# ascentai/diy-gym

Hardware: NVIDIA B200
Metric: aggregate env-steps/sec (higher is better)
Workload: dtype f32

## Files before the change

diy_gym_b200/csrc/dg_env.cuh:

```cuda
#pragma once
#include "dg_math.cuh"
#include "dg_scene.h"

namespace dg {

struct Env {
  const DevScene* sc;
  float* ws;
  float* wg;
  float* st;
  float* pr;
  const float* act;
  float* obs;
  float* rew;
  uint8_t* term;
  const int* link_i;
  const float* link_f;
  const float* link_x;
  uint32_t seed;
  int env_id;
  bool active;
  int grp0, grp1;
  unsigned long long opmask[2];
  unsigned long long* dbg;
  unsigned* dropped;
  int split;
  int* rs_lists; int rs_stride;
  int* rs_count;
  int e_local;
  unsigned* rs_used;
  int no_hot;
};

#define SC (*C.sc)
#if defined(__CUDA_ARCH__)
DG_HD float* as_shared(float* p) { __builtin_assume(__isShared(p)); return p; }
DG_HD float* as_global(float* p) { __builtin_assume(__isGlobal(p)); return p; }
template <class P> DG_HD const P* gc(const P* p) { __builtin_assume(__isGlobal(p)); return p; }
template <class P> DG_HD const P* shc(const P* p) { __builtin_assume(__isShared(p)); return p; }
#else
DG_HD float* as_shared(float* p) { return p; }
DG_HD float* as_global(float* p) { return p; }
template <class P> DG_HD const P* gc(const P* p) { return p; }
template <class P> DG_HD const P* shc(const P* p) { return p; }
#endif
#define WSH(C, off) (as_shared((C).ws) + (off))
#define WSG(C, off) (as_global((C).wg) + (off))
#define WSI(C) ((int*)as_shared((C).ws))
#define WSP(C, off) ((off) >= 0 ? (C).ws + (off) : (C).wg + ~(off))
#define WSIP(C, off) ((int*)WSP(C, off))
#define KIN(s) (WSG(C, SC.W_KIN) + 12 * (s))
#define LNK(gl) (WSG(C, SC.W_LINK) + LK_W * (gl))
#define ABA(s) (WSG(C, SC.X_ABA) + AB_W * (s))
#define LNX(gl) (WSG(C, SC.X_LNK) + LX_W * (gl))
#define DOF(k, d) (as_shared(C.ws)[SC.W_DOF + (k) * SC.nd + (d)])
#define BST(di) (WSH(C, SC.W_BST) + 13 * (di))
#define ST(name) (as_global(C.st) + DG_SO(C.sc, name))
#define PR(name) (as_global(C.pr) + DG_PO(C.sc, name))

DG_HD float clampf(float x, float lo, float hi) { return fminf(fmaxf(x, lo), hi); }
DG_HD int float_as_int(float f) { union { float f; int i; } u; u.f = f; return u.i; }
DG_HD float int_as_float(int i) { union { float f; int i; } u; u.i = i; return u.f; }

DG_FN void phase_load(const Env& C, int ln, int nt) {
  const DevScene& sc = SC;
  for (int i = ln; i < 13 * sc.ndyn; i += nt) {
    int di = i / 13, k = i - 13 * di, b = gc(sc.dyn_body)[di];
    float v;
    if (k < 3) v = ST(S_BPOS)[3 * b + k];
    else if (k < 7) v = ST(S_BQUAT)[4 * b + k - 3];
    else if (k < 10) v = ST(S_BVEL)[3 * b + k - 7];
    else v = ST(S_BOMEGA)[3 * b + k - 10];
    BST(di)[k] = v;
  }
  for (int d = ln; d < sc.nd; d += nt) {
    float qd = ST(S_QD)[d];
    DOF(D_Q, d) = ST(S_Q)[d]; DOF(D_QD, d) = qd; DOF(D_APPLIED, d) = ST(S_MAPPLIED)[d];
    DOF(D_TAU, d) = ST(S_JTORQUE)[d] - PR(P_JDAMP)[d] * qd;
  }
  for (int f = ln; f < sc.nb; f += nt) {
    int s = gc(sc.frame_slot)[f];
    if (s < 0 || gc(sc.body_i)[DG_BODY_I_W * f] != 0) continue;
    float* K = KIN(s);
    q_to_mat(K, ST(S_BQUAT) + 4 * f); v_cpy(K + 9, ST(S_BPOS) + 3 * f);
  }
  if (ln == 0) for (int i = 0; i < WH_COUNT; i++) WSI(C)[sc.W_HDR + i] = 0;
}

DG_FN void joint_xform(const Env& C, int gl, float q, float* E, float* r) {
  const int* li = shc(C.link_i) + DG_LINK_I_W * gl; const float* lf = shc(C.link_f) + DG_LINK_F_W * gl; const float* R0 = shc(C.link_x) + 16 * gl;
  float Rrel[9], tmp[3];
  if (li[2] == 1) { float Ra[9]; axis_angle_mat(Ra, lf + 10, q, C.sc->precise != 0); m_mul(Rrel, R0, Ra); m_vec(tmp, Rrel, lf + 7); }
  else if (li[2] == 2) { m_cpy(Rrel, R0); float dd[3] = {lf[7] + lf[10] * q, lf[8] + lf[11] * q, lf[9] + lf[12] * q}; m_vec(tmp, R0, dd); }
  else { m_cpy(Rrel, R0); m_vec(tmp, R0, lf + 7); }
  v_add(r, lf + 4, tmp);
  E[0] = Rrel[0]; E[1] = Rrel[3]; E[2] = Rrel[6]; E[3] = Rrel[1]; E[4] = Rrel[4]; E[5] = Rrel[7]; E[6] = Rrel[2]; E[7] = Rrel[5]; E[8] = Rrel[8];
}
DG_HD int parent_slot(const int* li, int l0, int s0) { return li[1] < 0 ? s0 : s0 + 1 + (li[1] - l0); }

struct F4 { float x, y, z, w; };
DG_HD F4 ld4(const float* p) {
#if defined(__CUDA_ARCH__)
  float4 v = *reinterpret_cast<const float4*>(p); F4 o = {v.x, v.y, v.z, v.w}; return o;
#else
  F4 o = {p[0], p[1], p[2], p[3]}; return o;
#endif
}
DG_HD void st4(float* p, float x, float y, float z, float w) {
#if defined(__CUDA_ARCH__)
  *reinterpret_cast<float4*>(p) = make_float4(x, y, z, w);
#else
  p[0] = x; p[1] = y; p[2] = z; p[3] = w;
#endif
}
template <int N> DG_HD void ldn(const float* p, float* o) {
#pragma unroll
  for (int c = 0; c < N / 4; c++) { F4 v = ld4(p + 4 * c); o[4 * c] = v.x; o[4 * c + 1] = v.y; o[4 * c + 2] = v.z; o[4 * c + 3] = v.w; }
}
template <int N> DG_HD void stn(float* p, const float* v) {
#pragma unroll
  for (int c = 0; c < N / 4; c++) st4(p + 4 * c, v[4 * c], v[4 * c + 1], v[4 * c + 2], v[4 * c + 3]);
}

template <bool BIAS>
DG_FN void fk_vel_body(const Env& C, int b) {
  const DevScene& sc = SC;
  const int* bi = gc(sc.body_i) + DG_BODY_I_W * b; const int* bp = gc(sc.body_plan) + BP_W * b;
  const int kind = bi[0], l0 = bi[1], nlb = bi[2], s0 = bp[BP_SLOT];
  const float* bs = BST(bp[BP_DI]);
  const float *mass = PR(P_MASS), *inertia = PR(P_INERTIA);
  const float kl = PR(P_LINDAMP)[b], ka = PR(P_ANGDAMP)[b];
  float Kp[12], Vp[6];
  q_to_mat(Kp, bs + 3); v_cpy(Kp + 9, bs);
  mT_vec(Vp, Kp, bs + 10); mT_vec(Vp + 3, Kp, bs + 7);
  int prev = s0;
  for (int k = -1; k < nlb; k++) {
    const int s = s0 + 1 + k, f = k < 0 ? b : sc.nb + l0 + k;
    float K[12], V[6], cacc[8] = {0, 0, 0, 0, 0, 0, 0, 0};
    if (k < 0) {
      for (int i = 0; i < 12; i++) K[i] = Kp[i];
      for (int i = 0; i < 6; i++) V[i] = Vp[i];
    } else {
      const int gl = l0 + k; const int* li = shc(C.link_i) + DG_LINK_I_W * gl; const float* lx = shc(C.link_x) + 16 * gl;
      const int ps = parent_slot(li, l0, s0), dof = li[3];
      if (ps != prev) { ldn<12>(KIN(ps), Kp); const float* pv = ABA(ps) + AB_WV; for (int i = 0; i < 6; i++) Vp[i] = pv[i]; }
      float E[9], r[3], t[3], t2[3];
      joint_xform(C, gl, dof >= 0 ? DOF(D_Q, dof) : 0.f, E, r);
      float* L = LNK(gl);
      st4(L, E[0], E[1], E[2], E[3]); st4(L + 4, E[4], E[5], E[6], E[7]); st4(L + 8, E[8], r[0], r[1], r[2]);
      m_mulT(K, Kp, E);
      m_vec(t, Kp, r); v_add(K + 9, Kp + 9, t);
      m_vec(V, E, Vp);
      v_cross(t, Vp, r); v_add(t2, Vp + 3, t); m_vec(V + 3, E, t2);
      if (dof >= 0) {
        const float qd = DOF(D_QD, dof);
        if (BIAS) { float sa[3], sl[3]; v_scale(sa, lx + 9, qd); v_scale(sl, lx + 12, qd); v_cross(cacc, V, sa); v_cross(cacc + 3, V, sl); v_cross(t2, V + 3, sa); v_add(cacc + 3, cacc + 3, t2); }
        v_madd(V, lx + 9, qd); v_madd(V + 3, lx + 12, qd);
      }
      if (BIAS) stn<8>(LNX(gl), cacc);
    }
    stn<12>(KIN(s), K);
    float* X = ABA(s);
    if (!BIAS) {
      for (int i = 0; i < 6; i++) X[AB_WV + i] = V[i];
    } else if (k < 0 && kind != 2) {
      float z[40]; for (int i = 0; i < 40; i++) z[i] = 0.f;
      for (int i = 0; i < 6; i++) z[AB_WV + i] = V[i];
      stn<40>(X, z);
    } else {
      const float wsc = ((sc.sem & SEM_WRENCH_FIRST_SUBSTEP) && WSI(C)[sc.W_HDR + WH_SUB] > 0) ? 0.f : 1.f;
      const float efv[3] = {wsc * ST(S_EXTF)[3 * f], wsc * ST(S_EXTF)[3 * f + 1], wsc * ST(S_EXTF)[3 * f + 2]}, etv[3] = {wsc * ST(S_EXTT)[3 * f], wsc * ST(S_EXTT)[3 * f + 1], wsc * ST(S_EXTT)[3 * f + 2]};
      const float *ef = efv, *et = etv;
      const float m = mass[f]; const float* I = inertia + 3 * f; const float *w = V, *v = V + 3;
      float Iw[3] = {I[0] * w[0], I[1] * w[1], I[2] * w[2]}, t[3], fw[3], pa[3], pl[3];
      v_cross(pa, w, Iw);
      v_cross(t, w, v); v_scale(pl, t, m);
      fw[0] = sc.g[0] * m + ef[0]; fw[1] = sc.g[1] * m + ef[1]; fw[2] = sc.g[2] * m + ef[2];
      mT_vec(t, K, fw); v_sub(pl, pl, t);
      mT_vec(t, K, et); v_sub(pa, pa, t);
      const float wn = v_len(w), vn = v_len(v);
      const bool dlin = (sc.sem & SEM_DAMPING_LINEAR) != 0;
      v_madd(pa, Iw, dlin ? ka : ka + ka * wn);
      float mv[3]; v_scale(mv, v, m); v_madd(pl, mv, dlin ? kl : kl + kl * vn);
      float z[40]; for (int i = 0; i < 40; i++) z[i] = 0.f;
      for (int i = 0; i < 3; i++) { z[AB_PA + i] = pa[i]; z[AB_PA + 3 + i] = pl[i]; z[AB_WV + i] = w[i]; z[AB_WV + 3 + i] = v[i]; }
      z[AB_A] = I[0]; z[AB_A + 4] = I[1]; z[AB_A + 8] = I[2]; z[AB_C] = m; z[AB_C + 4] = m; z[AB_C + 8] = m;
      stn<40>(X, z);
    }
    for (int i = 0; i < 12; i++) Kp[i] = K[i];
    for (int i = 0; i < 6; i++) Vp[i] = V[i];
    prev = s;
  }
}

DG_HD void ia_mul(const float* A, const float* B, const float* Cm, const float* a, const float* l, float* n, float* f) {
  float t[3]; m_vec(n, A, a); m_vec(t, B, l); v_add(n, n, t); mT_vec(f, B, a); m_vec(t, Cm, l); v_add(f, f, t);
}
DG_FN int invert_small(float* M, int n, float* inv) {
  for (int i = 0; i < n; i++) for (int j = 0; j < n; j++) inv[i * n + j] = (i == j) ? 1.f : 0.f;
  for (int c = 0; c < n; c++) {
    int p = c;
    for (int r2 = c + 1; r2 < n; r2++) if (fabsf(M[r2 * n + c]) > fabsf(M[p * n + c])) p = r2;
    if (fabsf(M[p * n + c]) < 1e-30f) return -1;
    if (p != c) for (int j = 0; j < n; j++) { float t = M[c * n + j]; M[c * n + j] = M[p * n + j]; M[p * n + j] = t; t = inv[c * n + j]; inv[c * n + j] = inv[p * n + j]; inv[p * n + j] = t; }
    float d = 1.0f / M[c * n + c];
    for (int j = 0; j < n; j++) { M[c * n + j] *= d; inv[c * n + j] *= d; }
    for (int r2 = 0; r2 < n; r2++) if (r2 != c) {
      float fct = M[r2 * n + c];
      if (fct != 0.f) for (int j = 0; j < n; j++) { M[r2 * n + j] -= fct * M[c * n + j]; inv[r2 * n + j] -= fct * inv[c * n + j]; }
    }
  }
  return 0;
}

template <int N> DG_HD void inv_spd(const float (&A)[N][N], float (&Out)[N][N]) {
  float L[N][N], Li[N][N], invd[N];
#pragma unroll
  for (int j = 0; j < N; j++) {
    float d = A[j][j];
#pragma unroll
    for (int k = 0; k < N; k++) if (k < j) d -= L[j][k] * L[j][k];
    const float ljj = sqrtf(fmaxf(d, 1e-30f)), inv = 1.0f / ljj;
    L[j][j] = ljj; invd[j] = inv;
#pragma unroll
    for (int i = 0; i < N; i++) if (i > j) {
      float v = A[i][j];
#pragma unroll
      for (int k = 0; k < N; k++) if (k < j) v -= L[i][k] * L[j][k];
      L[i][j] = v * inv;
    }
  }
#pragma unroll
  for (int j = 0; j < N; j++) {
    Li[j][j] = invd[j];
#pragma unroll
    for (int i = 0; i < N; i++) if (i > j) {
      float v = 0.f;
#pragma unroll
      for (int k = 0; k < N; k++) if (k >= j && k < i) v -= L[i][k] * Li[k][j];
      Li[i][j] = v * invd[i];
    }
  }
#pragma unroll
  for (int i = 0; i < N; i++)
#pragma unroll
    for (int j = 0; j < N; j++) {
      float v = 0.f;
#pragma unroll
      for (int k = 0; k < N; k++) if (k >= i && k >= j) v += Li[k][i] * Li[k][j];
      Out[i][j] = v;
    }
}
DG_FN void aba_body(const Env& C, int b, float h) {
  const DevScene& sc = SC;
  const int* bi = gc(sc.body_i) + DG_BODY_I_W * b; const int* bp = gc(sc.body_plan) + BP_W * b;
  const int kind = bi[0], l0 = bi[1], nlb = bi[2], s0 = bp[BP_SLOT], di = bp[BP_DI];
  for (int k = nlb - 1; k >= 0; k--) {
    const int gl = l0 + k, s = s0 + 1 + k; const int* li = shc(C.link_i) + DG_LINK_I_W * gl;
    const int ps = parent_slot(li, l0, s0);
    float Xr[40], Lr[12], cx[8];
    ldn<40>(ABA(s), Xr); ldn<12>(LNK(gl), Lr); ldn<8>(LNX(gl), cx);
    float* Aa = Xr + AB_A; float* Ba = Xr + AB_B; float* Ca = Xr + AB_C; const float* pA = Xr + AB_PA;
    float pa[6], n[3], fo[3];
    if (li[3] >= 0) {
      const float* lx = shc(C.link_x) + 16 * gl; const float *sa = lx + 9, *sl = lx + 12;
      float U[6];
      ia_mul(Aa, Ba, Ca, sa, sl, U, U + 3);
      const float D = v_dot(sa, U) + v_dot(sl, U + 3);
      const float uu = DOF(D_TAU, li[3]) - (v_dot(sa, pA) + v_dot(sl, pA + 3));
      float* L = LNK(gl);
      st4(L + 12, U[0], U[1], U[2], U[3]); st4(L + 16, U[4], U[5], D, 0.f);
      LNX(gl)[6] = uu;
      const float Dinv = 1.0f / D;
#pragma unroll
      for (int i = 0; i < 3; i++)
#pragma unroll
        for (int j = 0; j < 3; j++) { Aa[3 * i + j] -= U[i] * U[j] * Dinv; Ba[3 * i + j] -= U[i] * U[3 + j] * Dinv; Ca[3 * i + j] -= U[3 + i] * U[3 + j] * Dinv; }
      ia_mul(Aa, Ba, Ca, cx, cx + 3, n, fo);
      for (int i = 0; i < 3; i++) { pa[i] = pA[i] + n[i] + U[i] * uu * Dinv; pa[3 + i] = pA[3 + i] + fo[i] + U[3 + i] * uu * Dinv; }
    } else {
      ia_mul(Aa, Ba, Ca, cx, cx + 3, n, fo);
      for (int i = 0; i < 3; i++) { pa[i] = pA[i] + n[i]; pa[3 + i] = pA[3 + i] + fo[i]; }
    }
    const float* E = Lr; const float* r = Lr + 9;
    float T1[9], Ar[9], Br[9], Cr[9];
    mT_mul(T1, E, Aa); m_mul(Ar, T1, E); mT_mul(T1, E, Ba); m_mul(Br, T1, E); mT_mul(T1, E, Ca); m_mul(Cr, T1, E);
    const float Kx[9] = {0, -r[2], r[1], r[2], 0, -r[0], -r[1], r[0], 0};
    float KC[9], BK[9], KBt[9], KCK[9];
    m_mul(KC, Kx, Cr); m_mul(BK, Br, Kx); m_mulT(KBt, Kx, Br); m_mul(KCK, KC, Kx);
    float fp[3], np_[3], t[3];
    mT_vec(fp, E, pa + 3); mT_vec(np_, E, pa); v_cross(t, r, fp); v_add(np_, np_, t);
    float* P = ABA(ps);
    float Pr[40];
    ldn<40>(P, Pr);
    for (int i = 0; i < 9; i++) { Pr[AB_A + i] += Ar[i] - BK[i] + KBt[i] - KCK[i]; Pr[AB_B + i] += Br[i] + KC[i]; Pr[AB_C + i] += Cr[i]; }
    for (int i = 0; i < 3; i++) { Pr[AB_PA + i] += np_[i]; Pr[AB_PA + 3 + i] += fp[i]; }
    stn<40>(P, Pr);
  }
  float* X0 = ABA(s0); float* a0 = X0 + AB_ACC;
#if defined(DG_OLD_INV)
  if (kind == 2) {
    float* M = WSG(C, sc.X_I0T) + bp[BP_I0OFF]; float* Iv = WSG(C, sc.W_I0) + bp[BP_I0OFF];
    const float *A = X0 + AB_A, *B = X0 + AB_B, *Cm = X0 + AB_C;
    for (int i = 0; i < 3; i++) for (int j = 0; j < 3; j++) { M[6 * i + j] = A[3 * i + j]; M[6 * i + 3 + j] = B[3 * i + j]; M[6 * (3 + i) + j] = B[3 * j + i]; M[6 * (3 + i) + 3 + j] = Cm[3 * i + j]; }
    invert_small(M, 6, Iv);
    for (int i = 0; i < 6; i++) { float sum = 0.f; for (int j = 0; j < 6; j++) sum -= Iv[6 * i + j] * X0[AB_PA + j]; a0[i] = sum; }
  } else for (int i = 0; i < 6; i++) a0[i] = 0.f;
#else
  if (kind == 2) {
    float* Iv = WSG(C, sc.W_I0) + bp[BP_I0OFF];
    float Xr[40]; ldn<40>(X0, Xr);
    const float *A = Xr + AB_A, *B = Xr + AB_B, *Cm = Xr + AB_C;
    float M[6][6], Inv[6][6];
#pragma unroll
    for (int i = 0; i < 3; i++)
#pragma unroll
      for (int j = 0; j < 3; j++) { M[i][j] = A[3 * i + j]; M[i][3 + j] = B[3 * i + j]; M[3 + i][j] = B[3 * j + i]; M[3 + i][3 + j] = Cm[3 * i + j]; }
    inv_spd<6>(M, Inv);
    float iv[36];
#pragma unroll
    for (int i = 0; i < 6; i++)
#pragma unroll
      for (int j = 0; j < 6; j++) iv[6 * i + j] = Inv[i][j];
    stn<36>(Iv, iv);
#pragma unroll
    for (int i = 0; i < 6; i++) { float sum = 0.f;
#pragma unroll
      for (int j = 0; j < 6; j++) sum -= Inv[i][j] * Xr[AB_PA + j];
      a0[i] = sum; }
  } else for (int i = 0; i < 6; i++) a0[i] = 0.f;
#endif
  float ap[8]; int prev = s0;
  ldn<8>(a0, ap);
  for (int k = 0; k < nlb; k++) {
    const int gl = l0 + k, s = s0 + 1 + k; const int* li = shc(C.link_i) + DG_LINK_I_W * gl;
    const int ps = parent_slot(li, l0, s0);
    if (ps != prev) ldn<8>(ABA(ps) + AB_ACC, ap);
    float Lr[20], cx[8];
    ldn<20>(LNK(gl), Lr); ldn<8>(LNX(gl), cx);
    float t[3], t2[3], acc[8];
    m_vec(acc, Lr, ap); v_cross(t, ap, Lr + 9); v_add(t2, ap + 3, t); m_vec(acc + 3, Lr, t2);
    v_add(acc, acc, cx); v_add(acc + 3, acc + 3, cx + 3);
    if (li[3] >= 0) {
      const float* lx = shc(C.link_x) + 16 * gl;
      const float qdd = (cx[6] - (v_dot(Lr + 12, acc) + v_dot(Lr + 15, acc + 3))) / Lr[18];
      DOF(D_QD, li[3]) += h * qdd;
      v_madd(acc, lx + 9, qdd); v_madd(acc + 3, lx + 12, qdd);
    }
    acc[6] = 0.f; acc[7] = 0.f;
    stn<8>(ABA(s) + AB_ACC, acc);
    for (int i = 0; i < 8; i++) ap[i] = acc[i];
    prev = s;
  }
  if (kind == 2) {
    const float* K0 = KIN(s0); float* bs = BST(di); float t[3], lin[3], aw[3];
    v_cross(t, X0 + AB_WV, X0 + AB_WV + 3); v_add(lin, a0 + 3, t);
    m_vec(aw, K0, a0); v_madd(bs + 10, aw, h);
    m_vec(aw, K0, lin); v_madd(bs + 7, aw, h);
  }
}

DG_FN void joint_reactions(const Env& C, int b) {
  const DevScene& sc = SC;
  const int* bi = gc(sc.body_i) + DG_BODY_I_W * b; const int l0 = bi[1], nlb = bi[2], s0 = gc(sc.body_plan)[BP_W * b + BP_SLOT];
  for (int k = 0; k < nlb; k++) {
    float X[48], n[3], f[3];
    ldn<48>(ABA(s0 + 1 + k), X);
    ia_mul(X + AB_A, X + AB_B, X + AB_C, X + AB_ACC, X + AB_ACC + 3, n, f);
    float* o = ST(S_JREACT) + 6 * (l0 + k);
    for (int i = 0; i < 3; i++) { o[i] = X[AB_PA + 3 + i] + f[i]; o[3 + i] = X[AB_PA + i] + n[i]; }
  }
}
DG_FN void phase_dynamics(const Env& C, int ln, int nt, float h) {
  for (int di = ln; di < SC.ndyn; di += nt) { int b = gc(SC.dyn_body)[di]; fk_vel_body<true>(C, b); aba_body(C, b, h); if (SC.need_react) joint_reactions(C, b); }
}

DG_FN void minv_column(const Env& C, int b, int col, float* scr) {
  const DevScene& sc = SC;
  const int* bi = gc(sc.body_i) + DG_BODY_I_W * b; const int* bp = gc(sc.body_plan) + BP_W * b;
  const int kind = bi[0], l0 = bi[1], nlb = bi[2], d0 = bi[3], s0 = bp[BP_SLOT], g = bp[BP_GDIM], gs = bp[BP_GS];
  const int jo = kind == 2 ? 6 : 0;
  float* out = WSH(C, sc.W_MINV) + bp[BP_MINVOFF] + col * gs;
  for (int i = g; i < gs; i++) out[i] = 0.f;
  (void)scr;
  float uu[DG_MINV_MAXL], ast[6 * DG_MINV_MAXD];
  for (int k = 0; k < nlb; k++) uu[k] = 0.f;
  float p[6] = {0, 0, 0, 0, 0, 0};
  if (col >= jo) {
    int k0 = -1;
    for (int k = 0; k < nlb; k++) if (shc(C.link_i)[DG_LINK_I_W * (l0 + k) + 3] == d0 + col - jo) { k0 = k; break; }
    for (int k = k0; k >= 0;) {
      const int gl = l0 + k; const int* li = shc(C.link_i) + DG_LINK_I_W * gl;
      float L[20]; ldn<20>(LNK(gl), L);
      float pa[6] = {p[0], p[1], p[2], p[3], p[4], p[5]};
      if (li[3] >= 0) {
        const float* lx = shc(C.link_x) + 16 * gl;
        const float u1 = (k == k0 ? 1.f : 0.f) - (v_dot(lx + 9, pa) + v_dot(lx + 12, pa + 3));
        uu[k] = u1; const float s = u1 / L[18];
        for (int i = 0; i < 6; i++) pa[i] += L[12 + i] * s;
      }
      float fp[3], np_[3], t[3];
      mT_vec(fp, L, pa + 3); mT_vec(np_, L, pa); v_cross(t, L + 9, fp); v_add(np_, np_, t);
      v_cpy(p, np_); v_cpy(p + 3, fp);
      k = li[1] < 0 ? -1 : li[1] - l0;
    }
  }
  float a0[6];
  if (kind == 2) {
    float K0[12]; ldn<12>(KIN(s0), K0); const float* Iv = WSG(C, sc.W_I0) + bp[BP_I0OFF];
    float gen[6] = {0, 0, 0, 0, 0, 0}, rhs[6], t[3];
    for (int i = 0; i < 6; i++) gen[i] = (i == col) ? 1.f : 0.f;
    mT_vec(t, K0, gen); v_sub(rhs, t, p); mT_vec(t, K0, gen + 3); v_sub(rhs + 3, t, p + 3);
    for (int i = 0; i < 6; i++) { float s = 0.f; for (int j = 0; j < 6; j++) s += Iv[6 * i + j] * rhs[j]; a0[i] = s; }
    m_vec(out, K0, a0); m_vec(out + 3, K0, a0 + 3);
  } else for (int i = 0; i < 6; i++) a0[i] = 0.f;
  for (int i = 0; i < 6; i++) ast[i] = a0[i];
  float ap[6] = {a0[0], a0[1], a0[2], a0[3], a0[4], a0[5]}; int prev_dep = -1;
  for (int k = 0; k < nlb; k++) {
    const int gl = l0 + k; const int* li = shc(C.link_i) + DG_LINK_I_W * gl;
    const int dep = gc(sc.link_depth)[gl];
    if (dep - 1 != prev_dep) { const float* src = ast + 6 * dep; for (int i = 0; i < 6; i++) ap[i] = src[i]; }
    float L[20]; ldn<20>(LNK(gl), L);
    float t[3], t2[3], aa[3], al[3];
    m_vec(aa, L, ap); v_cross(t, ap, L + 9); v_add(t2, ap + 3, t); m_vec(al, L, t2);
    if (li[3] >= 0) {
      const float* lx = shc(C.link_x) + 16 * gl;
      const float qdd = (uu[k] - (v_dot(L + 12, aa) + v_dot(L + 15, al))) / L[18];
      out[jo + li[3] - d0] = qdd;
      v_madd(aa, lx + 9, qdd); v_madd(al, lx + 12, qdd);
    }
    float* ak = ast + 6 * (dep + 1);
    v_cpy(ak, aa); v_cpy(ak + 3, al);
    v_cpy(ap, aa); v_cpy(ap + 3, al); prev_dep = dep;
  }
}
DG_FN void phase_minv(const Env& C, int ln, int nt) {
  const DevScene& sc = SC;
  float* scr = WSG(C, sc.X_MSCR) + sc.mscr_stride * ln;
  int item = 0;
  for (int di = 0; di < sc.ndyn; di++) {
    int b = gc(sc.dyn_body)[di], g = gc(sc.body_plan)[BP_W * b + BP_GDIM];
    for (int col = 0; col < g; col++, item++) if (item % nt == ln) minv_column(C, b, col, scr);
  }
}

struct Ct { int fa, fb; float pa[3], pb[3], n[3], dist, mu; };

DG_FN void shape_pose(const Env& C, int s, const float** R, const float** p) {
  int sl = gc(SC.shape_slot)[s];
  const float* w = sl >= 0 ? WSP(C, SC.X_SHW) + 12 * sl : gc(SC.shape_wb) + 12 * s;
  *R = w; *p = w + 9;
}
DG_FN void phase_shape_world(const Env& C, int ln, int nt) {
  const DevScene& sc = SC;
  for (int s = ln; s < sc.ns; s += nt) {
    int sl = gc(sc.shape_slot)[s];
    if (sl < 0) continue;
    const float* sf = gc(sc.shape_f) + DG_SHAPE_F_W * s; const float* K = KIN(gc(sc.frame_slot)[gc(sc.shape_i)[DG_SHAPE_I_W * s + 1]]);
    float* w = WSP(C, sc.X_SHW) + 12 * sl; float Rl[9], R[9], t[3];
    q_to_mat(Rl, sf + 3); m_mul(R, K, Rl); m_cpy(w, R); m_vec(t, K, sf); v_add(w + 9, K + 9, t);
  }
  int nw = (sc.npair + 31) / 32;
  for (int i = ln; i < nw; i += nt) WSIP(C, sc.X_SURV)[i] = 0;
  if (ln == 0) { int* hdr = WSI(C) + sc.W_HDR; hdr[WH_NCONTACT] = 0; hdr[WH_RS_R] = 0; hdr[WH_RS_DEFER] = 0; }
}
DG_HD void ct_add(Ct* list, int* n, int cap, int fa, int fb, const float* pa, const float* pb, const float* nrm, float dist, float mu, float margin) {
  if (dist > margin || *n >= cap) return;
  Ct* c = &list[(*n)++]; c->fa = fa; c->fb = fb; v_cpy(c->pa, pa); v_cpy(c->pb, pb); v_cpy(c->n, nrm); c->dist = dist; c->mu = mu;
}
DG_FN int sphere_box(const float* c, float r, const float* Rb, const float* pb, const float* h, float* pa_out, float* pb_out, float* n, float* dist) {
  float d[3], cl[3], q[3]; v_sub(d, c, pb); mT_vec(cl, Rb, d);
  int inside = 1;
  for (int i = 0; i < 3; i++) { q[i] = cl[i]; if (q[i] > h[i]) { q[i] = h[i]; inside = 0; } else if (q[i] < -h[i]) { q[i] = -h[i]; inside = 0; } }
  float nl[3] = {0, 0, 0};
  if (!inside) {
    float dv[3]; v_sub(dv, cl, q); float len = v_len(dv);
    if (len < 1e-12f) return 0;
    v_scale(nl, dv, 1.0f / len); *dist = len - r;
  } else {
    int ax = 0; float best = 1e30f;
    for (int i = 0; i < 3; i++) { float pen = h[i] - fabsf(cl[i]); if (pen < best) { best = pen; ax = i; } }
    float sg = cl[ax] >= 0 ? 1.0f : -1.0f;
    for (int i = 0; i < 3; i++) if (i == ax) { nl[i] = sg; q[i] = sg * h[i]; }
    *dist = -best - r;
  }
  m_vec(n, Rb, nl); float t[3]; m_vec(t, Rb, q); v_add(pb_out, pb, t);
  v_scale(t, n, -r); v_add(pa_out, c, t);
  return 1;
}
DG_FN int point_box(const float* p, const float* Rb, const float* pb, const float* h, float margin, float* pb_out, float* n, float* dist) {
  float d[3], pl[3]; v_sub(d, p, pb); mT_vec(pl, Rb, d);
  int ax = 0; float best = 1e30f;
  for (int i = 0; i < 3; i++) { float pen = h[i] - fabsf(pl[i]); if (pen < -margin) return 0; if (pen < best) { best = pen; ax = i; } }
  float nl[3] = {0, 0, 0}, q[3] = {pl[0], pl[1], pl[2]};
  float sg = pl[ax] >= 0 ? 1.0f : -1.0f;
  for (int i = 0; i < 3; i++) if (i == ax) { nl[i] = sg; q[i] = sg * h[i]; }
  m_vec(n, Rb, nl); float t[3]; m_vec(t, Rb, q); v_add(pb_out, pb, t); *dist = -best;
  return 1;
}
DG_FN void seg_closest(const float* p1, const float* d1, const float* p2, const float* d2, float* s, float* t) {
  float r[3]; v_sub(r, p1, p2);
  float a = v_dot(d1, d1), e = v_dot(d2, d2), f = v_dot(d2, r);
  if (a <= 1e-18f && e <= 1e-18f) { *s = *t = 0; return; }
  if (a <= 1e-18f) { *s = 0; *t = clampf(f / e, 0.f, 1.f); return; }
  float c = v_dot(d1, r);
  if (e <= 1e-18f) { *t = 0; *s = clampf(-c / a, 0.f, 1.f); return; }
  float b = v_dot(d1, d2), den = a * e - b * b;
  *s = den > 1e-18f ? clampf((b * f - c * e) / den, 0.f, 1.f) : 0.0f;
  *t = (b * (*s) + f) / e;
  if (*t < 0) { *t = 0; *s = clampf(-c / a, 0.f, 1.f); } else if (*t > 1) { *t = 1; *s = clampf((b - c) / a, 0.f, 1.f); }
}
DG_FN void as_capsule(int type, const float* dims, const float* R, const float* p, float* e0, float* e1, float* rad) {
  float half = 0; *rad = dims[0];
  if (type == SHAPE_CAPSULE) half = dims[1];
  else if (type == SHAPE_CYLINDER) half = dims[1] - dims[0] > 0 ? dims[1] - dims[0] : 0;
  float ax[3] = {R[2] * half, R[5] * half, R[8] * half};
  v_sub(e0, p, ax); v_add(e1, p, ax);
}
DG_HD bool pair_in_reach(const Env& C, int sa, int sb) {
  const float *Ra, *pa, *Rb, *pb;
  shape_pose(C, sa, &Ra, &pa); shape_pose(C, sb, &Rb, &pb);
  float dc[3]; v_sub(dc, pa, pb);
  const float ra = gc(SC.shape_f)[DG_SHAPE_F_W * sa + 11], rb = gc(SC.shape_f)[DG_SHAPE_F_W * sb + 11];
  float reach = ra + rb + SC.margin;
  if (v_dot(dc, dc) > reach * reach) return false;
  for (int side = 0; side < 2; side++) {
    const int sx = side ? sa : sb;
    const int* ix = gc(SC.shape_i) + DG_SHAPE_I_W * sx;
    if (ix[2] != SHAPE_BOX || ix[5] > 0) continue;
    const float *Rx = side ? Ra : Rb, *px = side ? pa : pb, *po = side ? pb : pa; const float* h = gc(SC.shape_f) + DG_SHAPE_F_W * sx + 7;
    float d[3], pl[3]; v_sub(d, po, px); mT_vec(pl, Rx, d);
    float d2 = 0.f;
    for (int i = 0; i < 3; i++) { const float ex = fabsf(pl[i]) - h[i]; if (ex > 0.f) d2 += ex * ex; }
    const float r = (side ? rb : ra) + SC.margin;
    if (d2 > r * r) return false;
  }
  return true;
}
DG_FN int point_hull(const float* p, const float* R, const float* pos, const float* planes, int np_, float margin, float* surf, float* n, float* dist) {
  float d[3], pl[3]; v_sub(d, p, pos); mT_vec(pl, R, d);
  float best = -1e30f; int bi = 0;
  for (int k = 0; k < np_; k++) { const float* q = planes + 4 * k; const float s = q[0] * pl[0] + q[1] * pl[1] + q[2] * pl[2] - q[3]; if (s > margin) return 0; if (s > best) { best = s; bi = k; } }
  m_vec(n, R, planes + 4 * bi); *dist = best;
  surf[0] = p[0] - n[0] * best; surf[1] = p[1] - n[1] * best; surf[2] = p[2] - n[2] * best;
  return 1;
}
DG_FN void collide_convex(const Env& C, const int* ia, const float* fa, const float* Ra, const float* pa, const int* ib, const float* fb, const float* Rb, const float* pb,
                          float mu, float margin, Ct* loc, int* nloc) {
  const float* H = gc(SC.hull_f);
  for (int side = 0; side < 2; side++) {
    const int* ix = side ? ib : ia; const int* iy = side ? ia : ib; const float* fx = side ? fb : fa; const float* fy = side ? fa : fb;
    const float *Rx = side ? Rb : Ra, *px = side ? pb : pa, *Ry = side ? Ra : Rb, *py = side ? pa : pb;
    const int nvx = ix[5] > 0 ? ix[5] : 8;
    const float reach2 = (fy[11] + margin) * (fy[11] + margin);
    for (int k = 0; k < nvx; k++) {
      float vl[3], t[3], pt[3], surf[3], n[3], dist;
      if (ix[5] > 0) { const float* v = H + ix[4] + 3 * k; vl[0] = v[0]; vl[1] = v[1]; vl[2] = v[2]; }
      else { vl[0] = (k & 1 ? 1 : -1) * fx[7]; vl[1] = (k & 2 ? 1 : -1) * fx[8]; vl[2] = (k & 4 ? 1 : -1) * fx[9]; }
      m_vec(t, Rx, vl); v_add(pt, px, t);
      { float dy[3]; v_sub(dy, pt, py); if (v_dot(dy, dy) > reach2) continue; }
      const int hit = iy[5] > 0 ? point_hull(pt, Ry, py, H + iy[6], iy[7], margin, surf, n, &dist) : point_box(pt, Ry, py, fy + 7, margin, surf, n, &dist);
      if (!hit) continue;
      if (side == 0) ct_add(loc, nloc, 16, ia[1], ib[1], pt, surf, n, dist, mu, margin);
      else { float nn[3]; v_scale(nn, n, -1.0f); ct_add(loc, nloc, 16, ia[1], ib[1], surf, pt, nn, dist, mu, margin); }
    }
  }
}
DG_FN int collide_pair(const Env& C, int sa, int sb, Ct* out) {
  const DevScene& sc = SC;
  const int *ia = gc(sc.shape_i) + DG_SHAPE_I_W * sa, *ib = gc(sc.shape_i) + DG_SHAPE_I_W * sb;
  const float *fa = gc(sc.shape_f) + DG_SHAPE_F_W * sa, *fb = gc(sc.shape_f) + DG_SHAPE_F_W * sb;
  const float *Ra, *pa, *Rb, *pb;
  shape_pose(C, sa, &Ra, &pa); shape_pose(C, sb, &Rb, &pb);
  float margin = sc.margin;
  int ta = ia[2], tb = ib[2];
  float mu = PR(P_FRICTION)[sa] * PR(P_FRICTION)[sb];
  int nt_ = 0;
  float ca[3], cb[3], n[3], dist;
  const bool ha = ia[5] > 0, hb_ = ib[5] > 0;
  if ((ha && (hb_ || tb == SHAPE_BOX)) || (hb_ && (ha || ta == SHAPE_BOX))) {
    Ct loc[16]; int nloc = 0;
    collide_convex(C, ia, fa, Ra, pa, ib, fb, Rb, pb, mu, margin, loc, &nloc);
    for (int i = 0; i < nloc; i++) for (int j = i + 1; j < nloc; j++) if (loc[j].dist < loc[i].dist) { Ct t = loc[i]; loc[i] = loc[j]; loc[j] = t; }
    if (nloc > 4) nloc = 4;
    for (int i = 0; i < nloc; i++) out[nt_++] = loc[i];
    return nt_;
  }
  if (ta != SHAPE_BOX && tb != SHAPE_BOX) {
    float a0[3], a1[3], b0[3], b1[3], ra, rb, d1[3], d2[3], s, t, c1[3], c2[3];
    as_capsule(ta, fa + 7, Ra, pa, a0, a1, &ra); as_capsule(tb, fb + 7, Rb, pb, b0, b1, &rb);
    v_sub(d1, a1, a0); v_sub(d2, b1, b0); seg_closest(a0, d1, b0, d2, &s, &t);
    v_cpy(c1, a0); v_madd(c1, d1, s); v_cpy(c2, b0); v_madd(c2, d2, t);
    float d[3]; v_sub(d, c1, c2); float len = v_len(d);
    if (len < 1e-12f) v_set(n, 0, 0, 1); else v_scale(n, d, 1.0f / len);
    dist = len - ra - rb; float tt[3]; v_scale(tt, n, -ra); v_add(ca, c1, tt); v_scale(tt, n, rb); v_add(cb, c2, tt);
    ct_add(out, &nt_, 4, ia[1], ib[1], ca, cb, n, dist, mu, margin);
    return nt_;
  }
  int swap = (tb != SHAPE_BOX);
  const float *Rx = swap ? Rb : Ra, *px = swap ? pb : pa, *dx = swap ? fb + 7 : fa + 7;
  const float *Rbx = swap ? Ra : Rb, *pbx = swap ? pa : pb, *hb = swap ? fa + 7 : fb + 7;
  int tx = swap ? tb : ta; int fx = swap ? ib[1] : ia[1], fbx = swap ? ia[1] : ib[1];
  Ct loc[16]; int nloc = 0;
  if (tx == SHAPE_SPHERE) {
    if (sphere_box(px, dx[0], Rbx, pbx, hb, ca, cb, n, &dist)) ct_add(loc, &nloc, 16, fx, fbx, ca, cb, n, dist, mu, margin);
  } else if (tx == SHAPE_CAPSULE) {
    float e0[3], e1[3], rad, mid[3], dseg[3], rel[3];
    as_capsule(tx, dx, Rx, px, e0, e1, &rad);
    v_sub(dseg, e1, e0); v_sub(rel, pbx, e0);
    float dd = v_dot(dseg, dseg), tt = dd > 1e-18f ? clampf(v_dot(rel, dseg) / dd, 0.f, 1.f) : 0.0f;
    v_cpy(mid, e0); v_madd(mid, dseg, tt);
    if (sphere_box(e0, rad, Rbx, pbx, hb, ca, cb, n, &dist)) ct_add(loc, &nloc, 16, fx, fbx, ca, cb, n, dist, mu, margin);
    if (dd > 1e-18f && sphere_box(e1, rad, Rbx, pbx, hb, ca, cb, n, &dist)) ct_add(loc, &nloc, 16, fx, fbx, ca, cb, n, dist, mu, margin);
    if (tt > 1e-6f && tt < 1 - 1e-6f && sphere_box(mid, rad, Rbx, pbx, hb, ca, cb, n, &dist)) ct_add(loc, &nloc, 16, fx, fbx, ca, cb, n, dist, mu, margin);
  } else if (tx == SHAPE_CYLINDER) {
    float zc[3] = {Rx[2], Rx[5], Rx[8]}, xc[3] = {Rx[0], Rx[3], Rx[6]}, yc[3] = {Rx[1], Rx[4], Rx[7]};
    for (int cap = -1; cap <= 1; cap += 2) {
      float cc[3]; v_cpy(cc, px); v_madd(cc, zc, cap * dx[1]);
      for (int k = 0; k < 6; k++) {
        float sg = k < 3 ? 1.f : -1.f; int a3 = k % 3;
        float nk[3] = {-Rbx[a3] * sg, -Rbx[3 + a3] * sg, -Rbx[6 + a3] * sg};
        float t[3]; v_cpy(t, nk); v_madd(t, zc, -v_dot(nk, zc));
        float len = v_len(t), pt[3];
        int npt = len < 1e-6f ? 4 : 1;
        for (int j4 = 0; j4 < npt; j4++) {
          if (npt == 4) { const float* bx = (j4 & 1) ? yc : xc; float s2 = (j4 & 2) ? -1.0f : 1.0f; v_cpy(pt, cc); v_madd(pt, bx, s2 * dx[0]); }
          else { v_cpy(pt, cc); v_madd(pt, t, dx[0] / len); }
          if (point_box(pt, Rbx, pbx, hb, margin, cb, n, &dist)) {
            int dup = 0;
            for (int j = 0; j < nloc; j++) { float dd[3]; v_sub(dd, loc[j].pa, pt); if (v_dot(dd, dd) < 1e-12f) dup = 1; }
            if (!dup) ct_add(loc, &nloc, 16, fx, fbx, pt, cb, n, dist, mu, margin);
          }
        }
      }
    }
  } else {
    for (int k = 0; k < 8; k++) {
      float cl[3] = {(k & 1 ? 1 : -1) * dx[0], (k & 2 ? 1 : -1) * dx[1], (k & 4 ? 1 : -1) * dx[2]}, pt[3], t[3];
      m_vec(t, Rx, cl); v_add(pt, px, t);
      if (point_box(pt, Rbx, pbx, hb, margin, cb, n, &dist)) ct_add(loc, &nloc, 16, fx, fbx, pt, cb, n, dist, mu, margin);
    }
    for (int k = 0; k < 8; k++) {
      float cl[3] = {(k & 1 ? 1 : -1) * hb[0], (k & 2 ? 1 : -1) * hb[1], (k & 4 ? 1 : -1) * hb[2]}, pt[3], t[3], nn[3], cx[3];
      m_vec(t, Rbx, cl); v_add(pt, pbx, t);
      if (point_box(pt, Rx, px, dx, margin, cx, nn, &dist)) { v_scale(nn, nn, -1.0f); ct_add(loc, &nloc, 16, fx, fbx, cx, pt, nn, dist, mu, margin); }
    }
  }
  for (int i = 0; i < nloc; i++) for (int j = i + 1; j < nloc; j++) if (loc[j].dist < loc[i].dist) { Ct t = loc[i]; loc[i] = loc[j]; loc[j] = t; }
  if (nloc > 4) nloc = 4;
  for (int i = 0; i < nloc; i++) {
    Ct c = loc[i];
    if (swap) { Ct s2 = c; s2.fa = c.fb; s2.fb = c.fa; v_cpy(s2.pa, c.pb); v_cpy(s2.pb, c.pa); v_scale(s2.n, c.n, -1.0f); c = s2; }
    out[nt_++] = c;
  }
  return nt_;
}
DG_HD void surv_set(int* word, int bit) {
#if defined(__CUDA_ARCH__)
  atomicOr(word, 1 << bit);
#else
  *word |= 1 << bit;
#endif
}
DG_HD int ffs64(unsigned long long x) {
#if defined(__CUDA_ARCH__)
  return __ffsll((long long)x);
#else
  return __builtin_ffsll((long long)x);
#endif
}
DG_HD int popc32(unsigned x) {
#if defined(__CUDA_ARCH__)
  return __popc(x);
#else
  return __builtin_popcount(x);
#endif
}
DG_FN void phase_broad(const Env& C, int ln, int nt) {
  const DevScene& sc = SC;
  for (int it = ln; it < sc.ngrp + sc.nloose; it += nt) {
    if (it < sc.ngrp) {
      const int* g = gc(sc.grp_i) + 4 * it; const float* w = gc(sc.shape_wb) + 12 * g[0];
      const float* cb = KIN(gc(sc.body_plan)[BP_W * g[1] + BP_SLOT]) + 9;
      float dc[3]; v_sub(dc, w + 9, cb);
      float reach = gc(sc.shape_f)[DG_SHAPE_F_W * g[0] + 11] + gc(sc.body_reach)[g[1]] + sc.margin;
      if (v_dot(dc, dc) > reach * reach) continue;
      {
        const int* is = gc(sc.shape_i) + DG_SHAPE_I_W * g[0];
        if (is[2] == SHAPE_BOX && is[5] == 0) {
          const float* h = gc(sc.shape_f) + DG_SHAPE_F_W * g[0] + 7;
          float d[3], pl[3]; v_sub(d, cb, w + 9); mT_vec(pl, w, d);
          float d2 = 0.f;
          for (int i = 0; i < 3; i++) { const float ex = fabsf(pl[i]) - h[i]; if (ex > 0.f) d2 += ex * ex; }
          const float r = gc(sc.body_reach)[g[1]] + sc.margin;
          if (d2 > r * r) continue;
        }
      }
      for (int j = 0; j < g[3]; j++) {
        int k = gc(sc.grp_pairs)[g[2] + j];
        if (pair_in_reach(C, gc(sc.pair_i)[2 * k], gc(sc.pair_i)[2 * k + 1])) surv_set(WSIP(C, sc.X_SURV) + (k >> 5), k & 31);
      }
    } else {
      int k = gc(sc.loose_pairs)[it - sc.ngrp];
      if (pair_in_reach(C, gc(sc.pair_i)[2 * k], gc(sc.pair_i)[2 * k + 1])) surv_set(WSIP(C, sc.X_SURV) + (k >> 5), k & 31);
    }
  }
}
DG_FN void phase_count_survivors(const Env& C, int ln, int nt) {
  if (ln != 0) return;
  int nw = (SC.npair + 31) / 32, n = 0;
  for (int i = 0; i < nw; i++) n += popc32((unsigned)WSIP(C, SC.X_SURV)[i]);
  WSI(C)[SC.W_HDR + WH_NSURV] = n;
}
DG_FN void phase_narrow(const Env& C, int ln, int nt, int rnd) {
  const DevScene& sc = SC;
  float* tmp = WSG(C, sc.X_CTMP) + sc.ctmp_stride * ln;
  int want = rnd * nt + ln, nw = (sc.npair + 31) / 32, seen = 0, pair = -1;
  for (int i = 0; i < nw && pair < 0; i++) {
    unsigned wd = (unsigned)WSIP(C, sc.X_SURV)[i]; int c = popc32(wd);
    if (seen + c <= want) { seen += c; continue; }
    for (int bit = 0; bit < 32; bit++) if (wd & (1u << bit)) { if (seen == want) { pair = 32 * i + bit; break; } seen++; }
  }
  int n = 0;
  if (pair >= 0) {
    Ct out[4];
    n = collide_pair(C, gc(sc.pair_i)[2 * pair], gc(sc.pair_i)[2 * pair + 1], out);
    for (int i = 0; i < n; i++) {
      float* c = tmp + 1 + CT_W * i;
      c[CT_FA] = int_as_float(out[i].fa); c[CT_FB] = int_as_float(out[i].fb);
      v_cpy(c + CT_PA, out[i].pa); v_cpy(c + CT_PB, out[i].pb); v_cpy(c + CT_N, out[i].n); c[CT_DIST] = out[i].dist; c[CT_MU] = out[i].mu;
    }
  }
  tmp[0] = int_as_float(n);
}
DG_FN void phase_append(const Env& C, int ln, int nt) {
  if (ln != 0) return;
  const DevScene& sc = SC;
  int nc = WSI(C)[sc.W_HDR + WH_NCONTACT], lost = 0;
  for (int l = 0; l < nt; l++) {
    const float* tmp = WSG(C, sc.X_CTMP) + sc.ctmp_stride * l; int n = float_as_int(tmp[0]);
    for (int i = 0; i < n; i++) {
      const float* src = tmp + 1 + CT_W * i; float* dst;
      if (nc < sc.maxc) dst = WSP(C, sc.X_CON) + CT_W * nc++;
      else {
        lost++;
        int worst = 0; float wd = (WSP(C, sc.X_CON))[CT_DIST];
        for (int j = 1; j < nc; j++) { const float dj = (WSP(C, sc.X_CON) + CT_W * j)[CT_DIST]; if (dj > wd) { wd = dj; worst = j; } }
        if (nc == 0 || !(src[CT_DIST] < wd)) continue;
        dst = WSP(C, sc.X_CON) + CT_W * worst;
      }
      for (int j = 0; j < CT_W; j++) dst[j] = src[j];
    }
  }
  WSI(C)[sc.W_HDR + WH_NCONTACT] = nc;
  if (lost && C.dropped) {
#if defined(__CUDA_ARCH__)
    atomicAdd(C.dropped, (unsigned)lost);
#else
    *C.dropped += (unsigned)lost;
#endif
  }
}

DG_HD int body_of_frame(const Env& C, int f) { return f < C.sc->nb ? f : shc(C.link_i)[DG_LINK_I_W * (f - C.sc->nb)]; }
DG_FN void point_jacobian(const Env& C, int f, const float* p, const float* dir, float* J) {
  const DevScene& sc = SC;
  int b = body_of_frame(C, f); const int* bi = gc(sc.body_i) + DG_BODY_I_W * b; const int* bp = gc(sc.body_plan) + BP_W * b;
  int g = bp[BP_GDIM], d0 = bi[3], s0 = bp[BP_SLOT], l0 = bi[1];
  for (int i = 0; i < g; i++) J[i] = 0.f;
  int jo = 0;
  if (bi[0] == 2) { float rel[3]; v_sub(rel, p, KIN(s0) + 9); v_cross(J, rel, dir); v_cpy(J + 3, dir); jo = 6; }
  int gl = f < sc.nb ? -1 : f - sc.nb;
  while (gl >= 0) {
    const int* li = shc(C.link_i) + DG_LINK_I_W * gl; const float* lf = shc(C.link_f) + DG_LINK_F_W * gl; const float* K = KIN(s0 + 1 + gl - l0);
    if (li[2] == 1) {
      float aw[3], dw[3], o[3], rel[3], t[3];
      m_vec(aw, K, lf + 10); m_vec(dw, K, lf + 7); v_sub(o, K + 9, dw);
      v_sub(rel, p, o); v_cross(t, aw, rel); J[jo + li[3] - d0] = v_dot(dir, t);
    } else if (li[2] == 2) { float aw[3]; m_vec(aw, K, lf + 10); J[jo + li[3] - d0] = v_dot(dir, aw); }
    gl = li[1];
  }
}
DG_FN void angular_jacobian(const Env& C, int f, const float* dir, float* J) {
  const DevScene& sc = SC;
  int b = body_of_frame(C, f); const int* bi = gc(sc.body_i) + DG_BODY_I_W * b; const int* bp = gc(sc.body_plan) + BP_W * b;
  int g = bp[BP_GDIM], d0 = bi[3], s0 = bp[BP_SLOT], l0 = bi[1], jo = 0;
  for (int i = 0; i < g; i++) J[i] = 0.f;
  if (bi[0] == 2) { v_cpy(J, dir); jo = 6; }
  for (int gl = f < sc.nb ? -1 : f - sc.nb; gl >= 0; gl = shc(C.link_i)[DG_LINK_I_W * gl + 1]) {
    const int* li = shc(C.link_i) + DG_LINK_I_W * gl;
    if (li[2] == 1) { float aw[3]; m_vec(aw, KIN(s0 + 1 + gl - l0), shc(C.link_f) + DG_LINK_F_W * gl + 10); J[jo + li[3] - d0] = v_dot(dir, aw); }
  }
}
DG_FN void body_genvel(const Env& C, int b, float* gv) {
  const int* bi = gc(SC.body_i) + DG_BODY_I_W * b; int jo = 0;
  if (bi[0] == 2) { const float* bs = BST(gc(SC.body_plan)[BP_W * b + BP_DI]); v_cpy(gv, bs + 10); v_cpy(gv + 3, bs + 7); jo = 6; }
  for (int i = 0; i < bi[4]; i++) gv[jo + i] = DOF(D_QD, bi[3] + i);
}
DG_FN void phase_unit_rows(const Env& C, int ln, int nt, float h) {
  const DevScene& sc = SC;
  for (int di = ln; di < sc.ndyn; di += nt) {
    int b = gc(sc.dyn_body)[di]; const int* bi = gc(sc.body_i) + DG_BODY_I_W * b; const int* bp = gc(sc.body_plan) + BP_W * b;
    int l0 = bi[1], nlb = bi[2], d0 = bi[3], g = bp[BP_GDIM], gs = bp[BP_GS], jo = bi[0] == 2 ? 6 : 0;
    const float* Minv = WSH(C, sc.W_MINV) + bp[BP_MINVOFF];
    float* rows = WSH(C, sc.X_UROW) + UR_W * bp[BP_UROW]; int n = 0;
    for (int k = 0; k < nlb; k++) {
      const int* li = shc(C.link_i) + DG_LINK_I_W * (l0 + k); const float* lf = shc(C.link_f) + DG_LINK_F_W * (l0 + k);
      int d = li[3];
      if (d < 0 || !li[4]) continue;
      for (int side = 0; side < 2; side++) {
        float pen = side == 0 ? DOF(D_Q, d) - lf[20] : lf[21] - DOF(D_Q, d);
        if (pen > 0) continue;
        int col = jo + d - d0; float sg = side == 0 ? 1.f : -1.f;
        float den = Minv[col * gs + col], dinv = den > 1e-30f ? 1.0f / den : 0.f, rel = sg * DOF(D_QD, d);
        float* r = rows + UR_W * n++;
        r[UR_RHS] = (-rel + (-pen) * sc.erp / h) * dinv; r[UR_DINV] = dinv; r[UR_LO] = 0.f; r[UR_HI] = sc.limit_max_impulse; r[UR_APPLIED] = 0.f;
        r[UR_COL] = int_as_float(side == 0 ? col : -1 - col); r[UR_MOTOR] = int_as_float(-1);
      }
    }
    for (int k = 0; k < nlb; k++) {
      int d = shc(C.link_i)[DG_LINK_I_W * (l0 + k) + 3];
      if (d < 0) continue;
      float maxf = ST(S_MMAXF)[d];
      DOF(D_APPLIED, d) = 0.f;
      if (maxf <= 0) continue;
      int col = jo + d - d0;
      float den = Minv[col * gs + col], dinv = den > 1e-30f ? 1.0f / den : 0.f, qd = DOF(D_QD, d);
      float desired = ST(S_MKP)[d] * (ST(S_MTPOS)[d] - DOF(D_Q, d)) / h + qd + ST(S_MKD)[d] * (ST(S_MTVEL)[d] - qd);
      float* r = rows + UR_W * n++;
      r[UR_RHS] = (desired - qd) * dinv; r[UR_DINV] = dinv; const float cdt = (sc.sem & SEM_MOTOR_CLAMP_SUBSTEP) ? h : sc.dt;
      r[UR_LO] = -maxf * cdt; r[UR_HI] = maxf * cdt; r[UR_APPLIED] = 0.f;
      r[UR_COL] = int_as_float(col); r[UR_MOTOR] = int_as_float(d);
    }
    WSI(C)[sc.W_UCNT + di] = n;
    float* dv = WSH(C, sc.W_DV) + bp[BP_GVOFF];
    for (int i = 0; i < gs; i++) dv[i] = 0.f;
    int nrs = bp[BP_NRS];
    if (n <= nrs) {
      float* A = WSH(C, sc.X_AMAT) + bp[BP_AOFF];
      for (int r = 0; r < n; r++) {
        int cr = float_as_int(rows[UR_W * r + UR_COL]); float sr = 1.f; if (cr < 0) { cr = -1 - cr; sr = -1.f; }
        for (int s2 = 0; s2 < nrs; s2++) {
          float a = 0.f;
          if (s2 < n) { int cs = float_as_int(rows[UR_W * s2 + UR_COL]); float ss = 1.f; if (cs < 0) { cs = -1 - cs; ss = -1.f; } a = sr * ss * Minv[cr * gs + cs]; }
          A[r * nrs + s2] = a;
        }
      }
    }
  }
  if (ln == 0) { WSI(C)[sc.W_HDR + WH_NCROW] = 3 * WSI(C)[sc.W_HDR + WH_NCONTACT]; WSI(C)[sc.W_HDR + WH_COUPLED] = 0; }
}
DG_FN void plane_space(const float* n, float* p, float* q) {
  if (fabsf(n[2]) > 0.7071067811865475244f) { float a = n[1] * n[1] + n[2] * n[2], k = 1.0f / sqrtf(a); p[0] = 0; p[1] = -n[2] * k; p[2] = n[1] * k; q[0] = a * k; q[1] = -n[0] * p[2]; q[2] = n[0] * p[1]; }
  else { float a = n[0] * n[0] + n[1] * n[1], k = 1.0f / sqrtf(a); p[0] = -n[1] * k; p[1] = n[0] * k; p[2] = 0; q[0] = -n[2] * p[1]; q[1] = n[2] * p[0]; q[2] = a * k; }
}
DG_FN void phase_contact_rows(const Env& C, int ln, int nt, float h) {
  const DevScene& sc = SC;
  int nc = WSI(C)[sc.W_HDR + WH_NCONTACT];
  for (int r = ln; r < 3 * nc; r += nt) {
    int k = r < nc ? r : (r - nc) >> 1, dirk = r < nc ? -1 : (r - nc) & 1;
    const float* c = WSP(C, sc.X_CON) + CT_W * k;
    int fa = float_as_int(c[CT_FA]), fb = float_as_int(c[CT_FB]);
    float dir[3];
    if (dirk < 0) v_cpy(dir, c + CT_N); else { float t1[3], t2[3]; plane_space(c + CT_N, t1, t2); v_cpy(dir, dirk == 0 ? t1 : t2); }
    float* row = WSP(C, sc.X_CROW) + sc.crow_stride * r; float* J = row + CR_HDR; float* M = J + sc.GP;
    int ba = body_of_frame(C, fa), bb = body_of_frame(C, fb);
    int dia = gc(sc.body_plan)[BP_W * ba + BP_DI], dib = gc(sc.body_plan)[BP_W * bb + BP_DI];
    float den = 0.f, rel = 0.f; int ga = 0;
    if (dia >= 0) {
      const int* bp = gc(sc.body_plan) + BP_W * ba; ga = bp[BP_GDIM]; const int gsa = bp[BP_GS]; const float* Minv = WSH(C, sc.W_MINV) + bp[BP_MINVOFF];
      point_jacobian(C, fa, c + CT_PA, dir, J);
      body_genvel(C, ba, M);
      for (int i = 0; i < ga; i++) rel += J[i] * M[i];
      for (int i = 0; i < ga; i++) { float s = 0.f; for (int j = 0; j < ga; j++) s += Minv[j * gsa + i] * J[j]; M[i] = s; }
      for (int i = 0; i < ga; i++) den += J[i] * M[i];
    }
    if (dib >= 0) {
      const int* bp = gc(sc.body_plan) + BP_W * bb; int gb = bp[BP_GDIM]; const int gsb = bp[BP_GS]; const float* Minv = WSH(C, sc.W_MINV) + bp[BP_MINVOFF];
      float nd_[3]; v_scale(nd_, dir, -1.0f);
      float *JB = J + ga, *MB = M + ga;
      point_jacobian(C, fb, c + CT_PB, nd_, JB);
      body_genvel(C, bb, MB);
      for (int i = 0; i < gb; i++) rel += JB[i] * MB[i];
      for (int i = 0; i < gb; i++) { float s = 0.f; for (int j = 0; j < gb; j++) s += Minv[j * gsb + i] * JB[j]; MB[i] = s; }
      for (int i = 0; i < gb; i++) den += JB[i] * MB[i];
    }
    { int used = ga + (dib >= 0 ? gc(sc.body_plan)[BP_W * bb + BP_GDIM] : 0); for (int i = used; i < sc.GP; i++) { J[i] = 0.f; M[i] = 0.f; } }
    if (dia >= 0 && dib >= 0) WSI(C)[sc.W_HDR + WH_COUPLED] = 1;
    float dinv = den > 1e-30f ? 1.0f / den : 0.f;
    row[CR_DINV] = dinv; row[CR_APPLIED] = 0.f; row[CR_MU] = c[CT_MU]; WSH(C, sc.W_CAPP)[r] = 0.f;
    row[CR_DA] = int_as_float(dia); row[CR_DB] = int_as_float(dib);
    if (dirk < 0) {
      float pen = c[CT_DIST] + sc.slop, pos_err = 0.f, vel_err = -rel;
      if (pen > 0) vel_err -= pen / h; else pos_err = -pen * sc.cerp / h;
      row[CR_RHS] = (pos_err + vel_err) * dinv; row[CR_LO] = 0.f; row[CR_HI] = 1e10f; row[CR_PARENT] = int_as_float(-1);
    } else {
      row[CR_RHS] = -rel * dinv; row[CR_LO] = 0.f; row[CR_HI] = 0.f; row[CR_PARENT] = int_as_float(k);
    }
  }
}

DG_FN void pgs_unit_sweep(const Env& C, int b, int di, int it) {
  const DevScene& sc = SC;
  const int* bp = gc(sc.body_plan) + BP_W * b; int g = bp[BP_GDIM], gs = bp[BP_GS], n = WSI(C)[sc.W_UCNT + di];
  const float* Minv = WSH(C, sc.W_MINV) + bp[BP_MINVOFF]; float* dv = WSH(C, sc.W_DV) + bp[BP_GVOFF];
  float* rows = WSH(C, sc.X_UROW) + UR_W * bp[BP_UROW];
  for (int j = 0; j < n; j++) {
    float* r = rows + UR_W * ((it & 1) ? j : n - 1 - j);
    int colc = float_as_int(r[UR_COL]); float sg = 1.f; int col = colc;
    if (colc < 0) { col = -1 - colc; sg = -1.f; }
    float d = r[UR_RHS] - sg * dv[col] * r[UR_DINV];
    float ap = r[UR_APPLIED], sum = ap + d, lo = r[UR_LO], hi = r[UR_HI];
    if (sum < lo) { d = lo - ap; sum = lo; } else if (sum > hi) { d = hi - ap; sum = hi; }
    r[UR_APPLIED] = sum;
    float sd = sg * d; const float* Mc = Minv + col * gs;
    for (int i = 0; i < g; i++) dv[i] = fmaf(Mc[i], sd, dv[i]);
  }
}
template <int NR>
DG_FN void pgs_unit_fast(const Env& C, int b, int di, int it0, int it1) {
  const DevScene& sc = SC;
  const int* bp = gc(sc.body_plan) + BP_W * b; const int g = bp[BP_GDIM], gs = bp[BP_GS], nrs = bp[BP_NRS], n = WSI(C)[sc.W_UCNT + di];
  const float* Minv = WSH(C, sc.W_MINV) + bp[BP_MINVOFF]; float* dv = WSH(C, sc.W_DV) + bp[BP_GVOFF];
  float* rows = WSH(C, sc.X_UROW) + UR_W * bp[BP_UROW]; const float* A = WSH(C, sc.X_AMAT) + bp[BP_AOFF];
  constexpr bool kRegA = NR <= 8;
  float rhs[NR], dinv[NR], lo[NR], hi[NR], ap[NR], ap0[NR], y[NR], Ar[kRegA ? NR * NR : 1];
#pragma unroll
  for (int r = 0; r < NR; r++) {
    rhs[r] = 0.f; dinv[r] = 0.f; lo[r] = 0.f; hi[r] = 0.f; ap[r] = 0.f; y[r] = 0.f;
    if (r < n) {
      const float* rw = rows + UR_W * r;
      rhs[r] = rw[UR_RHS]; dinv[r] = rw[UR_DINV]; lo[r] = rw[UR_LO]; hi[r] = rw[UR_HI]; ap[r] = rw[UR_APPLIED];
      int c = float_as_int(rw[UR_COL]);
      y[r] = c < 0 ? -dv[-1 - c] : dv[c];
    }
    ap0[r] = ap[r];
    if (kRegA) {
#pragma unroll
      for (int s2 = 0; s2 < NR; s2++) Ar[kRegA ? r * NR + s2 : 0] = (r < n && s2 < n) ? A[r * nrs + s2] : 0.f;
    }
  }
#define DG_PGS_ROW(r)                                                                        \
  {                                                                                          \
    float d = rhs[r] - y[r] * dinv[r];                                                       \
    float sum = ap[r] + d;                                                                   \
    const bool below = sum < lo[r], above = sum > hi[r];                                     \
    d = below ? lo[r] - ap[r] : (above ? hi[r] - ap[r] : d);                                 \
    ap[r] = below ? lo[r] : (above ? hi[r] : sum);                                           \
    if (kRegA) {                                                                             \
      _Pragma("unroll") for (int s2 = 0; s2 < NR; s2++) y[s2] = fmaf(Ar[kRegA ? (r) * NR + s2 : 0], d, y[s2]); \
    } else if ((r) < n) {                                                                    \
      const float* Am = A + (r) * nrs;                                                       \
      _Pragma("unroll") for (int s2 = 0; s2 < NR; s2++) y[s2] = fmaf(Am[s2], d, y[s2]);      \
    }                                                                                        \
  }
  for (int it = it0; it < it1; it++) {
    if (it & 1) {
#pragma unroll
      for (int r = 0; r < NR; r++) DG_PGS_ROW(r)
    } else {
#pragma unroll
      for (int r = NR - 1; r >= 0; r--) DG_PGS_ROW(r)
    }
  }
#undef DG_PGS_ROW
#pragma unroll
  for (int r = 0; r < NR; r++) if (r < n) {
    float* rw = rows + UR_W * r;
    rw[UR_APPLIED] = ap[r];
    float dl = ap[r] - ap0[r];
    int c = float_as_int(rw[UR_COL]); if (c < 0) { c = -1 - c; dl = -dl; }
    const float* Mc = Minv + c * gs;
    for (int i = 0; i < g; i++) dv[i] = fmaf(Mc[i], dl, dv[i]);
  }
}
DG_FN void pgs_unit_any(const Env& C, int b, int di, int it0, int it1) {
  const int nrs = gc(SC.body_plan)[BP_W * b + BP_NRS], n = WSI(C)[SC.W_UCNT + di];
  if (n == 0) return;
  if (n <= nrs) {
    if (n <= 4) { pgs_unit_fast<4>(C, b, di, it0, it1); return; }
    if (n <= 6 && nrs >= 8) { pgs_unit_fast<6>(C, b, di, it0, it1); return; }
    if (n <= 8) { pgs_unit_fast<8>(C, b, di, it0, it1); return; }
    if (n <= 12) { pgs_unit_fast<12>(C, b, di, it0, it1); return; }
    if (n <= 16) { pgs_unit_fast<16>(C, b, di, it0, it1); return; }
  }
  for (int it = it0; it < it1; it++) pgs_unit_sweep(C, b, di, it);
}
template <int G>
DG_FN void pgs_body_full(const Env& C, int b, int di) {
  const DevScene& sc = SC;
  const int* bp = gc(sc.body_plan) + BP_W * b; const int gs = bp[BP_GS], n = WSI(C)[sc.W_UCNT + di];
  const int ncr = WSI(C)[sc.W_HDR + WH_NCROW];
  const float* Minv = WSH(C, sc.W_MINV) + bp[BP_MINVOFF]; float* dvs = WSH(C, sc.W_DV) + bp[BP_GVOFF];
  float* rows = WSH(C, sc.X_UROW) + UR_W * bp[BP_UROW];
  float* capp = WSH(C, sc.W_CAPP);
  unsigned long long mine = 0ull;
  for (int rr = 0; rr < ncr && rr < 63; rr++) {
    const float* row = WSP(C, sc.X_CROW) + sc.crow_stride * rr;
    if (float_as_int(row[CR_DA]) == di || float_as_int(row[CR_DB]) == di) mine |= 1ull << rr;
  }
  float dv[G];
#pragma unroll
  for (int i = 0; i < G; i++) dv[i] = 0.f;
  for (int it = 0; it < sc.iters; it++) {
    for (int j = 0; j < n; j++) {
      float* r = rows + UR_W * ((it & 1) ? j : n - 1 - j);
      int col = float_as_int(r[UR_COL]); float sg = 1.f;
      if (col < 0) { col = -1 - col; sg = -1.f; }
      float x = 0.f;
#pragma unroll
      for (int i = 0; i < G; i++) x = (i == col) ? dv[i] : x;
      float d = r[UR_RHS] - sg * x * r[UR_DINV];
      float ap = r[UR_APPLIED], sum = ap + d, lo = r[UR_LO], hi = r[UR_HI];
      if (sum < lo) { d = lo - ap; sum = lo; } else if (sum > hi) { d = hi - ap; sum = hi; }
      r[UR_APPLIED] = sum;
      float sd = sg * d; const float* Mc = Minv + col * gs;
#pragma unroll
      for (int c4 = 0; c4 < G / 4; c4++) if (4 * c4 < gs) {
        F4 m = ld4(Mc + 4 * c4);
        dv[4 * c4] = fmaf(m.x, sd, dv[4 * c4]); dv[4 * c4 + 1] = fmaf(m.y, sd, dv[4 * c4 + 1]);
        dv[4 * c4 + 2] = fmaf(m.z, sd, dv[4 * c4 + 2]); dv[4 * c4 + 3] = fmaf(m.w, sd, dv[4 * c4 + 3]);
      }
    }
    for (unsigned long long m = mine; m != 0ull; m &= m - 1ull) {
      const int rr = ffs64(m) - 1;
      const float* row = WSP(C, sc.X_CROW) + sc.crow_stride * rr;
      const float* J = row + CR_HDR; const float* M = J + sc.GP;
      const F4 h = ld4(row), h2 = ld4(row + 4), h3 = ld4(row + 8);
      F4 jv[G / 4], mv[G / 4];
#pragma unroll
      for (int c4 = 0; c4 < G / 4; c4++) {
        if (4 * c4 < gs) { jv[c4] = ld4(J + 4 * c4); mv[c4] = ld4(M + 4 * c4); }
        else { F4 z = {0.f, 0.f, 0.f, 0.f}; jv[c4] = z; mv[c4] = z; }
      }
      float d0 = 0.f, d1 = 0.f, d2 = 0.f, d3 = 0.f;
#pragma unroll
      for (int c4 = 0; c4 < G / 4; c4++) {
        d0 = fmaf(jv[c4].x, dv[4 * c4], d0); d1 = fmaf(jv[c4].y, dv[4 * c4 + 1], d1); d2 = fmaf(jv[c4].z, dv[4 * c4 + 2], d2); d3 = fmaf(jv[c4].w, dv[4 * c4 + 3], d3);
      }
      float d = h.x - ((d0 + d1) + (d2 + d3)) * h.y;
      float lo = h.z, hi = h.w;
      const int par = float_as_int(h3.x);
      if (par >= 0) { hi = h2.y * capp[par]; lo = -hi; }
      const float ap = capp[rr]; float sum = ap + d;
      const bool below = sum < lo, above = sum > hi;
      d = below ? lo - ap : (above ? hi - ap : d);
      capp[rr] = below ? lo : (above ? hi : sum);
#pragma unroll
      for (int c4 = 0; c4 < G / 4; c4++) {
        dv[4 * c4] = fmaf(mv[c4].x, d, dv[4 * c4]); dv[4 * c4 + 1] = fmaf(mv[c4].y, d, dv[4 * c4 + 1]);
        dv[4 * c4 + 2] = fmaf(mv[c4].z, d, dv[4 * c4 + 2]); dv[4 * c4 + 3] = fmaf(mv[c4].w, d, dv[4 * c4 + 3]);
      }
    }
  }
#pragma unroll
  for (int i = 0; i < G; i++) if (i < gs) dvs[i] = dv[i];
}
DG_FN void phase_pgs_full(const Env& C, int ln, int nt) {
  for (int di = ln; di < SC.ndyn; di += nt) {
    int b = gc(SC.dyn_body)[di], gs = gc(SC.body_plan)[BP_W * b + BP_GS];
    if (gs <= 8) pgs_body_full<8>(C, b, di); else if (gs <= 16) pgs_body_full<16>(C, b, di); else pgs_body_full<32>(C, b, di);
  }
}
DG_FN void pgs_contact_sweep(const Env& C) {
  const DevScene& sc = SC;
  int ncr = WSI(C)[sc.W_HDR + WH_NCROW];
  for (int r = 0; r < ncr; r++) {
    float* row = WSP(C, sc.X_CROW) + sc.crow_stride * r; const float* J = row + CR_HDR; const float* M = J + sc.GP;
    int dia = float_as_int(row[CR_DA]), dib = float_as_int(row[CR_DB]);
    float dot = 0.f; int ga = 0; float *dva = nullptr, *dvb = nullptr; int gb = 0;
    if (dia >= 0) { const int* bp = gc(sc.body_plan) + BP_W * gc(sc.dyn_body)[dia]; ga = bp[BP_GDIM]; dva = WSH(C, sc.W_DV) + bp[BP_GVOFF]; for (int i = 0; i < ga; i++) dot += J[i] * dva[i]; }
    if (dib >= 0) { const int* bp = gc(sc.body_plan) + BP_W * gc(sc.dyn_body)[dib]; gb = bp[BP_GDIM]; dvb = WSH(C, sc.W_DV) + bp[BP_GVOFF]; for (int i = 0; i < gb; i++) dot += J[ga + i] * dvb[i]; }
    float d = row[CR_RHS] - dot * row[CR_DINV];
    float lo = row[CR_LO], hi = row[CR_HI];
    int par = float_as_int(row[CR_PARENT]);
    float* capp = WSH(C, sc.W_CAPP);
    if (par >= 0) { hi = row[CR_MU] * capp[par]; lo = -hi; }
    float ap = capp[r], sum = ap + d;
    if (sum < lo) { d = lo - ap; sum = lo; } else if (sum > hi) { d = hi - ap; sum = hi; }
    capp[r] = sum;
    for (int i = 0; i < ga; i++) dva[i] = fmaf(M[i], d, dva[i]);
    for (int i = 0; i < gb; i++) dvb[i] = fmaf(M[ga + i], d, dvb[i]);
  }
}
DG_FN void phase_pgs_unit(const Env& C, int ln, int nt, int it0, int it1) {
  for (int di = ln; di < SC.ndyn; di += nt) pgs_unit_any(C, gc(SC.dyn_body)[di], di, it0, it1);
}
DG_FN void phase_pgs_contact(const Env& C, int ln, int nt) { if (ln == 0) pgs_contact_sweep(C); }
struct RsLayout { int K, nu, nk, nc, P1, nrm0, nrm1, P2, fr1, Rp; };
DG_HD int rs_pad(int n, int K) { return (n + K - 1) / K * K; }
DG_HD int rs_total(int nu, int nk, int nc, int K) { return rs_pad(nu, K) + rs_pad(nk + nc, K) + rs_pad(2 * nc, K); }
DG_HD RsLayout rs_layout(int K, int nu, int nk, int nc) {
  RsLayout L; L.K = K; L.nu = nu; L.nk = nk; L.nc = nc; L.P1 = rs_pad(nu, K); L.nrm0 = L.P1 + nk; L.nrm1 = L.nrm0 + nc;
  L.P2 = L.P1 + rs_pad(nk + nc, K); L.fr1 = L.P2 + 2 * nc; L.Rp = L.P2 + rs_pad(2 * nc, K);
  return L;
}
DG_HD bool rs_real(const RsLayout& L, int p) { return p < L.nu || (p >= L.P1 && p < L.nrm1) || (p >= L.P2 && p < L.fr1); }
DG_FN RsLayout rs_layout_of(const Env& C) {
  const int* hdr = WSI(C) + SC.W_HDR;
  return rs_layout(hdr[WH_RS_K], hdr[WH_RS_NU], 6 * SC.ncons, hdr[WH_NCROW] / 3);
}
DG_HD int rs_kneed(int nu, int nk, int nc, int nt, int cap) {
  for (int K = 2; K <= RS_KMAX; K *= 2) { const int t = rs_total(nu, nk, nc, K); if (t <= K * nt && t <= cap) return K; }
  return 0;
}
DG_FN void phase_rs_plan(const Env& C, int ln, int nt) {
  if (ln != 0) return;
  const DevScene& sc = SC;
  int* hdr = WSI(C) + sc.W_HDR; const int ncr = hdr[WH_NCROW];
  int nu = 0;
  for (int di = 0; di < sc.ndyn; di++) nu += WSI(C)[sc.W_UCNT + di];
  const int nk = 6 * sc.ncons, nc = ncr / 3;
  const bool want = sc.solver == 1 && nt >= 2 && (nk > 0 || (ncr > 0 && (hdr[WH_COUPLED] != 0 || ncr >= sc.rs_min)));
  hdr[WH_RS_NU] = nu; hdr[WH_RS_R] = 0; hdr[WH_RS_DEFER] = 0;
  int need = want ? rs_kneed(nu, nk, nc, nt, sc.rs_cap) : 0;
  if (want && C.split) {
    for (int c = 0; c < RS_NCLS; c++) {
      const int kc = sc.rs_cls_k[c], rc = sc.rs_cls_r[c];
      if (rc <= 0) continue;
      const int t = rs_total(nu, nk, nc, kc);
      if (t <= rc && t <= sc.rs_cap) { need = kc; hdr[WH_RS_DEFER] = c + 1; break; }
    }
  }
  hdr[WH_RS_NEED] = need;
}
DG_FN void phase_rs_setup(const Env& C, int ln, int nt) {
  const DevScene& sc = SC;
  int* hdr = WSI(C) + sc.W_HDR; const int ncr = hdr[WH_NCROW], GV = sc.GV;
  if (hdr[WH_RS_NEED] == 0) return;
  int K = 0;
  const bool defer = hdr[WH_RS_DEFER] != 0;
  if (defer) K = hdr[WH_RS_NEED];
  else for (int e2 = C.grp0; e2 < C.grp1; e2++) {
    const int* h2 = (const int*)(as_shared(C.ws) + (long)e2 * sc.w_total) + sc.W_HDR;
    const int k2 = h2[WH_RS_DEFER] ? 0 : h2[WH_RS_NEED]; K = k2 > K ? k2 : K;
  }
  const int nu = hdr[WH_RS_NU], nk = 6 * sc.ncons;
  const RsLayout L = rs_layout(K, nu, nk, ncr / 3);
  if (L.Rp > sc.rs_cap) return;
  if (ln == 0) {
    hdr[WH_RS_R] = L.Rp; hdr[WH_RS_K] = K;
#if defined(__CUDA_ARCH__)
    if (C.rs_used) atomicAdd(C.rs_used, 1u);
    if (defer) { const int cls = hdr[WH_RS_DEFER] - 1; const int slot = atomicAdd(C.rs_count + cls, 1); C.rs_lists[(size_t)cls * C.rs_stride + slot] = C.e_local; }
#endif
  }
  float* RSV = WSG(C, sc.X_RSV); float* REC = WSG(C, sc.X_RSREC);
  for (int p = ln; p < L.Rp; p += nt) if (!rs_real(L, p)) { float* rc = REC + RR_W * p; st4(rc, 0.f, 0.f, 0.f, 0.f); st4(rc + 4, 0.f, int_as_float(-1), 0.f, int_as_float(-1)); }
  int r = 0;
  for (int di = 0; di < sc.ndyn; di++) {
    const int* bp = gc(sc.body_plan) + BP_W * gc(sc.dyn_body)[di]; const int n = WSI(C)[sc.W_UCNT + di];
    for (int j = 0; j < n; j++, r++) {
      if (r % nt != ln) continue;
      const float* u = WSH(C, sc.X_UROW) + UR_W * (bp[BP_UROW] + j);
      int col = float_as_int(u[UR_COL]); float sg = 1.f; if (col < 0) { col = -1 - col; sg = -1.f; }
      float* Jd = RSV + (size_t)r * 2 * GV; float* Md = Jd + GV;
      for (int i = 0; i < 2 * GV; i += 4) st4(Jd + i, 0.f, 0.f, 0.f, 0.f);
      const int go = bp[BP_GVOFF], gs = bp[BP_GS]; const float* Mc = WSH(C, sc.W_MINV) + bp[BP_MINVOFF] + col * gs;
      Jd[go + col] = sg;
      for (int i = 0; i < gs; i++) Md[go + i] = sg * Mc[i];
      float* rc = REC + RR_W * r;
      st4(rc, u[UR_RHS], u[UR_DINV], u[UR_LO], u[UR_HI]); st4(rc + 4, 0.f, int_as_float(-1), int_as_float(((go + col) & ~3) | ((((go + col) & ~3) + 4) << 16)), int_as_float((di << 16) | j));
    }
  }
  for (int kr = 0; kr < nk; kr++) {
    const int r2 = L.P1 + kr;
    if (kr % nt != ln) continue;
    const int kc = kr / 6, i = kr % 6;
    const int* ci = gc(sc.cons_i) + DG_CONS_I_W * kc; const float* cf = gc(sc.cons_f) + DG_CONS_F_W * kc;
    const int fa = ci[0], fb = ci[1], ba = body_of_frame(C, fa), bb = body_of_frame(C, fb);
    const float *Ka = KIN(gc(sc.frame_slot)[fa]), *Kb = KIN(gc(sc.frame_slot)[fb]);
    float Pa[3], Pb[3], t[3], err;
    m_vec(t, Ka, cf); v_add(Pa, Ka + 9, t); m_vec(t, Kb, cf + 7); v_add(Pb, Kb + 9, t);
    if (i < 3) err = Pa[i] - Pb[i];
    else {
      float qa[4], qb[4], qaw[4], qbw[4], dq[4];
      mat_to_q(qa, Ka); mat_to_q(qb, Kb); q_mul(qaw, qa, cf + 3); q_mul(qbw, qb, cf + 10);
      const float qbi[4] = {-qbw[0], -qbw[1], -qbw[2], qbw[3]};
      q_mul(dq, qaw, qbi);
      const float vn = v_len(dq); float ang = 2.f * atan2f(vn, dq[3]); if (ang > kPi) ang -= 2.f * kPi;
      err = vn < 1e-12f ? 0.f : dq[i - 3] * ang / vn;
    }
    float e[3] = {0.f, 0.f, 0.f}, ne[3] = {0.f, 0.f, 0.f}; e[i % 3] = 1.f; ne[i % 3] = -1.f;
    float* Jd = RSV + (size_t)r2 * 2 * GV; float* Md = Jd + GV;
    for (int c = 0; c < 2 * GV; c += 4) st4(Jd + c, 0.f, 0.f, 0.f, 0.f);
    float den = 0.f, rel = 0.f, gvl[RS_GVMAX + 8];
    for (int side = 0; side < 2; side++) {
      const int b = side ? bb : ba, f = side ? fb : fa; const int* bp = gc(sc.body_plan) + BP_W * b;
      if (bp[BP_DI] < 0) continue;
      const int go = bp[BP_GVOFF], g = bp[BP_GDIM], gs = bp[BP_GS]; const float* Minv = WSH(C, sc.W_MINV) + bp[BP_MINVOFF];
      if (i < 3) point_jacobian(C, f, side ? Pb : Pa, side ? ne : e, Jd + go); else angular_jacobian(C, f, side ? ne : e, Jd + go);
      body_genvel(C, b, gvl);
      for (int c = 0; c < g; c++) { float sm = 0.f; for (int j = 0; j < g; j++) sm += Minv[j * gs + c] * Jd[go + j]; Md[go + c] = sm; den += Jd[go + c] * sm; rel += Jd[go + c] * gvl[c]; }
    }
    const float dinv = den > 1e-30f ? 1.0f / den : 0.f, lim = cf[14] * sc.dt, hsub = sc.dt / (float)sc.substeps;
    float* rc = REC + RR_W * r2;
    st4(rc, (-rel - err * sc.erp / hsub) * dinv, dinv, -lim, lim); st4(rc + 4, 0.f, int_as_float(-1), int_as_float(0 | (GV << 16)), int_as_float(RS_CONTACT | 0xffff));
  }
  const int nc = ncr / 3;
  for (int rr = 0; rr < ncr; rr++) {
    const int r2 = rr < nc ? L.nrm0 + rr : L.P2 + (rr - nc);
    if (rr % nt != ln) continue;
    const float* row = WSP(C, sc.X_CROW) + sc.crow_stride * rr; const float* J = row + CR_HDR; const float* M = J + sc.GP;
    const int dia = float_as_int(row[CR_DA]), dib = float_as_int(row[CR_DB]);
    float* Jd = RSV + (size_t)r2 * 2 * GV; float* Md = Jd + GV;
    for (int i = 0; i < 2 * GV; i += 4) st4(Jd + i, 0.f, 0.f, 0.f, 0.f);
    int off = 0, slo = GV, shi = 0;
#define DG_COPY_ROW(dstJ, dstM, srcJ, srcM, g_)                                                                                   \
    { int i_ = 0;                                                                                                                  \
      for (; i_ + 4 <= (g_); i_ += 4) {                                                                                            \
        const float j0_ = (srcJ)[i_], j1_ = (srcJ)[i_ + 1], j2_ = (srcJ)[i_ + 2], j3_ = (srcJ)[i_ + 3];                            \
        const float m0_ = (srcM)[i_], m1_ = (srcM)[i_ + 1], m2_ = (srcM)[i_ + 2], m3_ = (srcM)[i_ + 3];                            \
        (dstJ)[i_] = 0.f + j0_; (dstJ)[i_ + 1] = 0.f + j1_; (dstJ)[i_ + 2] = 0.f + j2_; (dstJ)[i_ + 3] = 0.f + j3_;                \
        (dstM)[i_] = 0.f + m0_; (dstM)[i_ + 1] = 0.f + m1_; (dstM)[i_ + 2] = 0.f + m2_; (dstM)[i_ + 3] = 0.f + m3_;                \
      }                                                                                                                            \
      for (; i_ < (g_); i_++) { const float j0_ = (srcJ)[i_], m0_ = (srcM)[i_]; (dstJ)[i_] = 0.f + j0_; (dstM)[i_] = 0.f + m0_; } }
    if (dia >= 0) { const int* bp = gc(sc.body_plan) + BP_W * gc(sc.dyn_body)[dia]; const int go = bp[BP_GVOFF], g = bp[BP_GDIM]; DG_COPY_ROW(Jd + go, Md + go, J, M, g) off = g; slo = go < slo ? go : slo; shi = go + bp[BP_GS] > shi ? go + bp[BP_GS] : shi; }
    if (dib >= 0) {
      const int* bp = gc(sc.body_plan) + BP_W * gc(sc.dyn_body)[dib]; const int go = bp[BP_GVOFF], g = bp[BP_GDIM];
      if (dib == dia) { for (int i = 0; i < g; i++) { Jd[go + i] += J[off + i]; Md[go + i] += M[off + i]; } }
      else DG_COPY_ROW(Jd + go, Md + go, J + off, M + off, g)
      slo = go < slo ? go : slo; shi = go + bp[BP_GS] > shi ? go + bp[BP_GS] : shi;
    }
    if (shi <= slo) { slo = 0; shi = 0; }
    float* rc = REC + RR_W * r2;
    st4(rc, row[CR_RHS], row[CR_DINV], row[CR_LO], row[CR_HI]); st4(rc + 4, row[CR_MU], row[CR_PARENT], int_as_float(slo | (shi << 16)), int_as_float(RS_CONTACT | rr));
  }
}
#undef DG_COPY_ROW
DG_FN void phase_rs_build(const Env& C, int ln, int nt) {
  const DevScene& sc = SC;
  const RsLayout L = rs_layout_of(C); const int GV = sc.GV, cap = sc.rs_cap;
  int ncol = L.K * nt; if (ncol > cap) ncol = cap; if (ncol < L.Rp) ncol = L.Rp;
  const float* RSV = WSG(C, sc.X_RSV); const float* REC = WSG(C, sc.X_RSREC); float* A = WSG(C, sc.X_RSA);
  for (int s2 = ln; s2 < ncol; s2 += nt) {
    const bool rs2 = s2 < L.Rp && rs_real(L, s2);
    int c0 = 0, c1 = 0;
    if (rs2) { const int sup = float_as_int(REC[RR_W * s2 + RR_APPLIED]); c0 = sup & 0xffff; c1 = (sup >> 16) & 0xffff; if (c1 > GV) c1 = GV; }
    const float* Jd = RSV + (size_t)s2 * 2 * GV;
    for (int p = 0; p < L.Rp; p++) {
      float a0 = 0.f, a1 = 0.f, a2 = 0.f, a3 = 0.f;
      if (rs2 && rs_real(L, p)) {
        const float* Md = RSV + (size_t)p * 2 * GV + GV;
        for (int c = c0; c < c1; c += 4) { const F4 jv = ld4(Jd + c), mv = ld4(Md + c); a0 = fmaf(jv.x, mv.x, a0); a1 = fmaf(jv.y, mv.y, a1); a2 = fmaf(jv.z, mv.z, a2); a3 = fmaf(jv.w, mv.w, a3); }
      }
      A[p * cap + s2] = (a0 + a1) + (a2 + a3);
    }
  }
}
DG_FN void phase_rs_finish(const Env& C, int ln, int nt) {
  const DevScene& sc = SC;
  const RsLayout L = rs_layout_of(C); const int GV = sc.GV;
  const float* RSV = WSG(C, sc.X_RSV); const float* REC = WSG(C, sc.X_RSREC); float* dv = WSH(C, sc.W_DV);
  for (int i = ln; i < GV; i += nt) {
    float sum = 0.f;
    for (int p = 0; p < L.Rp; p++) if (rs_real(L, p)) sum = fmaf(RSV[(size_t)p * 2 * GV + GV + i], REC[RR_W * p + RR_APPLIED], sum);
    dv[i] = sum;
  }
  for (int r = ln; r < L.nu; r += nt) {
    const int v = float_as_int(REC[RR_W * r + RR_ID]); const int* bp = gc(sc.body_plan) + BP_W * gc(sc.dyn_body)[(v >> 16) & 0x3fff];
    (WSH(C, sc.X_UROW) + UR_W * (bp[BP_UROW] + (v & 0xffff)))[UR_APPLIED] = REC[RR_W * r + RR_APPLIED];
  }
}
#if defined(__CUDA_ARCH__) && defined(DG_STEP_T)
template <int K> struct RsRow { float v[K]; };
template <int K> __device__ __forceinline__ RsRow<K> rs_ldrow(const float* p) {
  RsRow<K> r;
  if constexpr (K == 2) { const float2 v = *reinterpret_cast<const float2*>(p); r.v[0] = v.x; r.v[1] = v.y; }
  else {
#pragma unroll
    for (int c = 0; c < K / 4; c++) { const float4 v = *reinterpret_cast<const float4*>(p + 4 * c); r.v[4 * c] = v.x; r.v[4 * c + 1] = v.y; r.v[4 * c + 2] = v.z; r.v[4 * c + 3] = v.w; }
  }
  return r;
}
template <int K, int NT, bool FULL>
__device__ __noinline__ void rs_solve_team(const Env& C, const int l, const unsigned wmask_rt, const RsLayout L) {
  const unsigned wmask = FULL ? 0xffffffffu : wmask_rt;
  const DevScene& sc = SC;
  const int tbase = (threadIdx.x & 31) & ~(NT - 1), cap = sc.rs_cap;
  float* REC = WSG(C, sc.X_RSREC); const float* Al = WSG(C, sc.X_RSA) + l * K; float* capp = WSH(C, sc.W_CAPP);
  float rhs[K], dinv[K], lo[K], hi[K], ap[K], y[K], mu[K]; int par[K];
#pragma unroll
  for (int k = 0; k < K; k++) {
    rhs[k] = 0.f; dinv[k] = 0.f; lo[k] = 0.f; hi[k] = 0.f; ap[k] = 0.f; y[k] = 0.f; mu[k] = 0.f; par[k] = -1;
    const int p = l * K + k;
    if (p < L.Rp) { const F4 r0 = ld4(REC + RR_W * p), r1 = ld4(REC + RR_W * p + 4); rhs[k] = r0.x; dinv[k] = r0.y; lo[k] = r0.z; hi[k] = r0.w; mu[k] = r1.x; par[k] = float_as_int(r1.y); }
  }
  const int nb1 = L.P1 / K, nb2 = (L.P2 - L.P1) / K, nb3 = (L.Rp - L.P2) / K, plast = L.Rp > 0 ? L.Rp - 1 : 0;
  const int nb1m = __reduce_max_sync(wmask, nb1), nb2m = __reduce_max_sync(wmask, nb2), nb3m = __reduce_max_sync(wmask, nb3);
  float bprev = 0.f; int pprev = 0;
#define DG_RS_STEP(jt_, act_, k, HAND, NORMAL)                                                                   \
  {                                                                                                              \
    const int jc_ = (jt_) < NT ? (jt_) : NT - 1;                                                                 \
    const int p_ = min(jc_ * K + (k), plast);                                                                    \
    const bool own_ = (act_) && l == (jt_);                                                                      \
    if (HAND) {                                                                                                  \
      const RsRow<K> h_ = rs_ldrow<K>(Al + pprev * cap);                                                         \
      _Pragma("unroll") for (int kk = 0; kk < K; kk++) y[kk] = fmaf(h_.v[kk], bprev, y[kk]);                     \
      bprev = 0.f;                                                                                               \
    }                                                                                                            \
    const RsRow<K> a_ = rs_ldrow<K>(Al + (own_ ? p_ : pprev) * cap);                                             \
    const float new_ = fminf(fmaxf(ap[k] + fmaf(-y[k], dinv[k], rhs[k]), lo[k]), hi[k]);                         \
    const float dl_ = own_ ? new_ - ap[k] : 0.f;                                                                 \
    if (own_) { ap[k] = new_; if ((NORMAL) && p_ >= L.nrm0 && p_ < L.nrm1) capp[p_ - L.nrm0] = new_; }           \
    const float b_ = __shfl_sync(wmask, dl_, tbase + jc_);                                                       \
    const float cf_ = own_ ? dl_ : bprev;                                                                        \
    _Pragma("unroll") for (int kk = 0; kk < K; kk++) y[kk] = fmaf(a_.v[kk], cf_, y[kk]);                         \
    bprev = own_ ? 0.f : b_; pprev = p_;                                                                         \
  }
#define DG_RS_BLOCK_FWD(jt_, act_, NORMAL)                                                                       \
  { _Pragma("unroll") for (int k = 0; k < K; k++) { if (k == 0) DG_RS_STEP(jt_, act_, k, true, NORMAL) else DG_RS_STEP(jt_, act_, k, false, NORMAL) } }
#define DG_RS_BLOCK_REV(jt_, act_)                                                                               \
  { _Pragma("unroll") for (int k = K - 1; k >= 0; k--) { if (k == K - 1) DG_RS_STEP(jt_, act_, k, true, false) else DG_RS_STEP(jt_, act_, k, false, false) } }
  for (int it = 0; it < sc.iters; it++) {
    if (it & 1) { for (int jj = 0; jj < nb1m; jj++) DG_RS_BLOCK_FWD(jj, jj < nb1, false) }
    else { for (int jj = nb1m - 1; jj >= 0; jj--) DG_RS_BLOCK_REV(jj, jj < nb1) }
    for (int jj = 0; jj < nb2m; jj++) DG_RS_BLOCK_FWD(nb1 + jj, jj < nb2, true)
    __syncwarp(wmask);
#pragma unroll
    for (int k = 0; k < K; k++) if (par[k] >= 0) { hi[k] = mu[k] * capp[par[k]]; lo[k] = -hi[k]; }
    for (int jj = 0; jj < nb3m; jj++) DG_RS_BLOCK_FWD(nb1 + nb2 + jj, jj < nb3, false)
  }
#undef DG_RS_BLOCK_FWD
#undef DG_RS_BLOCK_REV
#undef DG_RS_STEP
#pragma unroll
  for (int k = 0; k < K; k++) { const int p = l * K + k; if (p < L.Rp) REC[RR_W * p + RR_APPLIED] = ap[k]; }
}
template <int NT>
__device__ __forceinline__ void rs_solve_block(const Env& C) {
  if constexpr (NT >= 2) {
  const DevScene& sc = SC;
  const int E = blockDim.x / NT, ei = threadIdx.x % E, e2 = threadIdx.x / NT, l2 = threadIdx.x % NT;
  Env C2 = C;
  C2.ws = C.ws + (long)(e2 - ei) * sc.w_total; C2.wg = C.wg + (long)(e2 - ei) * sc.g_total;
  const unsigned in_warp = blockDim.x - (threadIdx.x & ~31u);
  const unsigned wmask = in_warp >= 32u ? 0xffffffffu : (1u << in_warp) - 1u;
  const int* hdr = WSI(C2) + sc.W_HDR;
  const int R = hdr[WH_RS_DEFER] ? 0 : hdr[WH_RS_R];
  const RsLayout L = R > 0 ? rs_layout(hdr[WH_RS_K], hdr[WH_RS_NU], 6 * sc.ncons, hdr[WH_NCROW] / 3) : rs_layout(2, 0, 0, 0);
  const int Kw = __reduce_max_sync(wmask, R > 0 ? L.K : 0);
  if (Kw > 0) {
    if ((blockDim.x & 31u) == 0u) {
      if (Kw <= 2) rs_solve_team<2, NT, true>(C2, l2, wmask, L);
      else if (Kw <= 4) rs_solve_team<4, NT, true>(C2, l2, wmask, L);
      else rs_solve_team<RS_KMAX, NT, true>(C2, l2, wmask, L);
    } else {
      if (Kw <= 4) rs_solve_team<4, NT, false>(C2, l2, wmask, L);
      else rs_solve_team<RS_KMAX, NT, false>(C2, l2, wmask, L);
    }
  }
  }
}
#elif defined(__CUDA_ARCH__)
template <int NT> __device__ __forceinline__ void rs_solve_block(const Env&) {}
#else
DG_FN void rs_solve_serial(const Env& C, int nt) {
  (void)nt;
  const DevScene& sc = SC;
  const RsLayout L = rs_layout_of(C); const int cap = sc.rs_cap;
  float* REC = WSG(C, sc.X_RSREC); const float* A = WSG(C, sc.X_RSA); float* capp = WSH(C, sc.W_CAPP);
  float lo[RS_KMAX * 32], hi[RS_KMAX * 32], ap[RS_KMAX * 32], y[RS_KMAX * 32];
  for (int p = 0; p < L.Rp; p++) { lo[p] = REC[RR_W * p + RR_LO]; hi[p] = REC[RR_W * p + RR_HI]; ap[p] = 0.f; y[p] = 0.f; }
  auto update = [&](int p, bool normal) {
    const float* rc = REC + RR_W * p;
    const float nw = fminf(fmaxf(ap[p] + fmaf(-y[p], rc[RR_DINV], rc[RR_RHS]), lo[p]), hi[p]), d = nw - ap[p];
    ap[p] = nw;
    if (normal && p >= L.nrm0 && p < L.nrm1) capp[p - L.nrm0] = nw;
    for (int s2 = 0; s2 < L.Rp; s2++) y[s2] = fmaf(A[p * cap + s2], d, y[s2]);
  };
  for (int it = 0; it < sc.iters; it++) {
    if (it & 1) for (int p = 0; p < L.P1; p++) update(p, false); else for (int p = L.P1 - 1; p >= 0; p--) update(p, false);
    for (int p = L.P1; p < L.P2; p++) update(p, true);
    for (int p = L.P2; p < L.fr1; p++) { hi[p] = REC[RR_W * p + RR_MU] * capp[float_as_int(REC[RR_W * p + RR_PAR])]; lo[p] = -hi[p]; }
    for (int p = L.P2; p < L.Rp; p++) update(p, false);
  }
  for (int p = 0; p < L.Rp; p++) REC[RR_W * p + RR_APPLIED] = ap[p];
}
#endif

DG_FN void integrate_base_quat(float* q, const float* om, float h) {
  float ang = v_len(om), ax[3];
  if (ang * h > 0.25f * kPi) ang = 0.25f * kPi / h;
  if (ang < 0.001f) v_scale(ax, om, 0.5f * h - h * h * h * 0.020833333333f * ang * ang); else v_scale(ax, om, sinf(0.5f * ang * h) / ang);
  float dq[4] = {ax[0], ax[1], ax[2], cosf(0.5f * ang * h)}, out[4];
  q_mul(out, dq, q); q_norm(out); q[0] = out[0]; q[1] = out[1]; q[2] = out[2]; q[3] = out[3];
}
DG_FN void phase_integrate(const Env& C, int ln, int nt, float h) {
  const DevScene& sc = SC;
  for (int di = ln; di < sc.ndyn; di += nt) {
    int b = gc(sc.dyn_body)[di]; const int* bi = gc(sc.body_i) + DG_BODY_I_W * b; const int* bp = gc(sc.body_plan) + BP_W * b;
    const float* dv = WSH(C, sc.W_DV) + bp[BP_GVOFF]; int jo = 0;
    int n = WSI(C)[sc.W_UCNT + di]; const float* rows = WSH(C, sc.X_UROW) + UR_W * bp[BP_UROW];
    for (int j = 0; j < n; j++) { int md = float_as_int(rows[UR_W * j + UR_MOTOR]); if (md >= 0) DOF(D_APPLIED, md) = rows[UR_W * j + UR_APPLIED]; }
    if (bi[0] == 2) {
      float* bs = BST(di);
      for (int i = 0; i < 3; i++) { bs[10 + i] += dv[i]; bs[7 + i] += dv[3 + i]; }
      for (int i = 0; i < 3; i++) bs[i] += h * bs[7 + i];
      integrate_base_quat(bs + 3, bs + 10, h);
      jo = 6;
    }
    for (int i = 0; i < bi[4]; i++) {
      int d = bi[3] + i; float qd = DOF(D_QD, d) + dv[jo + i];
      qd = clampf(qd, -sc.max_joint_vel, sc.max_joint_vel);
      DOF(D_QD, d) = qd; DOF(D_Q, d) += h * qd;
      if ((sc.sem & SEM_WRENCH_FIRST_SUBSTEP) && WSI(C)[sc.W_HDR + WH_SUB] == 0) DOF(D_TAU, d) -= ST(S_JTORQUE)[d];
    }
  }
}
DG_FN void phase_next_substep(const Env& C, int ln, int nt) { (void)nt; if (ln == 0) WSI(C)[SC.W_HDR + WH_SUB] += 1; }
DG_FN void phase_final_kin(const Env& C, int ln, int nt) {
  for (int di = ln; di < SC.ndyn; di += nt) fk_vel_body<false>(C, gc(SC.dyn_body)[di]);
}
DG_FN void phase_store(const Env& C, int ln, int nt, int clear_forces) {
  const DevScene& sc = SC;
  for (int i = ln; i < 13 * sc.ndyn; i += nt) {
    int di = i / 13, k = i - 13 * di, b = gc(sc.dyn_body)[di]; float v = BST(di)[k];
    if (k < 3) ST(S_BPOS)[3 * b + k] = v;
    else if (k < 7) ST(S_BQUAT)[4 * b + k - 3] = v;
    else if (k < 10) ST(S_BVEL)[3 * b + k - 7] = v;
    else ST(S_BOMEGA)[3 * b + k - 10] = v;
  }
  for (int d = ln; d < sc.nd; d += nt) {
    ST(S_Q)[d] = DOF(D_Q, d); ST(S_QD)[d] = DOF(D_QD, d); ST(S_MAPPLIED)[d] = DOF(D_APPLIED, d);
    if (clear_forces) ST(S_JTORQUE)[d] = 0.f;
  }
  for (int gl = ln; gl < sc.nl; gl += nt) {
    int s = gc(sc.frame_slot)[sc.nb + gl];
    if (s < 0) continue;
    const float* K = KIN(s); float q[4], t[3];
    v_cpy(ST(S_LPOS) + 3 * gl, K + 9);
    mat_to_q(q, K); for (int i = 0; i < 4; i++) ST(S_LQUAT)[4 * gl + i] = q[i];
    const float* V = ABA(s) + AB_WV;
    m_vec(t, K, V + 3); v_cpy(ST(S_LVEL) + 3 * gl, t);
    m_vec(t, K, V); v_cpy(ST(S_LOMEGA) + 3 * gl, t);
  }
  if (clear_forces) for (int f = ln; f < sc.nframes; f += nt) {
    if (gc(sc.frame_slot)[f] < 0) continue;
    for (int i = 0; i < 3; i++) { ST(S_EXTF)[3 * f + i] = 0.f; ST(S_EXTT)[3 * f + i] = 0.f; }
  }
}

DG_FN void frame_com_state(const Env& C, int f, float* pos, float* quat, float* vel, float* om) {
  const DevScene& sc = SC;
  if (f < sc.nb) { v_cpy(pos, ST(S_BPOS) + 3 * f); for (int i = 0; i < 4; i++) quat[i] = ST(S_BQUAT)[4 * f + i]; v_cpy(vel, ST(S_BVEL) + 3 * f); v_cpy(om, ST(S_BOMEGA) + 3 * f); }
  else { int gl = f - sc.nb; v_cpy(pos, ST(S_LPOS) + 3 * gl); for (int i = 0; i < 4; i++) quat[i] = ST(S_LQUAT)[4 * gl + i]; v_cpy(vel, ST(S_LVEL) + 3 * gl); v_cpy(om, ST(S_LOMEGA) + 3 * gl); }
}
DG_FN void frame_link_pose(const Env& C, int f, float* pos, float* quat) {
  float v[3], o[3];
  frame_com_state(C, f, pos, quat, v, o);
  if (f >= SC.nb) {
    const float* lf = C.link_f + DG_LINK_F_W * (f - SC.nb);
    float R[9], t[3], qi[4] = {-lf[16], -lf[17], -lf[18], lf[19]}, qo[4];
    q_to_mat(R, quat); m_vec(t, R, lf + 7); v_sub(pos, pos, t);
    q_mul(qo, quat, qi); for (int i = 0; i < 4; i++) quat[i] = qo[i];
  }
}

DG_FN int solve_dense(float* A, float* bvec, int n) {
  for (int c = 0; c < n; c++) {
    int p = c;
    for (int r2 = c + 1; r2 < n; r2++) if (fabsf(A[r2 * n + c]) > fabsf(A[p * n + c])) p = r2;
    if (fabsf(A[p * n + c]) < 1e-30f) return -1;
    if (p != c) { for (int j = 0; j < n; j++) { float t = A[c * n + j]; A[c * n + j] = A[p * n + j]; A[p * n + j] = t; } float t = bvec[c]; bvec[c] = bvec[p]; bvec[p] = t; }
    for (int r2 = c + 1; r2 < n; r2++) { float f = A[r2 * n + c] / A[c * n + c]; if (f != 0.f) { for (int j = c; j < n; j++) A[r2 * n + j] -= f * A[c * n + j]; bvec[r2] -= f * bvec[c]; } }
  }
  for (int r2 = n - 1; r2 >= 0; r2--) { float s = bvec[r2]; for (int j = r2 + 1; j < n; j++) s -= A[r2 * n + j] * bvec[j]; bvec[r2] = s / A[r2 * n + r2]; }
  return 0;
}
DG_FN void ik_solve(const Env& C, int b, int ee_gl, const float* tpos_w, const float* torn_w, int use_orn, int nullspace,
                    const float* lower, const float* upper, const float* range, const float* rest, float* scr) {
  const DevScene& sc = SC;
  const int* bi = gc(sc.body_i) + DG_BODY_I_W * b; int d0 = bi[3], ndb = bi[4];
  int mc = sc.max_depth + 2;
  float* qb = scr; float* nullv = qb + ndb; float* dth = nullv + ndb; float* J = dth + ndb;
  float* A = J + 6 * ndb; int asz = ndb * ndb > 36 ? ndb * ndb : 36;
  float* rhs = A + asz; float* axw = rhs + (ndb > 6 ? ndb : 6); float* orgw = axw + 3 * mc;
  int* chain = (int*)(orgw + 3 * mc);
  for (int i = 0; i < ndb; i++) qb[i] = ST(S_Q)[d0 + i];
  const float *bp = ST(S_BPOS) + 3 * b, *bq = ST(S_BQUAT) + 4 * b;
  float Rb[9], tp[3], d[3], tq[4] = {0, 0, 0, 1};
  q_to_mat(Rb, bq); v_sub(d, tpos_w, bp); mT_vec(tp, Rb, d);
  if (use_orn) { float bqi[4] = {-bq[0], -bq[1], -bq[2], bq[3]}; q_mul(tq, bqi, torn_w); }
  if (nullspace) for (int i = 0; i < ndb; i++) {
    float nv = 0.001f * (rest[i] - qb[i]);
    if (qb[i] > upper[i]) nv += 10.0f * (upper[i] - qb[i]) / range[i];
    if (qb[i] < lower[i]) nv += 10.0f * (lower[i] - qb[i]) / range[i];
    nullv[i] = nv;
  }
  int nc = 0;
  for (int gl = ee_gl; gl >= 0; gl = shc(C.link_i)[DG_LINK_I_W * gl + 1]) chain[nc++] = gl;
  int m = use_orn ? 6 : 3;
  float diff = 1e30f;
  for (int it = 0; it < sc.ik_iters && diff > sc.ik_threshold; it++) {
    float Rc[9] = {1, 0, 0, 0, 1, 0, 0, 0, 1}, pc[3] = {0, 0, 0};
    for (int i = nc - 1; i >= 0; i--) {
      int gl = chain[i]; const int* li = shc(C.link_i) + DG_LINK_I_W * gl; const float* lf = shc(C.link_f) + DG_LINK_F_W * gl;
      float E[9], r[3], t[3], Rn[9];
      joint_xform(C, gl, li[3] >= 0 ? qb[li[3] - d0] : 0.0f, E, r);
      m_vec(t, Rc, r); v_add(pc, pc, t); m_mulT(Rn, Rc, E); m_cpy(Rc, Rn);
      m_vec(axw + 3 * i, Rc, lf + 10);
      float dw[3]; m_vec(dw, Rc, lf + 7); v_sub(orgw + 3 * i, pc, dw);
    }
    const float* lfe = shc(C.link_f) + DG_LINK_F_W * ee_gl;
    float pos[3], R[9], dw[3], Rli[9], qi[4] = {-lfe[16], -lfe[17], -lfe[18], lfe[19]};
    m_vec(dw, Rc, lfe + 7); v_sub(pos, pc, dw);
    q_to_mat(Rli, qi); m_mul(R, Rc, Rli);
    for (int i = 0; i < 6 * ndb; i++) J[i] = 0.f;
    for (int i = 0; i < nc; i++) {
      const int* li = shc(C.link_i) + DG_LINK_I_W * chain[i];
      if (li[3] < 0) continue;
      int jd = li[3] - d0;
      if (li[2] == 1) { float rel[3], t[3]; v_sub(rel, pos, orgw + 3 * i); v_cross(t, axw + 3 * i, rel); for (int k = 0; k < 3; k++) { J[k * ndb + jd] = t[k]; J[(3 + k) * ndb + jd] = axw[3 * i + k]; } }
      else if (li[2] == 2) for (int k = 0; k < 3; k++) J[k * ndb + jd] = axw[3 * i + k];
    }
    float e[6];
    v_sub(e, tp, pos); diff = v_len(e);
    if (use_orn) {
      float qc[4], qci[4], dq[4]; mat_to_q(qc, R); qci[0] = -qc[0]; qci[1] = -qc[1]; qci[2] = -qc[2]; qci[3] = qc[3];
      q_mul(dq, tq, qci);
      float vn = v_len(dq), ax[3];
      float ang = 2 * atan2f(vn, dq[3]);
      if (vn * vn < 10 * 2.220446049250313e-16f) v_set(ax, 1, 0, 0); else v_scale(ax, dq, 1.0f / vn);
      if (ang > kPi) ang -= 2 * kPi; else if (ang < -kPi) ang += 2 * kPi;
      v_scale(e + 3, ax, ang);
    }
    if (!nullspace) {
      for (int i = 0; i < ndb; i++) {
        for (int j = 0; j < ndb; j++) { float s = 0.f; for (int k = 0; k < m; k++) s += J[k * ndb + i] * J[k * ndb + j]; A[i * ndb + j] = s + (i == j ? sc.ik_damping : 0.f); }
        float s = 0.f; for (int k = 0; k < m; k++) s += J[k * ndb + i] * e[k]; rhs[i] = s;
      }
      if (solve_dense(A, rhs, ndb) != 0) break;
      for (int i = 0; i < ndb; i++) dth[i] = rhs[i];
    } else {
      for (int i = 0; i < m; i++) { float s = 0.f; for (int k = 0; k < ndb; k++) s += J[i * ndb + k] * nullv[k]; rhs[i] = e[i] - s; }
      for (int i = 0; i < m; i++) for (int j = 0; j < m; j++) { float s = 0.f; for (int k = 0; k < ndb; k++) s += J[i * ndb + k] * J[j * ndb + k]; A[i * m + j] = s + (i == j ? sc.ik_null_lambda_sq : 0.f); }
      if (solve_dense(A, rhs, m) != 0) break;
      for (int k = 0; k < ndb; k++) { float s = nullv[k]; for (int i = 0; i < m; i++) s += J[i * ndb + k] * rhs[i]; dth[k] = s; }
    }
    float mx = 0.f; for (int i = 0; i < ndb; i++) mx = fmaxf(mx, fabsf(dth[i]));
    float cap = 45.0f * kPi / 180.0f;
    if (mx > cap) for (int i = 0; i < ndb; i++) dth[i] *= cap / mx;
    for (int i = 0; i < ndb; i++) qb[i] += dth[i];
  }
}

template <int MAXD, int M>
DG_FN void ik_solve_fast(const Env& C, int b, int ee_gl, const float* tpos_w, const float* torn_w, int nullspace,
                         const float* lower, const float* upper, const float* range, const float* rest, float* scr) {
  const DevScene& sc = SC;
  const int* bi = gc(sc.body_i) + DG_BODY_I_W * b; const int d0 = bi[3], ndb = bi[4];
  const int mc = sc.max_depth + 2;
  float* qb = scr; float* axw = scr + MAXD; float* orgw = axw + 3 * mc;
  int* chain = (int*)(orgw + 3 * mc); int* cpos = chain + mc;
  float nullv[MAXD];
#pragma unroll
  for (int k = 0; k < MAXD; k++) { nullv[k] = 0.f; if (k < ndb) { qb[k] = ST(S_Q)[d0 + k]; cpos[k] = -1; } }
  const float *bp = ST(S_BPOS) + 3 * b, *bq = ST(S_BQUAT) + 4 * b;
  float Rb[9], tp[3], d[3], tq[4] = {0, 0, 0, 1};
  q_to_mat(Rb, bq); v_sub(d, tpos_w, bp); mT_vec(tp, Rb, d);
  if (M == 6) { float bqi[4] = {-bq[0], -bq[1], -bq[2], bq[3]}; q_mul(tq, bqi, torn_w); }
  if (nullspace) {
#pragma unroll
    for (int k = 0; k < MAXD; k++) if (k < ndb) {
      float q = qb[k], nv = 0.001f * (rest[k] - q);
      if (q > upper[k]) nv += 10.0f * (upper[k] - q) / range[k];
      if (q < lower[k]) nv += 10.0f * (lower[k] - q) / range[k];
      nullv[k] = nv;
    }
  }
  int nc = 0;
  for (int gl = ee_gl; gl >= 0; gl = shc(C.link_i)[DG_LINK_I_W * gl + 1]) { int dof = shc(C.link_i)[DG_LINK_I_W * gl + 3]; if (dof >= 0) cpos[dof - d0] = nc; chain[nc++] = gl; }
  const float lam = nullspace ? sc.ik_null_lambda_sq : sc.ik_damping;
  const float* lfe = shc(C.link_f) + DG_LINK_F_W * ee_gl;
  float Rli[9]; { float qi[4] = {-lfe[16], -lfe[17], -lfe[18], lfe[19]}; q_to_mat(Rli, qi); }
  float diff = 1e30f;
  for (int it = 0; it < sc.ik_iters && diff > sc.ik_threshold; it++) {
    float Rc[9] = {1, 0, 0, 0, 1, 0, 0, 0, 1}, pc[3] = {0, 0, 0};
    for (int i = nc - 1; i >= 0; i--) {
      int gl = chain[i]; const int* li = shc(C.link_i) + DG_LINK_I_W * gl; const float* lf = shc(C.link_f) + DG_LINK_F_W * gl;
      float E[9], r[3], t[3], Rn[9];
      joint_xform(C, gl, li[3] >= 0 ? qb[li[3] - d0] : 0.0f, E, r);
      m_vec(t, Rc, r); v_add(pc, pc, t); m_mulT(Rn, Rc, E); m_cpy(Rc, Rn);
      if (li[3] >= 0) { m_vec(axw + 3 * i, Rc, lf + 10); float dw[3]; m_vec(dw, Rc, lf + 7); v_sub(orgw + 3 * i, pc, dw); }
    }
    float pos[3], dw[3];
    m_vec(dw, Rc, lfe + 7); v_sub(pos, pc, dw);
    float J[M][MAXD];
#pragma unroll
    for (int k = 0; k < MAXD; k++) {
#pragma unroll
      for (int r = 0; r < M; r++) J[r][k] = 0.f;
      if (k < ndb && cpos[k] >= 0) {
        int i = cpos[k]; const float* ax = axw + 3 * i;
        if (shc(C.link_i)[DG_LINK_I_W * chain[i] + 2] == 1) {
          float rel[3], t[3]; v_sub(rel, pos, orgw + 3 * i); v_cross(t, ax, rel);
          J[0][k] = t[0]; J[1][k] = t[1]; J[2][k] = t[2];
          if (M == 6) { J[M - 3][k] = ax[0]; J[M - 2][k] = ax[1]; J[M - 1][k] = ax[2]; }
        } else { J[0][k] = ax[0]; J[1][k] = ax[1]; J[2][k] = ax[2]; }
      }
    }
    float e[M];
    { float e3[3]; v_sub(e3, tp, pos); diff = v_len(e3); e[0] = e3[0]; e[1] = e3[1]; e[2] = e3[2]; }
    if (M == 6) {
      float R[9], qc[4], qci[4], dq[4]; m_mul(R, Rc, Rli); mat_to_q(qc, R); qci[0] = -qc[0]; qci[1] = -qc[1]; qci[2] = -qc[2]; qci[3] = qc[3];
      q_mul(dq, tq, qci);
      float vn = v_len(dq), ax[3];
      float ang = 2 * atan2f(vn, dq[3]);
      if (vn * vn < 10 * 2.220446049250313e-16f) v_set(ax, 1, 0, 0); else v_scale(ax, dq, 1.0f / vn);
      if (ang > kPi) ang -= 2 * kPi; else if (ang < -kPi) ang += 2 * kPi;
      e[M - 3] = ax[0] * ang; e[M - 2] = ax[1] * ang; e[M - 1] = ax[2] * ang;
    }
    float x[M], U[M][M];
#pragma unroll
    for (int r = 0; r < M; r++) {
      float sdot = 0.f;
#pragma unroll
      for (int k = 0; k < MAXD; k++) sdot = fmaf(J[r][k], nullv[k], sdot);
      x[r] = e[r] - sdot;
#pragma unroll
      for (int c = 0; c <= r; c++) {
        float u = 0.f;
#pragma unroll
        for (int k = 0; k < MAXD; k++) u = fmaf(J[r][k], J[c][k], u);
        U[r][c] = u + (r == c ? lam : 0.f);
      }
    }
#pragma unroll
    for (int c = 0; c < M; c++) {
      float inv = 1.0f / U[c][c];
#pragma unroll
      for (int r = c + 1; r < M; r++) {
        float urc = U[r][c], f = urc * inv;
#pragma unroll
        for (int c2 = c + 1; c2 < r; c2++) U[r][c2] -= urc * U[c2][c];
        U[r][r] -= urc * f;
        x[r] -= f * x[c];
        U[r][c] = f;
      }
    }
#pragma unroll
    for (int r = M - 1; r >= 0; r--) {
      float sdot = x[r] / U[r][r];
#pragma unroll
      for (int r2 = r + 1; r2 < M; r2++) sdot -= U[r2][r] * x[r2];
      x[r] = sdot;
    }
    float dth[MAXD], mx = 0.f;
#pragma unroll
    for (int k = 0; k < MAXD; k++) {
      float sdot = nullv[k];
#pragma unroll
      for (int r = 0; r < M; r++) sdot = fmaf(J[r][k], x[r], sdot);
      dth[k] = sdot; mx = fmaxf(mx, fabsf(sdot));
    }
    const float cap = 45.0f * kPi / 180.0f;
    float sc_ = mx > cap ? cap / mx : 1.0f;
#pragma unroll
    for (int k = 0; k < MAXD; k++) if (k < ndb) qb[k] += dth[k] * sc_;
  }
}
DG_FN void ik_solve_any(const Env& C, int b, int ee_gl, const float* tpos_w, const float* torn_w, int use_orn, int nullspace,
                        const float* lower, const float* upper, const float* range, const float* rest, float* scr) {
  const int ndb = gc(SC.body_i)[DG_BODY_I_W * b + 4];
  if (ndb <= 6) { if (use_orn) ik_solve_fast<6, 6>(C, b, ee_gl, tpos_w, torn_w, nullspace, lower, upper, range, rest, scr); else ik_solve_fast<6, 3>(C, b, ee_gl, tpos_w, torn_w, nullspace, lower, upper, range, rest, scr); }
  else if (ndb <= 12) { if (use_orn) ik_solve_fast<12, 6>(C, b, ee_gl, tpos_w, torn_w, nullspace, lower, upper, range, rest, scr); else ik_solve_fast<12, 3>(C, b, ee_gl, tpos_w, torn_w, nullspace, lower, upper, range, rest, scr); }
  else ik_solve(C, b, ee_gl, tpos_w, torn_w, use_orn, nullspace, lower, upper, range, rest, scr);
}

DG_FN void admittance_update(const Env& C, const int* ia, const float* fa, const float* a);
DG_FN void phase_actions(const Env& C, int ln, int nt) {
  const DevScene& sc = SC;
  int ik_seen = 0;
  for (int k = 0; k < sc.nop; k++) {
    const int* op = gc(sc.op_i) + DG_OP_I_W * k; const int* ia = gc(sc.oparg_i) + op[1]; const float* fa = gc(sc.oparg_f) + op[2];
    const float* a = op[3] >= 0 ? C.act + op[3] : nullptr;
    if (k < 128 && !((C.opmask[k >> 6] >> (k & 63)) & 1ull)) { if (op[0] == OP_IK_CTRL) ik_seen++; continue; }
    if (op[0] == OP_JOINT_CTRL && ln == 0) {
      int mode = ia[0], n = ia[1];
      for (int i = 0; i < n; i++) {
        int d = ia[2 + i];
        if (mode == 2) { ST(S_JTORQUE)[d] += a[i]; continue; }
        ST(S_MKD)[d] = fa[1]; ST(S_MMAXF)[d] = fa[2 + i];
        if (mode == 0) { ST(S_MKP)[d] = fa[0]; ST(S_MTPOS)[d] = a[i]; ST(S_MTVEL)[d] = 0.f; }
        else { ST(S_MKP)[d] = 0.f; ST(S_MTPOS)[d] = 0.f; ST(S_MTVEL)[d] = a[i]; }
      }
    } else if (op[0] == OP_EXT_FORCE && ln == 0) {
      int f = ia[0]; float pos[3], quat[4], v[3], o[3], F[3], rel[3], t[3];
      frame_com_state(C, f, pos, quat, v, o);
      if (ia[1] == 0) { v_cpy(F, a); v_sub(rel, fa, pos); }
      else { float R[9]; q_to_mat(R, quat); m_vec(F, R, a); m_vec(rel, R, fa); }
      v_add(ST(S_EXTF) + 3 * f, ST(S_EXTF) + 3 * f, F); v_cross(t, rel, F); v_add(ST(S_EXTT) + 3 * f, ST(S_EXTT) + 3 * f, t);
    } else if (op[0] == OP_FILTERED_WRENCH && ln == 0) {
      float* st_ = ST(S_ADDON) + ia[2]; const float s_ = st_[0] + (a[0] - st_[0]) * fa[0];
      st_[0] = s_;
      const int f = ia[0]; float pos[3], quat[4], v[3], o[3], R[9], F[3], T[3], rel[3], t[3];
      frame_com_state(C, f, pos, quat, v, o); q_to_mat(R, quat);
      const float Fl[3] = {fa[1] * s_, fa[2] * s_, fa[3] * s_}, Tl[3] = {fa[4] * s_, fa[5] * s_, fa[6] * s_};
      m_vec(F, R, Fl); m_vec(T, R, Tl); m_vec(rel, R, fa + 7);
      v_add(ST(S_EXTF) + 3 * f, ST(S_EXTF) + 3 * f, F); v_cross(t, rel, F); v_add(t, t, T); v_add(ST(S_EXTT) + 3 * f, ST(S_EXTT) + 3 * f, t);
    } else if (op[0] == OP_ADMITTANCE && ln == 0) {
      admittance_update(C, ia, fa, a);
    } else if (op[0] == OP_IK_CTRL) {
      int mine = (ik_seen++ % nt) == ln;
      if (!mine) continue;
      int b = ia[0], ee = ia[1], n = ia[2], use_orn = ia[3], nsp = ia[4]; int ndb = gc(sc.body_i)[DG_BODY_I_W * b + 4];
      float pos[3], quat[4], v[3], o[3], tq[4] = {0, 0, 0, 1};
      frame_com_state(C, sc.nb + ee, pos, quat, v, o);
      float tpos[3] = {pos[0] + a[0], pos[1] + a[1], pos[2] + a[2]};
      if (use_orn) { float dq[4]; q_from_euler(dq, a + 3); q_mul(tq, quat, dq); }
      const float* lim = fa + 2 + n;
      float* scr = WSG(C, sc.X_IK) + sc.ik_stride * (ln % (sc.n_ik < nt ? sc.n_ik : nt));
      ik_solve_any(C, b, ee, tpos, tq, use_orn, nsp, lim, lim + ndb, lim + 2 * ndb, lim + 3 * ndb, scr);
      for (int i = 0; i < n; i++) {
        int d = ia[5 + i];
        ST(S_MKP)[d] = fa[0]; ST(S_MKD)[d] = fa[1]; ST(S_MMAXF)[d] = fa[2 + i]; ST(S_MTPOS)[d] = scr[i]; ST(S_MTVEL)[d] = 0.f;
      }
    }
  }
  if (ln == 0) ST(S_STEP)[0] += 1.f;
}
DG_FN void joint_axis_world(const Env& C, int gl, float* aw, float* ow) {
  const float* lf = shc(C.link_f) + DG_LINK_F_W * gl;
  float R[9], dw[3];
  q_to_mat(R, ST(S_LQUAT) + 4 * gl); m_vec(aw, R, lf + 10); m_vec(dw, R, lf + 7); v_sub(ow, ST(S_LPOS) + 3 * gl, dw);
}
DG_FN void admittance_update(const Env& C, const int* ia, const float* fa, const float* a) {
  const DevScene& sc = SC;
  const int b = ia[0], ee = ia[1], n = ia[2]; const int* bi = gc(sc.body_i) + DG_BODY_I_W * b; const int l0 = bi[1], nlb = bi[2];
  const float kp = fa[0], kd = fa[1]; const float* target = fa + 5;
  for (int i = 0; i < n; i++) { const int d = ia[3 + i]; ST(S_JTORQUE)[d] += (target[i] - ST(S_Q)[d]) * kp - kd * ST(S_QD)[d]; }
  float Re[9], P[3], t[3];
  q_to_mat(Re, ST(S_LQUAT) + 4 * ee); m_vec(t, Re, fa + 2); v_add(P, ST(S_LPOS) + 3 * ee, t);
  for (int gl = ee; gl >= 0; gl = shc(C.link_i)[DG_LINK_I_W * gl + 1]) {
    const int* li = shc(C.link_i) + DG_LINK_I_W * gl;
    if (li[3] < 0) continue;
    float aw[3], ow[3], rel[3], c[3];
    joint_axis_world(C, gl, aw, ow);
    if (li[2] == 1) { v_sub(rel, P, ow); v_cross(c, aw, rel); ST(S_JTORQUE)[li[3]] += v_dot(a, c) + v_dot(a + 3, aw); }
    else ST(S_JTORQUE)[li[3]] += v_dot(a, aw);
  }
  for (int k = 0; k < nlb; k++) {
    const float m = PR(P_MASS)[sc.nb + l0 + k];
    if (m == 0.f) continue;
    const float* pk = ST(S_LPOS) + 3 * (l0 + k);
    for (int gl = l0 + k; gl >= 0; gl = shc(C.link_i)[DG_LINK_I_W * gl + 1]) {
      const int* li = shc(C.link_i) + DG_LINK_I_W * gl;
      if (li[3] < 0) continue;
      float aw[3], ow[3], rel[3], c[3];
      joint_axis_world(C, gl, aw, ow);
      if (li[2] == 1) { v_sub(rel, pk, ow); v_cross(c, aw, rel); } else v_cpy(c, aw);
      ST(S_JTORQUE)[li[3]] -= m * v_dot(sc.g, c);
    }
  }
}
DG_FN void phase_observe(const Env& C, int ln, int nt) {
  const DevScene& sc = SC;
  for (int k = ln; k < sc.nop; k += nt) {
    const int* op = gc(sc.op_i) + DG_OP_I_W * k; const int* ia = gc(sc.oparg_i) + op[1]; const float* fa = gc(sc.oparg_f) + op[2];
    float* o = op[4] >= 0 ? C.obs + op[4] : nullptr;
    if (op[0] == OP_JOINT_SENSOR) {
      int n = ia[0], flags = ia[1], j = 0;
      for (int i = 0; i < n; i++) o[j++] = ST(S_Q)[ia[2 + i]];
      if (flags & 1) for (int i = 0; i < n; i++) o[j++] = ST(S_QD)[ia[2 + i]];
      if (flags & 2) for (int i = 0; i < n; i++) o[j++] = ST(S_MAPPLIED)[ia[2 + i]] / sc.dt;
    } else if (op[0] == OP_OBJECT_SENSOR) {
      float p[3], q[4], v[3], w[3]; int flags = ia[2], j = 0;
      frame_com_state(C, ia[0], p, q, v, w);
      if (ia[1] >= 0) {
        float sp[3], sq[4], sv[3], sw[3], qq[4];
        frame_com_state(C, ia[1], sp, sq, sv, sw);
        v_sub(p, p, sp); v_sub(v, v, sv); q_mul(qq, sq, q); for (int i = 0; i < 4; i++) q[i] = qq[i]; v_sub(w, w, sw);
      }
      for (int i = 0; i < 3; i++) o[j++] = p[i];
      if (flags & 2) for (int i = 0; i < 3; i++) o[j++] = v[i];
      if (flags & 1) { float e[3]; euler_from_q(e, q); for (int i = 0; i < 3; i++) o[j++] = e[i]; }
      if ((flags & 3) == 3) for (int i = 0; i < 3; i++) o[j++] = w[i];
    } else if (op[0] == OP_FT_SENSOR) {
      for (int i = 0; i < 6; i++) o[i] = ST(S_JREACT)[6 * ia[0] + i];
    } else if (op[0] == OP_REACH_TARGET) {
      float sp[3], sq[4], tp[3], tq[4], d[3];
      frame_link_pose(C, ia[0], sp, sq); frame_link_pose(C, ia[1], tp, tq); v_sub(d, tp, sp);
      float dist = v_len(d);
      C.rew[op[5]] = -dist * fa[0]; C.term[op[6]] = dist < fa[1];
    } else if (op[0] == OP_ELECTRICITY) {
      const int* bi = gc(sc.body_i) + DG_BODY_I_W * ia[0]; float s = 0.f;
      for (int i = 0; i < bi[4]; i++) s += fabsf(ST(S_MAPPLIED)[bi[3] + i] / sc.dt * ST(S_QD)[bi[3] + i]);
      C.rew[op[5]] = -s * fa[0];
    } else if (op[0] == OP_STUCK_JOINT) {
      const int* bi = gc(sc.body_i) + DG_BODY_I_W * ia[0]; int stuck = 0;
      for (int l = 0; l < bi[2]; l++) {
        const int* li = shc(C.link_i) + DG_LINK_I_W * (bi[1] + l); const float* lf = shc(C.link_f) + DG_LINK_F_W * (bi[1] + l);
        if (li[3] < 0) continue;
        float qq = ST(S_Q)[li[3]];
        if (fminf(fabsf(lf[20] - qq), fabsf(lf[21] - qq)) < 0.01f) stuck = 1;
      }
      C.rew[op[5]] = stuck ? -fa[0] : 0.0f;
    } else if (op[0] == OP_TIME_PENALTY) {
      C.rew[op[5]] = fa[0];
    } else if (op[0] == OP_FILTERED_WRENCH) {
      o[0] = ST(S_ADDON)[ia[2]];
    } else if (op[0] == OP_TILT_TERMINAL) {
      const float* q = ST(S_BQUAT) + 4 * ia[0];
      C.term[op[6]] = 2.0f * atan2f(sqrtf(q[0] * q[0] + q[1] * q[1] + q[2] * q[2]), fabsf(q[3])) > fa[0];
    } else if (op[0] == OP_EPISODE_TIMER) {
      C.term[op[6]] = ST(S_STEP)[0] >= fa[0];
    }
  }
}
DG_FN void phase_reset_ops(const Env& C, int ln, int nt) {
  if (ln != 0) return;
  const DevScene& sc = SC;
  ST(S_STEP)[0] = 0.f;
  uint32_t epoch = (uint32_t)ST(S_RESETS)[0];
  for (int k = 0; k < sc.nop; k++) {
    const int* op = gc(sc.op_i) + DG_OP_I_W * k; const int* ia = gc(sc.oparg_i) + op[1]; const float* fa = gc(sc.oparg_f) + op[2];
    if (op[0] == OP_FILTERED_WRENCH) {
      if (ia[1]) ST(S_ADDON)[ia[2]] = 0.f;
    } else if (op[0] == OP_JOINT_RESET) {
      for (int i = 0; i < ia[0]; i++) { ST(S_Q)[ia[1 + i]] = fa[i]; ST(S_QD)[ia[1 + i]] = 0.f; }
    } else if (op[0] == OP_RESPAWN) {
      int b = ia[0]; uint32_t ep = ia[1] ? 0u : epoch; const float* ip = PR(P_INITPOSE) + 7 * b;
      float e[3], dq[4], qo[4];
      for (int i = 0; i < 3; i++) ST(S_BPOS)[3 * b + i] = ip[i] + (urand(C.seed, (uint32_t)C.env_id, ep, (uint32_t)(k * 8 + i)) - 0.5f) * fa[i];
      for (int i = 0; i < 3; i++) e[i] = (urand(C.seed, (uint32_t)C.env_id, ep, (uint32_t)(k * 8 + 3 + i)) - 0.5f) * fa[3 + i];
      q_from_euler(dq, e); q_mul(qo, ip + 3, dq); for (int i = 0; i < 4; i++) ST(S_BQUAT)[4 * b + i] = qo[i];
      v_set(ST(S_BVEL) + 3 * b, 0, 0, 0); v_set(ST(S_BOMEGA) + 3 * b, 0, 0, 0);
    } else if (op[0] == OP_VIS_RANDOMIZE) {
      for (int v = 0; v < sc.nv; v++) if (gc(sc.vis_i)[DG_VIS_I_W * v + 3] == ia[0])
        for (int i = 0; i < 3; i++) PR(P_COLOR)[3 * v + i] = urand(C.seed, (uint32_t)C.env_id, epoch, (uint32_t)(k * 8 + 128 + 3 * v + i));
    } else if (op[0] == OP_DYN_RANDOMIZE) {
      int b = ia[0]; const int* bi = gc(sc.body_i) + DG_BODY_I_W * b;
      for (int l = -1; l < bi[2]; l++) {
        int f = l < 0 ? b : sc.nb + bi[1] + l; int d = l < 0 ? -1 : shc(C.link_i)[DG_LINK_I_W * (bi[1] + l) + 3];
        if (l >= 0 && d < 0) continue;
        if (l < 0 && bi[4] > 0) continue;
        float u1 = urand(C.seed, (uint32_t)C.env_id, epoch, (uint32_t)(k * 8 + 64 + 2 * (l + 1)));
        float u2 = urand(C.seed, (uint32_t)C.env_id, epoch, (uint32_t)(k * 8 + 65 + 2 * (l + 1)));
        float ms = expf(logf(fa[0]) + u1 * (logf(fa[1]) - logf(fa[0]))), ds = expf(logf(fa[2]) + u2 * (logf(fa[3]) - logf(fa[2])));
        PR(P_MASS)[f] = gc(sc.param_def)[DG_PO(C.sc, P_MASS) + f] * ms;
        for (int i = 0; i < 3; i++) PR(P_INERTIA)[3 * f + i] = gc(sc.param_def)[DG_PO(C.sc, P_INERTIA) + 3 * f + i] * ms;
        if (d >= 0) { const float nom = gc(sc.param_def)[DG_PO(C.sc, P_JDAMP) + d]; PR(P_JDAMP)[d] = (nom > 0.f ? nom : fa[6]) * ds; }
      }
      if (fa[5] > 0.f) {
        const float u3 = urand(C.seed, (uint32_t)C.env_id, epoch, (uint32_t)(k * 8 + 63));
        const float fr = fa[4] + u3 * (fa[5] - fa[4]);
        for (int s2 = 0; s2 < sc.ns; s2++) if (gc(sc.shape_i)[DG_SHAPE_I_W * s2] == b) PR(P_FRICTION)[s2] = fr;
      }
    }
  }
  ST(S_RESETS)[0] += 1.f;
}

#if defined(__CUDA_ARCH__)
#define DG_PHASE(call) do { const long long t0_ = C.dbg ? clock64() : 0; if (C.active) { call; } if (nt > 1) __syncthreads(); \
                            if (C.dbg && threadIdx.x == 0) C.dbg[(size_t)blockIdx.x * 64 + (__LINE__ & 63)] += (unsigned long long)(clock64() - t0_); } while (0)
#define DG_LANE_ARGS int ln
DG_HD bool block_any(bool p, int nt) { return nt > 1 ? (__syncthreads_or(p ? 1 : 0) != 0) : p; }
#else
#define DG_PHASE(call) do { for (int ln = 0; ln < nt; ln++) { call; } } while (0)
#define DG_LANE_ARGS int
DG_HD bool block_any(bool p, int) { return p; }
#endif
#define HDRV(k) (C.active ? WSI(C)[SC.W_HDR + (k)] : 0)

DG_NOINLINE DG_FN void physics_pre(const Env& C, int nt, float h, DG_LANE_ARGS) {
  const DevScene& sc = SC;
  DG_PHASE(phase_dynamics(C, ln, nt, h));
  DG_PHASE(phase_shape_world(C, ln, nt));
  if (sc.npair > 0) {
    DG_PHASE(phase_broad(C, ln, nt));
    DG_PHASE(phase_count_survivors(C, ln, nt));
    for (int rnd = 0; block_any(rnd * nt < HDRV(WH_NSURV), nt); rnd++) {
      DG_PHASE(phase_narrow(C, ln, nt, rnd));
      DG_PHASE(phase_append(C, ln, nt));
    }
  }
  DG_PHASE(phase_minv(C, ln, nt));
  DG_PHASE(phase_unit_rows(C, ln, nt, h));
  if (sc.ncons == 0 && !block_any(HDRV(WH_NCROW) > 0, nt)) {
    DG_PHASE(phase_pgs_unit(C, ln, nt, 0, sc.iters));
  } else {
    DG_PHASE(phase_contact_rows(C, ln, nt, h));
#if defined(__CUDA_ARCH__)
    if (!C.active && ln == 0) { WSI(C)[sc.W_HDR + WH_RS_R] = 0; WSI(C)[sc.W_HDR + WH_RS_NEED] = 0; WSI(C)[sc.W_HDR + WH_RS_DEFER] = 0; }
#endif
    DG_PHASE(phase_rs_plan(C, ln, nt));
    DG_PHASE(phase_rs_setup(C, ln, nt));
    DG_PHASE(if (HDRV(WH_RS_R) > 0) { if (HDRV(WH_RS_DEFER) == 0) phase_rs_build(C, ln, nt); }
             else if (HDRV(WH_COUPLED) == 0) { if (HDRV(WH_NCROW) > 0) phase_pgs_full(C, ln, nt); else phase_pgs_unit(C, ln, nt, 0, sc.iters); });
    if (sc.solver == 1 && nt > 1 && block_any(HDRV(WH_RS_R) > 0 && HDRV(WH_RS_DEFER) == 0, nt)) {
#if defined(__CUDA_ARCH__)
      const long long t0_ = C.dbg ? clock64() : 0;
#if defined(DG_STEP_T)
      rs_solve_block<DG_STEP_T>(C);
#endif
      __syncthreads();
      if (C.dbg && threadIdx.x == 0) C.dbg[(size_t)blockIdx.x * 64 + (__LINE__ & 63)] += (unsigned long long)(clock64() - t0_);
#else
      DG_PHASE(if (ln == 0 && HDRV(WH_RS_R) > 0) rs_solve_serial(C, nt));
#endif
      DG_PHASE(if (HDRV(WH_RS_R) > 0 && HDRV(WH_RS_DEFER) == 0) phase_rs_finish(C, ln, nt));
    }
    if (block_any(HDRV(WH_COUPLED) != 0 && HDRV(WH_RS_R) == 0, nt)) {
      for (int it = 0; it < sc.iters; it++) {
        DG_PHASE(if (HDRV(WH_COUPLED) != 0 && HDRV(WH_RS_R) == 0) phase_pgs_unit(C, ln, nt, it, it + 1));
        DG_PHASE(if (HDRV(WH_COUPLED) != 0 && HDRV(WH_RS_R) == 0) phase_pgs_contact(C, ln, nt));
      }
    }
  }
}
DG_NOINLINE DG_FN void physics_post(const Env& C, int nt, float h, DG_LANE_ARGS) {
  DG_PHASE(phase_integrate(C, ln, nt, h));
  if (SC.sem & SEM_WRENCH_FIRST_SUBSTEP) DG_PHASE(phase_next_substep(C, ln, nt));
}
DG_NOINLINE DG_FN void run_physics(const Env& C, int nt, int nsub, int clear_forces, DG_LANE_ARGS) {
  const DevScene& sc = SC;
  float h = sc.dt / (float)sc.substeps;
  DG_PHASE(phase_load(C, ln, nt));
  for (int sub = 0; sub < nsub; sub++) {
#if defined(__CUDA_ARCH__)
    physics_pre(C, nt, h, ln); physics_post(C, nt, h, ln);
#else
    physics_pre(C, nt, h, 0); physics_post(C, nt, h, 0);
#endif
  }
  DG_PHASE(phase_final_kin(C, ln, nt));
  DG_PHASE(phase_store(C, ln, nt, clear_forces));
}
#if defined(__CUDA_ARCH__)
DG_FN void run_env_step_stages(const Env& C, int nt, int stages, int ln) {
  const DevScene& sc = SC;
  const float h = sc.dt / (float)sc.substeps;
  if (stages & ST_ACT) { DG_PHASE(phase_actions(C, ln, nt)); DG_PHASE(phase_load(C, ln, nt)); }
  if (stages & ST_LOAD) { DG_PHASE(phase_load(C, ln, nt)); }
  if (stages & ST_POST) physics_post(C, nt, h, ln);
  if (stages & ST_PRE) physics_pre(C, nt, h, ln);
  if (stages & ST_END) { DG_PHASE(phase_final_kin(C, ln, nt)); DG_PHASE(phase_store(C, ln, nt, 1)); DG_PHASE(phase_observe(C, ln, nt)); }
}
#endif

DG_FN void run_env_step(const Env& C, int nt, DG_LANE_ARGS) {
#if defined(__CUDA_ARCH__)
  DG_PHASE(phase_actions(C, ln, nt));
  run_physics(C, nt, SC.substeps, 1, ln);
  DG_PHASE(phase_observe(C, ln, nt));
#else
  DG_PHASE(phase_actions(C, ln, nt));
  run_physics(C, nt, SC.substeps, 1, 0);
  DG_PHASE(phase_observe(C, ln, nt));
#endif
}
DG_FN void run_env_observe(const Env& C, int nt, DG_LANE_ARGS) {
#if defined(__CUDA_ARCH__)
  run_physics(C, nt, 0, 0, ln);
#else
  run_physics(C, nt, 0, 0, 0);
#endif
  DG_PHASE(phase_observe(C, ln, nt));
}
DG_FN void run_env_reset(const Env& C, int nt, DG_LANE_ARGS) {
#if defined(__CUDA_ARCH__)
  DG_PHASE(phase_reset_ops(C, ln, nt));
  run_physics(C, nt, 0, 0, ln);
  for (int i = 0; i < (C.no_hot ? 0 : SC.hot_start); i++) run_physics(C, nt, SC.substeps, 1, ln);
  DG_PHASE(phase_observe(C, ln, nt));
#else
  DG_PHASE(phase_reset_ops(C, ln, nt));
  run_physics(C, nt, 0, 0, 0);
  for (int i = 0; i < SC.hot_start; i++) run_physics(C, nt, SC.substeps, 1, 0);
  DG_PHASE(phase_observe(C, ln, nt));
#endif
}

}
```

diy_gym_b200/csrc/dg_scene.h:

```cpp
#pragma once
#include <stdint.h>

#include "scene_sections.h"

namespace dg {

enum { D_Q = 0, D_QD, D_APPLIED, D_TAU, D_COUNT };
enum { BP_DI = 0, BP_GDIM, BP_GVOFF, BP_MINVOFF, BP_I0OFF, BP_SLOT, BP_UROW, BP_DEPTH, BP_NRS, BP_AOFF, BP_GS, BP_W };
enum { WH_NCONTACT = 0, WH_NCROW, WH_NSURV, WH_COUPLED, WH_RS_R, WH_RS_NU, WH_RS_K, WH_RS_NEED, WH_RS_DEFER, WH_SUB, WH_COUNT = 12 };
enum { ST_ACT = 1, ST_PRE = 2, ST_POST = 4, ST_END = 8, ST_LOADC = 16, ST_SAVEC = 32, ST_LOAD = 128, ST_ALL = 15 };
enum { RS_NCLS = 3 };
enum { DG_MINV_MAXL = 64, DG_MINV_MAXD = 24 };
enum { RS_CONTACT = 0x40000000, RS_KMAX = 8, RS_GVMAX = 128 };
enum { RR_RHS = 0, RR_DINV, RR_LO, RR_HI, RR_MU, RR_PAR, RR_APPLIED, RR_ID, RR_W = 8 };
enum { UR_RHS = 0, UR_DINV, UR_LO, UR_HI, UR_APPLIED, UR_COL, UR_MOTOR, UR_W = 8 };
enum { CR_RHS = 0, CR_DINV, CR_LO, CR_HI, CR_APPLIED, CR_MU, CR_DA, CR_DB, CR_PARENT, CR_HDR = 12 };
enum { LK_W = 20, AB_PA = 0, AB_WV = 6, AB_A = 12, AB_B = 21, AB_C = 30, AB_ACC = 40, AB_W = 48, LX_W = 8 };
enum { CT_FA = 0, CT_FB, CT_PA = 2, CT_PB = 5, CT_N = 8, CT_DIST = 11, CT_MU = 12, CT_W = 13 };

struct DevScene {
  int nb, nl, nd, ns, nv, npair, ncam, nop, nframes, S, P, substeps, iters, maxc, hot_start, ik_iters;
  int n_act, n_obs, n_rew, n_term;
  int so[24];
  int po[12];
  float dt, g[3], erp, cerp, slop, margin, ik_damping, ik_threshold, max_joint_vel, limit_max_impulse, ik_null_lambda_sq;
  const int *body_i, *link_i, *shape_i, *pair_i, *vis_i, *op_i, *oparg_i, *cam_i;
  const float *body_f, *link_f, *shape_f, *vis_f, *oparg_f, *cam_f, *param_def, *state_def;
  const float* hull_f;
  int ndyn, nslot, nshw, nfloat, GD, GP, max_depth, max_nlb, n_ik, team;
  const int* dyn_body;
  const int* body_plan;
  const int* frame_slot;
  const int* link_depth;
  const int* shape_slot;
  const float* shape_wb;
  const float* vis_wb;
  const float* link_x;
  int ngrp, nloose;
  const int* grp_i;
  const int* grp_pairs;
  const int* loose_pairs;
  const float* body_reach;
  int w_total, g_total, ws_mode;
  int W_HDR, W_BST, W_DOF, W_EXT, W_KIN, W_LINK, W_MINV, W_DV, W_I0, W_UCNT, W_CAPP, W_X;
  int X_ABA, X_LNK, X_I0T;
  int X_SHW, X_CON, X_SURV, X_CTMP, X_UROW, X_CROW, X_MSCR, X_AMAT, X_IK, X_RSA, X_RSAS, X_RSV, X_RSREC;
  int GV;
  int rs_ashared;
  int rs_cap;
  int ncons;
  const int* cons_i; const float* cons_f;
  int need_react;
  int rs_min;
  int rs_cls_k[RS_NCLS], rs_cls_r[RS_NCLS];
  int solver;
  int crow_stride, mscr_stride, ctmp_stride, ik_stride;
  int sem;
  int precise;
};

#define DG_SO(sc, name) ((sc)->so[HI_##name - HI_S_BPOS])
#define DG_PO(sc, name) ((sc)->po[HI_##name - HI_P_MASS])

}

#ifndef __CUDACC_RTC__
#include <algorithm>
#include <cmath>
#include <string>
#include <vector>

namespace dg {

struct HostScene {
  std::vector<int> ints;
  std::vector<float> floats;
  DevScene dev;
  std::string error;

  struct Off { size_t body_i, link_i, shape_i, pair_i, vis_i, op_i, oparg_i, cam_i, dyn_body, body_plan, frame_slot, link_depth, shape_slot, grp_i, grp_pairs, loose_pairs;
               size_t body_f, link_f, shape_f, vis_f, oparg_f, cam_f, param_def, state_def, shape_wb, vis_wb, link_x, body_reach, cons_i, cons_f, hull_f; } off;

  static void quat_to_mat(const double* q, double* m) {
    double x = q[0], y = q[1], z = q[2], w = q[3];
    double n = 1.0 / std::sqrt(x * x + y * y + z * z + w * w); x *= n; y *= n; z *= n; w *= n;
    m[0] = 1 - 2 * (y * y + z * z); m[1] = 2 * (x * y - z * w); m[2] = 2 * (x * z + y * w);
    m[3] = 2 * (x * y + z * w); m[4] = 1 - 2 * (x * x + z * z); m[5] = 2 * (y * z - x * w);
    m[6] = 2 * (x * z - y * w); m[7] = 2 * (y * z + x * w); m[8] = 1 - 2 * (x * x + y * y);
  }

  void point(DevScene& d, const int* ib, const float* fb) const {
    d.body_i = ib + off.body_i; d.link_i = ib + off.link_i; d.shape_i = ib + off.shape_i; d.pair_i = ib + off.pair_i;
    d.vis_i = ib + off.vis_i; d.op_i = ib + off.op_i; d.oparg_i = ib + off.oparg_i; d.cam_i = ib + off.cam_i;
    d.dyn_body = ib + off.dyn_body; d.body_plan = ib + off.body_plan; d.frame_slot = ib + off.frame_slot;
    d.link_depth = ib + off.link_depth; d.shape_slot = ib + off.shape_slot;
    d.grp_i = ib + off.grp_i; d.grp_pairs = ib + off.grp_pairs; d.loose_pairs = ib + off.loose_pairs; d.body_reach = fb + off.body_reach;
    d.body_f = fb + off.body_f; d.link_f = fb + off.link_f; d.shape_f = fb + off.shape_f; d.vis_f = fb + off.vis_f;
    d.oparg_f = fb + off.oparg_f; d.cam_f = fb + off.cam_f; d.param_def = fb + off.param_def; d.state_def = fb + off.state_def;
    d.shape_wb = fb + off.shape_wb; d.vis_wb = fb + off.vis_wb; d.link_x = fb + off.link_x;
    d.cons_i = ib + off.cons_i; d.cons_f = fb + off.cons_f; d.hull_f = fb + off.hull_f;
  }

  bool build(const int32_t* ibuf, int ni, const double* fbuf, int nf, int team, int ws_mode = 0, int rs_ashared = 0) {
    if (ni < 2 + 3 * DG_NSECTIONS || ibuf[0] != (int32_t)DG_SCENE_MAGIC || ibuf[1] != DG_NSECTIONS) { error = "bad scene magic / section count"; return false; }
    auto sec_off = [&](int s) { return (size_t)ibuf[2 + 3 * s + 1]; };
    auto sec_len = [&](int s) { return (size_t)ibuf[2 + 3 * s + 2]; };
    for (int s = 0; s < DG_NSECTIONS; s++) {
      bool is_f = ibuf[2 + 3 * s] != 0;
      if (sec_off(s) + sec_len(s) > (size_t)(is_f ? nf : ni)) { error = "section out of range"; return false; }
    }
    const int32_t* hi = ibuf + sec_off(SEC_HDR_I);
    const double* hf = fbuf + sec_off(SEC_HDR_F);
    DevScene& d = dev;
    d = DevScene();
    d.nb = hi[HI_nb]; d.nl = hi[HI_nl]; d.nd = hi[HI_nd]; d.ns = hi[HI_ns]; d.nv = hi[HI_nv]; d.npair = hi[HI_npair];
    d.ncam = hi[HI_ncam]; d.nop = hi[HI_nop]; d.nframes = hi[HI_nframes]; d.S = hi[HI_S]; d.P = hi[HI_P];
    d.substeps = hi[HI_substeps]; d.iters = hi[HI_iterations]; d.maxc = hi[HI_max_contacts]; d.hot_start = hi[HI_hot_start];
    d.ik_iters = hi[HI_ik_iters]; d.n_act = hi[HI_n_act]; d.n_obs = hi[HI_n_obs]; d.n_rew = hi[HI_n_rew]; d.n_term = hi[HI_n_term];
    for (int k = HI_S_BPOS; k <= HI_S_ADDON; k++) d.so[k - HI_S_BPOS] = hi[k];
    for (int k = HI_P_MASS; k <= HI_P_COLOR; k++) d.po[k - HI_P_MASS] = hi[k];
    d.dt = (float)hf[HF_dt]; d.g[0] = (float)hf[HF_gx]; d.g[1] = (float)hf[HF_gy]; d.g[2] = (float)hf[HF_gz];
    d.erp = (float)hf[HF_erp]; d.cerp = (float)hf[HF_contact_erp]; d.slop = (float)hf[HF_linear_slop]; d.margin = (float)hf[HF_contact_margin];
    d.ik_damping = (float)hf[HF_ik_damping]; d.ik_threshold = (float)hf[HF_ik_threshold]; d.max_joint_vel = (float)hf[HF_max_joint_vel];
    d.limit_max_impulse = (float)hf[HF_limit_max_impulse]; d.ik_null_lambda_sq = (float)hf[HF_ik_null_lambda_sq];
    d.team = team;

    ints.clear(); floats.clear();
    auto put_i = [&](int s) { size_t o = ints.size(); ints.insert(ints.end(), ibuf + sec_off(s), ibuf + sec_off(s) + sec_len(s)); ints.push_back(0); return o; };
    auto put_f = [&](int s) { size_t o = floats.size(); const double* p = fbuf + sec_off(s); for (size_t i = 0; i < sec_len(s); i++) floats.push_back((float)p[i]); floats.push_back(0.f); return o; };
    off.body_i = put_i(SEC_BODY_I); off.link_i = put_i(SEC_LINK_I); off.shape_i = put_i(SEC_SHAPE_I); off.pair_i = put_i(SEC_PAIR_I);
    off.vis_i = put_i(SEC_VIS_I); off.op_i = put_i(SEC_OP_I); off.oparg_i = put_i(SEC_OPARG_I); off.cam_i = put_i(SEC_CAM_I);
    off.body_f = put_f(SEC_BODY_F); off.link_f = put_f(SEC_LINK_F); off.shape_f = put_f(SEC_SHAPE_F); off.vis_f = put_f(SEC_VIS_F);
    off.oparg_f = put_f(SEC_OPARG_F); off.cam_f = put_f(SEC_CAM_F); off.param_def = put_f(SEC_PARAM_DEFAULT); off.state_def = put_f(SEC_STATE_DEFAULT);
    off.cons_i = put_i(SEC_CONS_I); off.cons_f = put_f(SEC_CONS_F); off.hull_f = put_f(SEC_HULL_F);
    d.ncons = hi[HI_ncons];

    const int32_t* body_i = ibuf + sec_off(SEC_BODY_I);
    const int32_t* link_i = ibuf + sec_off(SEC_LINK_I);
    const int32_t* shape_i = ibuf + sec_off(SEC_SHAPE_I);
    const double* shape_f = fbuf + sec_off(SEC_SHAPE_F);
    const int32_t* vis_i = ibuf + sec_off(SEC_VIS_I);
    const double* vis_f = fbuf + sec_off(SEC_VIS_F);
    const int32_t* pair_i = ibuf + sec_off(SEC_PAIR_I);
    const int32_t* op_i = ibuf + sec_off(SEC_OP_I);

    std::vector<int> dyn_body, body_plan((size_t)d.nb * BP_W, 0), frame_slot(d.nframes, -1), link_depth(std::max(d.nl, 1), 0), shape_slot(std::max(d.ns, 1), -1);
    int nslot = 0, gv = 0, minv = 0, i0 = 0, nfloat = 0, GD = 1, max_depth = 0, max_nlb = 0, amat = 0;
    for (int b = 0; b < d.nb; b++) {
      const int32_t* bi = body_i + DG_BODY_I_W * b; int* bp = &body_plan[(size_t)b * BP_W];
      int kind = bi[0], l0 = bi[1], nlb = bi[2], ndb = bi[4], baked = bi[7];
      bp[BP_DI] = -1; bp[BP_SLOT] = -1; bp[BP_I0OFF] = -1; bp[BP_UROW] = 2 * bi[3];
      if (kind != 0) {
        bp[BP_DI] = (int)dyn_body.size(); dyn_body.push_back(b);
        int gdim = (kind == 2 ? 6 : 0) + ndb;
        int gs = (gdim + 3) & ~3;
        bp[BP_GDIM] = gdim; bp[BP_GS] = gs; bp[BP_GVOFF] = gv; bp[BP_MINVOFF] = minv; gv += gs; minv += gdim * gs; GD = std::max(GD, gdim);
        if (kind == 2) { bp[BP_I0OFF] = 36 * nfloat; nfloat++; i0 += 36; }
        int nrs = std::min(2 * ndb, ((ndb + 2 + 3) / 4) * 4); nrs = std::min(((nrs + 3) / 4) * 4, 16);
        bp[BP_NRS] = ndb > 0 ? nrs : 0; bp[BP_AOFF] = amat; amat += bp[BP_NRS] * bp[BP_NRS];
        max_nlb = std::max(max_nlb, nlb);
      }
      if (kind != 0 || !baked) {
        bp[BP_SLOT] = nslot; frame_slot[b] = nslot++;
        for (int k = 0; k < nlb; k++) frame_slot[d.nb + l0 + k] = nslot++;
      }
      int depth_b = 0;
      for (int k = 0; k < nlb; k++) {
        int pl = link_i[DG_LINK_I_W * (l0 + k) + 1];
        link_depth[l0 + k] = pl < 0 ? 0 : link_depth[pl] + 1;
        depth_b = std::max(depth_b, link_depth[l0 + k]);
      }
      bp[BP_DEPTH] = depth_b; max_depth = std::max(max_depth, depth_b);
    }
    int nshw = 0;
    std::vector<float> shape_wb((size_t)std::max(d.ns, 1) * 12, 0.f), vis_wb((size_t)std::max(d.nv, 1) * 12, 0.f);
    for (int s = 0; s < d.ns; s++) {
      if (shape_i[DG_SHAPE_I_W * s + 3]) {
        double m[9]; quat_to_mat(shape_f + DG_SHAPE_F_W * s + 15, m);
        for (int i = 0; i < 9; i++) shape_wb[12 * s + i] = (float)m[i];
        for (int i = 0; i < 3; i++) shape_wb[12 * s + 9 + i] = (float)shape_f[DG_SHAPE_F_W * s + 12 + i];
      } else shape_slot[s] = nshw++;
    }
    for (int s = 0; s < d.nv; s++) if (vis_i[DG_VIS_I_W * s + 2]) {
      double m[9]; quat_to_mat(vis_f + DG_VIS_F_W * s + 19, m);
      for (int i = 0; i < 9; i++) vis_wb[12 * s + i] = (float)m[i];
      for (int i = 0; i < 3; i++) vis_wb[12 * s + 9 + i] = (float)vis_f[DG_VIS_F_W * s + 16 + i];
    }
    std::vector<float> link_x((size_t)std::max(d.nl, 1) * 16, 0.f);
    {
      const double* link_f = fbuf + sec_off(SEC_LINK_F);
      for (int gl = 0; gl < d.nl; gl++) {
        const double* lf = link_f + DG_LINK_F_W * gl; int jt = link_i[DG_LINK_I_W * gl + 2];
        double m[9]; quat_to_mat(lf, m);
        for (int i = 0; i < 9; i++) link_x[16 * gl + i] = (float)m[i];
        const double *a = lf + 10, *dd = lf + 7;
        if (jt == 1) {
          for (int i = 0; i < 3; i++) link_x[16 * gl + 9 + i] = (float)a[i];
          link_x[16 * gl + 12] = (float)(a[1] * dd[2] - a[2] * dd[1]); link_x[16 * gl + 13] = (float)(a[2] * dd[0] - a[0] * dd[2]);
          link_x[16 * gl + 14] = (float)(a[0] * dd[1] - a[1] * dd[0]);
        } else if (jt == 2) for (int i = 0; i < 3; i++) link_x[16 * gl + 12 + i] = (float)a[i];
      }
    }
    std::vector<float> body_reach(d.nb, 0.f);
    {
      const double* link_f = fbuf + sec_off(SEC_LINK_F);
      std::vector<double> lreach(std::max(d.nl, 1), 0.0);
      auto norm3 = [](const double* v) { return std::sqrt(v[0] * v[0] + v[1] * v[1] + v[2] * v[2]); };
      for (int gl = 0; gl < d.nl; gl++) {
        const double* lf = link_f + DG_LINK_F_W * gl; const int32_t* li = link_i + DG_LINK_I_W * gl;
        double travel = li[2] == 2 ? std::max(std::fabs(lf[20]), std::fabs(lf[21])) : 0.0;
        lreach[gl] = (li[1] < 0 ? 0.0 : lreach[li[1]]) + norm3(lf + 4) + norm3(lf + 7) + travel;
      }
      for (int s = 0; s < d.ns; s++) {
        int b = shape_i[DG_SHAPE_I_W * s], f = shape_i[DG_SHAPE_I_W * s + 1];
        double r = (f < d.nb ? 0.0 : lreach[f - d.nb]) + norm3(shape_f + DG_SHAPE_F_W * s) + shape_f[DG_SHAPE_F_W * s + 11];
        body_reach[b] = std::max(body_reach[b], (float)(r * 1.0001 + 1e-6));
      }
    }
    std::vector<int> grp_i, grp_pairs, loose_pairs;
    {
      std::vector<std::vector<int>> members;
      std::vector<long long> keys;
      for (int k = 0; k < d.npair; k++) {
        int sa = pair_i[2 * k], sb = pair_i[2 * k + 1];
        bool ba = shape_i[DG_SHAPE_I_W * sa + 3] != 0, bb = shape_i[DG_SHAPE_I_W * sb + 3] != 0;
        int stat = -1, dynb = -1;
        if (ba && !bb) { stat = sa; dynb = shape_i[DG_SHAPE_I_W * sb]; } else if (bb && !ba) { stat = sb; dynb = shape_i[DG_SHAPE_I_W * sa]; }
        if (stat < 0 || body_i[DG_BODY_I_W * dynb] == 0) { loose_pairs.push_back(k); continue; }
        long long key = (long long)stat * d.nb + dynb; size_t g = 0;
        for (; g < keys.size(); g++) if (keys[g] == key) break;
        if (g == keys.size()) { keys.push_back(key); members.emplace_back(); }
        members[g].push_back(k);
      }
      for (size_t g = 0; g < keys.size(); g++) {
        grp_i.push_back((int)(keys[g] / d.nb)); grp_i.push_back((int)(keys[g] % d.nb)); grp_i.push_back((int)grp_pairs.size()); grp_i.push_back((int)members[g].size());
        grp_pairs.insert(grp_pairs.end(), members[g].begin(), members[g].end());
      }
    }
    int GP = 1;
    auto gdim_of_shape = [&](int s) { int b = shape_i[DG_SHAPE_I_W * s]; return body_plan[(size_t)b * BP_W + BP_GDIM]; };
    for (int k = 0; k < d.npair; k++) GP = std::max(GP, gdim_of_shape(pair_i[2 * k]) + gdim_of_shape(pair_i[2 * k + 1]));
    int n_ik = 0;
    for (int k = 0; k < d.nop; k++) n_ik += op_i[DG_OP_I_W * k] == OP_IK_CTRL;
    d.need_react = hi[HI_S_STEP] > hi[HI_S_JREACT];
    d.precise = d.ncons > 0; d.sem = hi[HI_semantics];

    auto put_vi = [&](const std::vector<int>& v) { size_t o = ints.size(); ints.insert(ints.end(), v.begin(), v.end()); ints.push_back(0); return o; };
    auto put_vf = [&](const std::vector<float>& v) { size_t o = floats.size(); floats.insert(floats.end(), v.begin(), v.end()); floats.push_back(0.f); return o; };
    off.dyn_body = put_vi(dyn_body); off.body_plan = put_vi(body_plan); off.frame_slot = put_vi(frame_slot);
    off.link_depth = put_vi(link_depth); off.shape_slot = put_vi(shape_slot);
    off.shape_wb = put_vf(shape_wb); off.vis_wb = put_vf(vis_wb); off.link_x = put_vf(link_x); off.body_reach = put_vf(body_reach);
    off.grp_i = put_vi(grp_i); off.grp_pairs = put_vi(grp_pairs); off.loose_pairs = put_vi(loose_pairs);
    point(d, ints.data(), floats.data());

    d.ndyn = (int)dyn_body.size(); d.nslot = nslot; d.nshw = nshw; d.nfloat = nfloat; d.GD = GD; d.GP = GP;
    if (max_nlb > DG_MINV_MAXL || max_depth + 2 > DG_MINV_MAXD) { error = "a body has more than " + std::to_string((int)DG_MINV_MAXL) + " links or a kinematic tree deeper than " + std::to_string((int)DG_MINV_MAXD - 2); return false; }
    d.max_depth = max_depth; d.max_nlb = max_nlb; d.n_ik = n_ik; d.ngrp = (int)grp_i.size() / 4; d.nloose = (int)loose_pairs.size();

    enum { RC_SMALL = 0, RC_KIN, RC_ABA, RC_SOLVE, RC_CONTACT, RC_SCRATCH };
    auto is_cold = [&](int rc) {
      if (rc == RC_SMALL || rc == RC_SOLVE) return false;
      if (rc == RC_KIN || rc == RC_ABA || rc == RC_SCRATCH) return true;
      return ws_mode == 3;
    };
    int fix[2] = {0, 0};
    int ph[2][3] = {{0, 0, 0}, {0, 0, 0}};
    auto enc_rc = [&](int rc, int cold, int off) { return (rc == RC_CONTACT && cold) ? ~off : off; };
    auto take = [&](int rc, int n) { int c = is_cold(rc); int r = fix[c]; fix[c] += (n + 3) & ~3; return std::make_pair(c, r); };
    auto fixed = [&](int rc, int n) { auto pr = take(rc, n); return enc_rc(rc, pr.first, pr.second); };
    d.W_HDR = fixed(RC_SMALL, WH_COUNT);
    d.W_BST = fixed(RC_SMALL, 13 * d.ndyn);
    d.W_DOF = fixed(RC_SMALL, D_COUNT * d.nd);
    d.W_DV = fixed(RC_SMALL, gv);
    d.W_UCNT = fixed(RC_SMALL, d.ndyn);
    d.W_CAPP = fixed(RC_SMALL, 3 * d.maxc);
    d.W_MINV = fixed(RC_SOLVE, minv);
    d.W_KIN = fixed(RC_KIN, 12 * nslot);
    d.W_LINK = fixed(RC_KIN, LK_W * d.nl);
    d.W_I0 = fixed(RC_KIN, i0);
    d.W_EXT = 0; d.W_X = 0;
    struct Pending { int* field; int cold, phase, rel, rc; };
    std::vector<Pending> pend;
    auto phase_take = [&](int* field, int rc, int phase, int n) { int c = is_cold(rc); pend.push_back({field, c, phase, ph[c][phase], rc}); ph[c][phase] += (n + 3) & ~3; };
    d.crow_stride = 2 * (d.GP = GP = (GP + 3) & ~3) + CR_HDR;
    d.ctmp_stride = 1 + 4 * CT_W;
    d.mscr_stride = max_nlb + 6 * (max_depth + 2);
    int gj = 1;
    for (int b = 0; b < d.nb; b++) gj = std::max(gj, (int)body_i[DG_BODY_I_W * b + 4]);
    d.ik_stride = (9 * (max_depth + 2) + 6 * gj + std::max(gj * gj, 36) + 8 * gj + 32 + 3) & ~3;
    phase_take(&d.X_ABA, RC_ABA, 0, AB_W * nslot);
    phase_take(&d.X_LNK, RC_ABA, 0, LX_W * d.nl);
    phase_take(&d.X_I0T, RC_ABA, 0, 36 * nfloat);
    phase_take(&d.X_SHW, RC_CONTACT, 1, 12 * nshw);
    phase_take(&d.X_CON, RC_CONTACT, 1, CT_W * d.maxc);
    phase_take(&d.X_SURV, RC_CONTACT, 1, (d.npair + 31) / 32 + 1);
    phase_take(&d.X_UROW, RC_SOLVE, 1, UR_W * 2 * d.nd);
    phase_take(&d.X_AMAT, RC_SOLVE, 1, amat);
    phase_take(&d.X_CROW, RC_CONTACT, 1, d.crow_stride * 3 * d.maxc);
    phase_take(&d.X_CTMP, RC_SCRATCH, 1, d.ctmp_stride * team);
    phase_take(&d.X_MSCR, RC_SCRATCH, 1, d.mscr_stride * team);
    d.GV = gv;
    const int rows_max = 2 * d.nd + 3 * d.maxc + 6 * d.ncons;
    auto pad8 = [](int n) { return (n + RS_KMAX - 1) / RS_KMAX * RS_KMAX; };
    const int rows_pad = pad8(2 * d.nd) + pad8(d.maxc + 6 * d.ncons) + pad8(2 * d.maxc);
    d.rs_cap = (team > 1 && gv <= RS_GVMAX) ? std::min(rows_pad, RS_KMAX * team) : 0;
    if (d.ncons > 0 && d.rs_cap < rows_pad) {
      error = "scenes with fixed constraints between models are solved by the row-space team solver: " + std::to_string(rows_max) +
              " rows need a team of at least " + std::to_string((rows_pad + RS_KMAX - 1) / RS_KMAX) + " lanes (and at most " + std::to_string((int)RS_GVMAX) + " generalized coordinates)";
      return false;
    }
    d.rs_cls_k[0] = 2; d.rs_cls_r[0] = 32; d.rs_cls_k[1] = 0; d.rs_cls_r[1] = 0; d.rs_cls_k[2] = 2; d.rs_cls_r[2] = 64;
    d.solver = 1; d.rs_min = 0;
    d.rs_ashared = 0; d.X_RSAS = 0; (void)rs_ashared;
    phase_take(&d.X_RSA, RC_SCRATCH, 1, d.rs_cap * d.rs_cap + RS_KMAX * team);
    phase_take(&d.X_RSV, RC_SCRATCH, 1, d.rs_cap * 2 * gv);
    phase_take(&d.X_RSREC, RC_SCRATCH, 1, d.rs_cap * RR_W);
    phase_take(&d.X_IK, RC_SCRATCH, 2, n_ik ? d.ik_stride * std::min(team, n_ik) : 0);
    for (auto& pd : pend) *pd.field = enc_rc(pd.rc, pd.cold, fix[pd.cold] + pd.rel);
    d.w_total = fix[0] + std::max(ph[0][0], std::max(ph[0][1], ph[0][2]));
    d.g_total = fix[1] + std::max(ph[1][0], std::max(ph[1][1], ph[1][2]));
    d.ws_mode = ws_mode;
    return true;
  }
};

}
#endif
```

Baseline: 2.563 million.

## Parallelize articulated-body dynamics and mass-matrix inverse across tree levels

Adds a level-parallel path for forward kinematics, the articulated-body algorithm and the inverse-mass computation. Links at the same tree depth are distributed across team lanes per phase, where previously each lane walked a whole body serially. Host-side tree metadata (per-level link lists, child lists) and extra workspace for child contributions and per-column accelerations are built. It is enabled only when trees are wide enough (2*levels <= links) or when DG_TREE_LEVELS is set, and it adds more phase barriers and global-memory traffic.

```diff
diff --git a/diy_gym_b200/csrc/dg_env.cuh b/diy_gym_b200/csrc/dg_env.cuh
--- a/diy_gym_b200/csrc/dg_env.cuh
+++ b/diy_gym_b200/csrc/dg_env.cuh
@@ -123,70 +123,86 @@
 }
 
 template <bool BIAS>
+DG_HD void fk_link(const Env& C, int gl, const float* Kp, const float* Vp, float* K, float* V) {
+  const int* li = shc(C.link_i) + DG_LINK_I_W * gl; const float* lx = shc(C.link_x) + 16 * gl;
+  const int dof = li[3];
+  float E[9], r[3], t[3], t2[3], cacc[8] = {0, 0, 0, 0, 0, 0, 0, 0};
+  joint_xform(C, gl, dof >= 0 ? DOF(D_Q, dof) : 0.f, E, r);
+  float* L = LNK(gl);
+  st4(L, E[0], E[1], E[2], E[3]); st4(L + 4, E[4], E[5], E[6], E[7]); st4(L + 8, E[8], r[0], r[1], r[2]);
+  m_mulT(K, Kp, E);
+  m_vec(t, Kp, r); v_add(K + 9, Kp + 9, t);
+  m_vec(V, E, Vp);
+  v_cross(t, Vp, r); v_add(t2, Vp + 3, t); m_vec(V + 3, E, t2);
+  if (dof >= 0) {
+    const float qd = DOF(D_QD, dof);
+    if (BIAS) { float sa[3], sl[3]; v_scale(sa, lx + 9, qd); v_scale(sl, lx + 12, qd); v_cross(cacc, V, sa); v_cross(cacc + 3, V, sl); v_cross(t2, V + 3, sa); v_add(cacc + 3, cacc + 3, t2); }
+    v_madd(V, lx + 9, qd); v_madd(V + 3, lx + 12, qd);
+  }
+  if (BIAS) stn<8>(LNX(gl), cacc);
+}
+template <bool BIAS>
+DG_HD void frame_record(const Env& C, int b, int kind, int f, bool base, const float* K, const float* V, float* X) {
+  const DevScene& sc = SC;
+  if (!BIAS) {
+    for (int i = 0; i < 6; i++) X[AB_WV + i] = V[i];
+  } else if (base && kind != 2) {
+    float z[40]; for (int i = 0; i < 40; i++) z[i] = 0.f;
+    for (int i = 0; i < 6; i++) z[AB_WV + i] = V[i];
+    stn<40>(X, z);
+  } else {
+    const float *mass = PR(P_MASS), *inertia = PR(P_INERTIA);
+    const float kl = PR(P_LINDAMP)[b], ka = PR(P_ANGDAMP)[b];
+    const float wsc = ((sc.sem & SEM_WRENCH_FIRST_SUBSTEP) && WSI(C)[sc.W_HDR + WH_SUB] > 0) ? 0.f : 1.f;
+    const float efv[3] = {wsc * ST(S_EXTF)[3 * f], wsc * ST(S_EXTF)[3 * f + 1], wsc * ST(S_EXTF)[3 * f + 2]}, etv[3] = {wsc * ST(S_EXTT)[3 * f], wsc * ST(S_EXTT)[3 * f + 1], wsc * ST(S_EXTT)[3 * f + 2]};
+    const float *ef = efv, *et = etv;
+    const float m = mass[f]; const float* I = inertia + 3 * f; const float *w = V, *v = V + 3;
+    float Iw[3] = {I[0] * w[0], I[1] * w[1], I[2] * w[2]}, t[3], fw[3], pa[3], pl[3];
+    v_cross(pa, w, Iw);
+    v_cross(t, w, v); v_scale(pl, t, m);
+    fw[0] = sc.g[0] * m + ef[0]; fw[1] = sc.g[1] * m + ef[1]; fw[2] = sc.g[2] * m + ef[2];
+    mT_vec(t, K, fw); v_sub(pl, pl, t);
+    mT_vec(t, K, et); v_sub(pa, pa, t);
+    const float wn = v_len(w), vn = v_len(v);
+    const bool dlin = (sc.sem & SEM_DAMPING_LINEAR) != 0;
+    v_madd(pa, Iw, dlin ? ka : ka + ka * wn);
+    float mv[3]; v_scale(mv, v, m); v_madd(pl, mv, dlin ? kl : kl + kl * vn);
+    float z[40]; for (int i = 0; i < 40; i++) z[i] = 0.f;
+    for (int i = 0; i < 3; i++) { z[AB_PA + i] = pa[i]; z[AB_PA + 3 + i] = pl[i]; z[AB_WV + i] = w[i]; z[AB_WV + 3 + i] = v[i]; }
+    z[AB_A] = I[0]; z[AB_A + 4] = I[1]; z[AB_A + 8] = I[2]; z[AB_C] = m; z[AB_C + 4] = m; z[AB_C + 8] = m;
+    stn<40>(X, z);
+  }
+}
+DG_HD void base_frame(const Env& C, int b, float* K, float* V) {
+  const float* bs = BST(gc(SC.body_plan)[BP_W * b + BP_DI]);
+  q_to_mat(K, bs + 3); v_cpy(K + 9, bs);
+  mT_vec(V, K, bs + 10); mT_vec(V + 3, K, bs + 7);
+}
+
+template <bool BIAS>
 DG_FN void fk_vel_body(const Env& C, int b) {
   const DevScene& sc = SC;
   const int* bi = gc(sc.body_i) + DG_BODY_I_W * b; const int* bp = gc(sc.body_plan) + BP_W * b;
   const int kind = bi[0], l0 = bi[1], nlb = bi[2], s0 = bp[BP_SLOT];
   const float* bs = BST(bp[BP_DI]);
-  const float *mass = PR(P_MASS), *inertia = PR(P_INERTIA);
-  const float kl = PR(P_LINDAMP)[b], ka = PR(P_ANGDAMP)[b];
   float Kp[12], Vp[6];
   q_to_mat(Kp, bs + 3); v_cpy(Kp + 9, bs);
   mT_vec(Vp, Kp, bs + 10); mT_vec(Vp + 3, Kp, bs + 7);
   int prev = s0;
   for (int k = -1; k < nlb; k++) {
     const int s = s0 + 1 + k, f = k < 0 ? b : sc.nb + l0 + k;
-    float K[12], V[6], cacc[8] = {0, 0, 0, 0, 0, 0, 0, 0};
+    float K[12], V[6];
     if (k < 0) {
       for (int i = 0; i < 12; i++) K[i] = Kp[i];
       for (int i = 0; i < 6; i++) V[i] = Vp[i];
     } else {
-      const int gl = l0 + k; const int* li = shc(C.link_i) + DG_LINK_I_W * gl; const float* lx = shc(C.link_x) + 16 * gl;
-      const int ps = parent_slot(li, l0, s0), dof = li[3];
+      const int gl = l0 + k; const int* li = shc(C.link_i) + DG_LINK_I_W * gl;
+      const int ps = parent_slot(li, l0, s0);
       if (ps != prev) { ldn<12>(KIN(ps), Kp); const float* pv = ABA(ps) + AB_WV; for (int i = 0; i < 6; i++) Vp[i] = pv[i]; }
-      float E[9], r[3], t[3], t2[3];
-      joint_xform(C, gl, dof >= 0 ? DOF(D_Q, dof) : 0.f, E, r);
-      float* L = LNK(gl);
-      st4(L, E[0], E[1], E[2], E[3]); st4(L + 4, E[4], E[5], E[6], E[7]); st4(L + 8, E[8], r[0], r[1], r[2]);
-      m_mulT(K, Kp, E);
-      m_vec(t, Kp, r); v_add(K + 9, Kp + 9, t);
-      m_vec(V, E, Vp);
-      v_cross(t, Vp, r); v_add(t2, Vp + 3, t); m_vec(V + 3, E, t2);
-      if (dof >= 0) {
-        const float qd = DOF(D_QD, dof);
-        if (BIAS) { float sa[3], sl[3]; v_scale(sa, lx + 9, qd); v_scale(sl, lx + 12, qd); v_cross(cacc, V, sa); v_cross(cacc + 3, V, sl); v_cross(t2, V + 3, sa); v_add(cacc + 3, cacc + 3, t2); }
-        v_madd(V, lx + 9, qd); v_madd(V + 3, lx + 12, qd);
-      }
-      if (BIAS) stn<8>(LNX(gl), cacc);
+      fk_link<BIAS>(C, gl, Kp, Vp, K, V);
     }
     stn<12>(KIN(s), K);
-    float* X = ABA(s);
-    if (!BIAS) {
-      for (int i = 0; i < 6; i++) X[AB_WV + i] = V[i];
-    } else if (k < 0 && kind != 2) {
-      float z[40]; for (int i = 0; i < 40; i++) z[i] = 0.f;
-      for (int i = 0; i < 6; i++) z[AB_WV + i] = V[i];
-      stn<40>(X, z);
-    } else {
-      const float wsc = ((sc.sem & SEM_WRENCH_FIRST_SUBSTEP) && WSI(C)[sc.W_HDR + WH_SUB] > 0) ? 0.f : 1.f;
-      const float efv[3] = {wsc * ST(S_EXTF)[3 * f], wsc * ST(S_EXTF)[3 * f + 1], wsc * ST(S_EXTF)[3 * f + 2]}, etv[3] = {wsc * ST(S_EXTT)[3 * f], wsc * ST(S_EXTT)[3 * f + 1], wsc * ST(S_EXTT)[3 * f + 2]};
-      const float *ef = efv, *et = etv;
-      const float m = mass[f]; const float* I = inertia + 3 * f; const float *w = V, *v = V + 3;
-      float Iw[3] = {I[0] * w[0], I[1] * w[1], I[2] * w[2]}, t[3], fw[3], pa[3], pl[3];
-      v_cross(pa, w, Iw);
-      v_cross(t, w, v); v_scale(pl, t, m);
-      fw[0] = sc.g[0] * m + ef[0]; fw[1] = sc.g[1] * m + ef[1]; fw[2] = sc.g[2] * m + ef[2];
-      mT_vec(t, K, fw); v_sub(pl, pl, t);
-      mT_vec(t, K, et); v_sub(pa, pa, t);
-      const float wn = v_len(w), vn = v_len(v);
-      const bool dlin = (sc.sem & SEM_DAMPING_LINEAR) != 0;
-      v_madd(pa, Iw, dlin ? ka : ka + ka * wn);
-      float mv[3]; v_scale(mv, v, m); v_madd(pl, mv, dlin ? kl : kl + kl * vn);
-      float z[40]; for (int i = 0; i < 40; i++) z[i] = 0.f;
-      for (int i = 0; i < 3; i++) { z[AB_PA + i] = pa[i]; z[AB_PA + 3 + i] = pl[i]; z[AB_WV + i] = w[i]; z[AB_WV + 3 + i] = v[i]; }
-      z[AB_A] = I[0]; z[AB_A + 4] = I[1]; z[AB_A + 8] = I[2]; z[AB_C] = m; z[AB_C + 4] = m; z[AB_C + 8] = m;
-      stn<40>(X, z);
-    }
+    frame_record<BIAS>(C, b, kind, f, k < 0, K, V, ABA(s));
     for (int i = 0; i < 12; i++) Kp[i] = K[i];
     for (int i = 0; i < 6; i++) Vp[i] = V[i];
     prev = s;
@@ -251,52 +267,50 @@
       Out[i][j] = v;
     }
 }
-DG_FN void aba_body(const Env& C, int b, float h) {
+DG_HD void aba_p2_link(const Env& C, int gl, float* Xr, float* c) {
+  const int* li = shc(C.link_i) + DG_LINK_I_W * gl;
+  float Lr[12], cx[8];
+  ldn<12>(LNK(gl), Lr); ldn<8>(LNX(gl), cx);
+  float* Aa = Xr + AB_A; float* Ba = Xr + AB_B; float* Ca = Xr + AB_C; const float* pA = Xr + AB_PA;
+  float pa[6], n[3], fo[3];
+  if (li[3] >= 0) {
+    const float* lx = shc(C.link_x) + 16 * gl; const float *sa = lx + 9, *sl = lx + 12;
+    float U[6];
+    ia_mul(Aa, Ba, Ca, sa, sl, U, U + 3);
+    const float D = v_dot(sa, U) + v_dot(sl, U + 3);
+    const float uu = DOF(D_TAU, li[3]) - (v_dot(sa, pA) + v_dot(sl, pA + 3));
+    float* L = LNK(gl);
+    st4(L + 12, U[0], U[1], U[2], U[3]); st4(L + 16, U[4], U[5], D, 0.f);
+    LNX(gl)[6] = uu;
+    const float Dinv = 1.0f / D;
+#pragma unroll
+    for (int i = 0; i < 3; i++)
+#pragma unroll
+      for (int j = 0; j < 3; j++) { Aa[3 * i + j] -= U[i] * U[j] * Dinv; Ba[3 * i + j] -= U[i] * U[3 + j] * Dinv; Ca[3 * i + j] -= U[3 + i] * U[3 + j] * Dinv; }
+    ia_mul(Aa, Ba, Ca, cx, cx + 3, n, fo);
+    for (int i = 0; i < 3; i++) { pa[i] = pA[i] + n[i] + U[i] * uu * Dinv; pa[3 + i] = pA[3 + i] + fo[i] + U[3 + i] * uu * Dinv; }
+  } else {
+    ia_mul(Aa, Ba, Ca, cx, cx + 3, n, fo);
+    for (int i = 0; i < 3; i++) { pa[i] = pA[i] + n[i]; pa[3 + i] = pA[3 + i] + fo[i]; }
+  }
+  const float* E = Lr; const float* r = Lr + 9;
+  float T1[9], Ar[9], Br[9], Cr[9];
+  mT_mul(T1, E, Aa); m_mul(Ar, T1, E); mT_mul(T1, E, Ba); m_mul(Br, T1, E); mT_mul(T1, E, Ca); m_mul(Cr, T1, E);
+  const float Kx[9] = {0, -r[2], r[1], r[2], 0, -r[0], -r[1], r[0], 0};
+  float KC[9], BK[9], KBt[9], KCK[9];
+  m_mul(KC, Kx, Cr); m_mul(BK, Br, Kx); m_mulT(KBt, Kx, Br); m_mul(KCK, KC, Kx);
+  float t[3];
+  mT_vec(c + 30, E, pa + 3); mT_vec(c + 27, E, pa); v_cross(t, r, c + 30); v_add(c + 27, c + 27, t);
+  for (int i = 0; i < 9; i++) { c[i] = Ar[i] - BK[i] + KBt[i] - KCK[i]; c[9 + i] = Br[i] + KC[i]; c[18 + i] = Cr[i]; }
+}
+DG_HD void aba_add(float* Pr, const float* c) {
+  for (int i = 0; i < 9; i++) { Pr[AB_A + i] += c[i]; Pr[AB_B + i] += c[9 + i]; Pr[AB_C + i] += c[18 + i]; }
+  for (int i = 0; i < 3; i++) { Pr[AB_PA + i] += c[27 + i]; Pr[AB_PA + 3 + i] += c[30 + i]; }
+}
+DG_FN void aba_base(const Env& C, int b) {
   const DevScene& sc = SC;
   const int* bi = gc(sc.body_i) + DG_BODY_I_W * b; const int* bp = gc(sc.body_plan) + BP_W * b;
-  const int kind = bi[0], l0 = bi[1], nlb = bi[2], s0 = bp[BP_SLOT], di = bp[BP_DI];
-  for (int k = nlb - 1; k >= 0; k--) {
-    const int gl = l0 + k, s = s0 + 1 + k; const int* li = shc(C.link_i) + DG_LINK_I_W * gl;
-    const int ps = parent_slot(li, l0, s0);
-    float Xr[40], Lr[12], cx[8];
-    ldn<40>(ABA(s), Xr); ldn<12>(LNK(gl), Lr); ldn<8>(LNX(gl), cx);
-    float* Aa = Xr + AB_A; float* Ba = Xr + AB_B; float* Ca = Xr + AB_C; const float* pA = Xr + AB_PA;
-    float pa[6], n[3], fo[3];
-    if (li[3] >= 0) {
-      const float* lx = shc(C.link_x) + 16 * gl; const float *sa = lx + 9, *sl = lx + 12;
-      float U[6];
-      ia_mul(Aa, Ba, Ca, sa, sl, U, U + 3);
-      const float D = v_dot(sa, U) + v_dot(sl, U + 3);
-      const float uu = DOF(D_TAU, li[3]) - (v_dot(sa, pA) + v_dot(sl, pA + 3));
-      float* L = LNK(gl);
-      st4(L + 12, U[0], U[1], U[2], U[3]); st4(L + 16, U[4], U[5], D, 0.f);
-      LNX(gl)[6] = uu;
-      const float Dinv = 1.0f / D;
-#pragma unroll
-      for (int i = 0; i < 3; i++)
-#pragma unroll
-        for (int j = 0; j < 3; j++) { Aa[3 * i + j] -= U[i] * U[j] * Dinv; Ba[3 * i + j] -= U[i] * U[3 + j] * Dinv; Ca[3 * i + j] -= U[3 + i] * U[3 + j] * Dinv; }
-      ia_mul(Aa, Ba, Ca, cx, cx + 3, n, fo);
-      for (int i = 0; i < 3; i++) { pa[i] = pA[i] + n[i] + U[i] * uu * Dinv; pa[3 + i] = pA[3 + i] + fo[i] + U[3 + i] * uu * Dinv; }
-    } else {
-      ia_mul(Aa, Ba, Ca, cx, cx + 3, n, fo);
-      for (int i = 0; i < 3; i++) { pa[i] = pA[i] + n[i]; pa[3 + i] = pA[3 + i] + fo[i]; }
-    }
-    const float* E = Lr; const float* r = Lr + 9;
-    float T1[9], Ar[9], Br[9], Cr[9];
-    mT_mul(T1, E, Aa); m_mul(Ar, T1, E); mT_mul(T1, E, Ba); m_mul(Br, T1, E); mT_mul(T1, E, Ca); m_mul(Cr, T1, E);
-    const float Kx[9] = {0, -r[2], r[1], r[2], 0, -r[0], -r[1], r[0], 0};
-    float KC[9], BK[9], KBt[9], KCK[9];
-    m_mul(KC, Kx, Cr); m_mul(BK, Br, Kx); m_mulT(KBt, Kx, Br); m_mul(KCK, KC, Kx);
-    float fp[3], np_[3], t[3];
-    mT_vec(fp, E, pa + 3); mT_vec(np_, E, pa); v_cross(t, r, fp); v_add(np_, np_, t);
-    float* P = ABA(ps);
-    float Pr[40];
-    ldn<40>(P, Pr);
-    for (int i = 0; i < 9; i++) { Pr[AB_A + i] += Ar[i] - BK[i] + KBt[i] - KCK[i]; Pr[AB_B + i] += Br[i] + KC[i]; Pr[AB_C + i] += Cr[i]; }
-    for (int i = 0; i < 3; i++) { Pr[AB_PA + i] += np_[i]; Pr[AB_PA + 3 + i] += fp[i]; }
-    stn<40>(P, Pr);
-  }
+  const int kind = bi[0], s0 = bp[BP_SLOT];
   float* X0 = ABA(s0); float* a0 = X0 + AB_ACC;
 #if defined(DG_OLD_INV)
   if (kind == 2) {
@@ -330,61 +344,155 @@
       a0[i] = sum; }
   } else for (int i = 0; i < 6; i++) a0[i] = 0.f;
 #endif
+}
+DG_HD void aba_p3_link(const Env& C, int gl, int s, const float* ap, float h, float* acc) {
+  const int* li = shc(C.link_i) + DG_LINK_I_W * gl;
+  float Lr[20], cx[8];
+  ldn<20>(LNK(gl), Lr); ldn<8>(LNX(gl), cx);
+  float t[3], t2[3];
+  m_vec(acc, Lr, ap); v_cross(t, ap, Lr + 9); v_add(t2, ap + 3, t); m_vec(acc + 3, Lr, t2);
+  v_add(acc, acc, cx); v_add(acc + 3, acc + 3, cx + 3);
+  if (li[3] >= 0) {
+    const float* lx = shc(C.link_x) + 16 * gl;
+    const float qdd = (cx[6] - (v_dot(Lr + 12, acc) + v_dot(Lr + 15, acc + 3))) / Lr[18];
+    DOF(D_QD, li[3]) += h * qdd;
+    v_madd(acc, lx + 9, qdd); v_madd(acc + 3, lx + 12, qdd);
+  }
+  acc[6] = 0.f; acc[7] = 0.f;
+  stn<8>(ABA(s) + AB_ACC, acc);
+}
+DG_FN void base_velocity(const Env& C, int b, float h) {
+  const DevScene& sc = SC;
+  const int* bp = gc(sc.body_plan) + BP_W * b;
+  const int s0 = bp[BP_SLOT], di = bp[BP_DI];
+  if (gc(sc.body_i)[DG_BODY_I_W * b] == 2) {
+    const float* X0 = ABA(s0); const float* a0 = X0 + AB_ACC;
+    const float* K0 = KIN(s0); float* bs = BST(di); float t[3], lin[3], aw[3];
+    v_cross(t, X0 + AB_WV, X0 + AB_WV + 3); v_add(lin, a0 + 3, t);
+    m_vec(aw, K0, a0); v_madd(bs + 10, aw, h);
+    m_vec(aw, K0, lin); v_madd(bs + 7, aw, h);
+  }
+}
+DG_FN void aba_body(const Env& C, int b, float h) {
+  const DevScene& sc = SC;
+  const int* bi = gc(sc.body_i) + DG_BODY_I_W * b; const int* bp = gc(sc.body_plan) + BP_W * b;
+  const int l0 = bi[1], nlb = bi[2], s0 = bp[BP_SLOT];
+  for (int k = nlb - 1; k >= 0; k--) {
+    const int gl = l0 + k, s = s0 + 1 + k; const int* li = shc(C.link_i) + DG_LINK_I_W * gl;
+    float Xr[40], c[33];
+    ldn<40>(ABA(s), Xr);
+    aba_p2_link(C, gl, Xr, c);
+    float* P = ABA(parent_slot(li, l0, s0));
+    float Pr[40];
+    ldn<40>(P, Pr);
+    aba_add(Pr, c);
+    stn<40>(P, Pr);
+  }
+  aba_base(C, b);
   float ap[8]; int prev = s0;
-  ldn<8>(a0, ap);
+  ldn<8>(ABA(s0) + AB_ACC, ap);
   for (int k = 0; k < nlb; k++) {
     const int gl = l0 + k, s = s0 + 1 + k; const int* li = shc(C.link_i) + DG_LINK_I_W * gl;
     const int ps = parent_slot(li, l0, s0);
     if (ps != prev) ldn<8>(ABA(ps) + AB_ACC, ap);
-    float Lr[20], cx[8];
-    ldn<20>(LNK(gl), Lr); ldn<8>(LNX(gl), cx);
-    float t[3], t2[3], acc[8];
-    m_vec(acc, Lr, ap); v_cross(t, ap, Lr + 9); v_add(t2, ap + 3, t); m_vec(acc + 3, Lr, t2);
-    v_add(acc, acc, cx); v_add(acc + 3, acc + 3, cx + 3);
-    if (li[3] >= 0) {
-      const float* lx = shc(C.link_x) + 16 * gl;
-      const float qdd = (cx[6] - (v_dot(Lr + 12, acc) + v_dot(Lr + 15, acc + 3))) / Lr[18];
-      DOF(D_QD, li[3]) += h * qdd;
-      v_madd(acc, lx + 9, qdd); v_madd(acc + 3, lx + 12, qdd);
-    }
-    acc[6] = 0.f; acc[7] = 0.f;
-    stn<8>(ABA(s) + AB_ACC, acc);
+    float acc[8];
+    aba_p3_link(C, gl, s, ap, h, acc);
     for (int i = 0; i < 8; i++) ap[i] = acc[i];
     prev = s;
   }
-  if (kind == 2) {
-    const float* K0 = KIN(s0); float* bs = BST(di); float t[3], lin[3], aw[3];
-    v_cross(t, X0 + AB_WV, X0 + AB_WV + 3); v_add(lin, a0 + 3, t);
-    m_vec(aw, K0, a0); v_madd(bs + 10, aw, h);
-    m_vec(aw, K0, lin); v_madd(bs + 7, aw, h);
-  }
-}
-
+  base_velocity(C, b, h);
+}
+
+DG_HD void joint_reaction_link(const Env& C, int gl, int s) {
+  float X[48], n[3], f[3];
+  ldn<48>(ABA(s), X);
+  ia_mul(X + AB_A, X + AB_B, X + AB_C, X + AB_ACC, X + AB_ACC + 3, n, f);
+  float* o = ST(S_JREACT) + 6 * gl;
+  for (int i = 0; i < 3; i++) { o[i] = X[AB_PA + 3 + i] + f[i]; o[3 + i] = X[AB_PA + i] + n[i]; }
+}
 DG_FN void joint_reactions(const Env& C, int b) {
   const DevScene& sc = SC;
   const int* bi = gc(sc.body_i) + DG_BODY_I_W * b; const int l0 = bi[1], nlb = bi[2], s0 = gc(sc.body_plan)[BP_W * b + BP_SLOT];
-  for (int k = 0; k < nlb; k++) {
-    float X[48], n[3], f[3];
-    ldn<48>(ABA(s0 + 1 + k), X);
-    ia_mul(X + AB_A, X + AB_B, X + AB_C, X + AB_ACC, X + AB_ACC + 3, n, f);
-    float* o = ST(S_JREACT) + 6 * (l0 + k);
-    for (int i = 0; i < 3; i++) { o[i] = X[AB_PA + 3 + i] + f[i]; o[3 + i] = X[AB_PA + i] + n[i]; }
-  }
+  for (int k = 0; k < nlb; k++) joint_reaction_link(C, l0 + k, s0 + 1 + k);
 }
 DG_FN void phase_dynamics(const Env& C, int ln, int nt, float h) {
   for (int di = ln; di < SC.ndyn; di += nt) { int b = gc(SC.dyn_body)[di]; fk_vel_body<true>(C, b); aba_body(C, b, h); if (SC.need_react) joint_reactions(C, b); }
 }
 
-DG_FN void minv_column(const Env& C, int b, int col, float* scr) {
+#define CTB(gl) (WSG(C, SC.X_CTB) + 36 * (gl))
+template <class F> DG_HD void level_links(const Env& C, int ln, int nt, int lev, F&& f) {
+  const DevScene& sc = SC;
+  int item = 0;
+  for (int di = 0; di < sc.ndyn; di++) {
+    const int* tb = gc(sc.tree_body) + 4 * di;
+    if (lev >= tb[1]) continue;
+    const int* lv = gc(sc.tree_lvl) + tb[0];
+    const int b = gc(sc.dyn_body)[di];
+    for (int j = lv[lev]; j < lv[lev + 1]; j++, item++) if (item % nt == ln) f(di, b, gc(sc.tree_link)[j]);
+  }
+}
+DG_HD int link_slot(const Env& C, int b, int gl) { return gc(SC.body_plan)[BP_W * b + BP_SLOT] + 1 + gl - gc(SC.body_i)[DG_BODY_I_W * b + 1]; }
+DG_HD void gather_children(const Env& C, int f, int s, float* Xr) {
+  ldn<40>(ABA(s), Xr);
+  const int k0 = gc(SC.tree_kid)[f], k1 = gc(SC.tree_kid)[f + 1];
+  for (int j = k0; j < k1; j++) { float c[36]; ldn<36>(CTB(gc(SC.tree_kids)[j]), c); aba_add(Xr, c); }
+  if (k1 > k0) stn<40>(ABA(s), Xr);
+}
+DG_FN void phase_tree_base(const Env& C, int ln, int nt) {
+  for (int di = ln; di < SC.ndyn; di += nt) {
+    const int b = gc(SC.dyn_body)[di]; const int s0 = gc(SC.body_plan)[BP_W * b + BP_SLOT];
+    float K[12], V[6];
+    base_frame(C, b, K, V);
+    stn<12>(KIN(s0), K);
+    frame_record<true>(C, b, gc(SC.body_i)[DG_BODY_I_W * b], b, true, K, V, ABA(s0));
+  }
+}
+DG_FN void phase_tree_p1(const Env& C, int ln, int nt, int lev) {
+  level_links(C, ln, nt, lev, [&](int, int b, int gl) {
+    const int* bi = gc(SC.body_i) + DG_BODY_I_W * b; const int s0 = gc(SC.body_plan)[BP_W * b + BP_SLOT];
+    const int ps = parent_slot(shc(C.link_i) + DG_LINK_I_W * gl, bi[1], s0), s = s0 + 1 + gl - bi[1];
+    float Kp[12], Vp[6], K[12], V[6];
+    ldn<12>(KIN(ps), Kp); const float* pv = ABA(ps) + AB_WV; for (int i = 0; i < 6; i++) Vp[i] = pv[i];
+    fk_link<true>(C, gl, Kp, Vp, K, V);
+    stn<12>(KIN(s), K);
+    frame_record<true>(C, b, bi[0], SC.nb + gl, false, K, V, ABA(s));
+  });
+}
+DG_FN void phase_tree_p2(const Env& C, int ln, int nt, int lev) {
+  level_links(C, ln, nt, lev, [&](int, int b, int gl) {
+    float Xr[40], c[36];
+    gather_children(C, SC.nb + gl, link_slot(C, b, gl), Xr);
+    aba_p2_link(C, gl, Xr, c);
+    c[33] = 0.f; c[34] = 0.f; c[35] = 0.f;
+    stn<36>(CTB(gl), c);
+  });
+}
+DG_FN void phase_tree_root(const Env& C, int ln, int nt, float h) {
+  for (int di = ln; di < SC.ndyn; di += nt) {
+    const int b = gc(SC.dyn_body)[di];
+    float Xr[40];
+    gather_children(C, b, gc(SC.body_plan)[BP_W * b + BP_SLOT], Xr);
+    aba_base(C, b);
+    base_velocity(C, b, h);
+  }
+}
+DG_FN void phase_tree_p3(const Env& C, int ln, int nt, int lev, float h) {
+  level_links(C, ln, nt, lev, [&](int, int b, int gl) {
+    const int* bi = gc(SC.body_i) + DG_BODY_I_W * b; const int s0 = gc(SC.body_plan)[BP_W * b + BP_SLOT];
+    const int ps = parent_slot(shc(C.link_i) + DG_LINK_I_W * gl, bi[1], s0), s = s0 + 1 + gl - bi[1];
+    float ap[8], acc[8];
+    ldn<8>(ABA(ps) + AB_ACC, ap);
+    aba_p3_link(C, gl, s, ap, h, acc);
+    if (SC.need_react) joint_reaction_link(C, gl, s);
+  });
+}
+
+DG_HD void minv_up(const Env& C, int b, int col, float* out, float* uu, int us, float* a0) {
   const DevScene& sc = SC;
   const int* bi = gc(sc.body_i) + DG_BODY_I_W * b; const int* bp = gc(sc.body_plan) + BP_W * b;
-  const int kind = bi[0], l0 = bi[1], nlb = bi[2], d0 = bi[3], s0 = bp[BP_SLOT], g = bp[BP_GDIM], gs = bp[BP_GS];
+  const int kind = bi[0], l0 = bi[1], nlb = bi[2], d0 = bi[3], s0 = bp[BP_SLOT];
   const int jo = kind == 2 ? 6 : 0;
-  float* out = WSH(C, sc.W_MINV) + bp[BP_MINVOFF] + col * gs;
-  for (int i = g; i < gs; i++) out[i] = 0.f;
-  (void)scr;
-  float uu[DG_MINV_MAXL], ast[6 * DG_MINV_MAXD];
-  for (int k = 0; k < nlb; k++) uu[k] = 0.f;
+  for (int k = 0; k < nlb; k++) uu[k * us] = 0.f;
   float p[6] = {0, 0, 0, 0, 0, 0};
   if (col >= jo) {
     int k0 = -1;
@@ -396,7 +504,7 @@
       if (li[3] >= 0) {
         const float* lx = shc(C.link_x) + 16 * gl;
         const float u1 = (k == k0 ? 1.f : 0.f) - (v_dot(lx + 9, pa) + v_dot(lx + 12, pa + 3));
-        uu[k] = u1; const float s = u1 / L[18];
+        uu[k * us] = u1; const float s = u1 / L[18];
         for (int i = 0; i < 6; i++) pa[i] += L[12 + i] * s;
       }
       float fp[3], np_[3], t[3];
@@ -405,7 +513,6 @@
       k = li[1] < 0 ? -1 : li[1] - l0;
     }
   }
-  float a0[6];
   if (kind == 2) {
     float K0[12]; ldn<12>(KIN(s0), K0); const float* Iv = WSG(C, sc.W_I0) + bp[BP_I0OFF];
     float gen[6] = {0, 0, 0, 0, 0, 0}, rhs[6], t[3];
@@ -414,6 +521,28 @@
     for (int i = 0; i < 6; i++) { float s = 0.f; for (int j = 0; j < 6; j++) s += Iv[6 * i + j] * rhs[j]; a0[i] = s; }
     m_vec(out, K0, a0); m_vec(out + 3, K0, a0 + 3);
   } else for (int i = 0; i < 6; i++) a0[i] = 0.f;
+}
+DG_HD void minv_down_link(const Env& C, const int* li, const float* lx, const float* L, float u, const float* ap, float* aa, float* al, float* row) {
+  float t[3], t2[3];
+  m_vec(aa, L, ap); v_cross(t, ap, L + 9); v_add(t2, ap + 3, t); m_vec(al, L, t2);
+  if (li[3] >= 0) {
+    const float qdd = (u - (v_dot(L + 12, aa) + v_dot(L + 15, al))) / L[18];
+    *row = qdd;
+    v_madd(aa, lx + 9, qdd); v_madd(al, lx + 12, qdd);
+  }
+}
+
+DG_FN void minv_column(const Env& C, int b, int col, float* scr) {
+  const DevScene& sc = SC;
+  const int* bi = gc(sc.body_i) + DG_BODY_I_W * b; const int* bp = gc(sc.body_plan) + BP_W * b;
+  const int kind = bi[0], l0 = bi[1], nlb = bi[2], d0 = bi[3], g = bp[BP_GDIM], gs = bp[BP_GS];
+  const int jo = kind == 2 ? 6 : 0;
+  float* out = WSH(C, sc.W_MINV) + bp[BP_MINVOFF] + col * gs;
+  for (int i = g; i < gs; i++) out[i] = 0.f;
+  (void)scr;
+  float uu[DG_MINV_MAXL], ast[6 * DG_MINV_MAXD];
+  float a0[6];
+  minv_up(C, b, col, out, uu, 1, a0);
   for (int i = 0; i < 6; i++) ast[i] = a0[i];
   float ap[6] = {a0[0], a0[1], a0[2], a0[3], a0[4], a0[5]}; int prev_dep = -1;
   for (int k = 0; k < nlb; k++) {
@@ -421,14 +550,8 @@
     const int dep = gc(sc.link_depth)[gl];
     if (dep - 1 != prev_dep) { const float* src = ast + 6 * dep; for (int i = 0; i < 6; i++) ap[i] = src[i]; }
     float L[20]; ldn<20>(LNK(gl), L);
-    float t[3], t2[3], aa[3], al[3];
-    m_vec(aa, L, ap); v_cross(t, ap, L + 9); v_add(t2, ap + 3, t); m_vec(al, L, t2);
-    if (li[3] >= 0) {
-      const float* lx = shc(C.link_x) + 16 * gl;
-      const float qdd = (uu[k] - (v_dot(L + 12, aa) + v_dot(L + 15, al))) / L[18];
-      out[jo + li[3] - d0] = qdd;
-      v_madd(aa, lx + 9, qdd); v_madd(al, lx + 12, qdd);
-    }
+    float aa[3], al[3];
+    minv_down_link(C, li, shc(C.link_x) + 16 * gl, L, uu[k], ap, aa, al, out + jo + li[3] - d0);
     float* ak = ast + 6 * (dep + 1);
     v_cpy(ak, aa); v_cpy(ak + 3, al);
     v_cpy(ap, aa); v_cpy(ap + 3, al); prev_dep = dep;
@@ -442,6 +565,41 @@
     int b = gc(sc.dyn_body)[di], g = gc(sc.body_plan)[BP_W * b + BP_GDIM];
     for (int col = 0; col < g; col++, item++) if (item % nt == ln) minv_column(C, b, col, scr);
   }
+}
+DG_FN void phase_minv_up(const Env& C, int ln, int nt) {
+  const DevScene& sc = SC;
+  int item = 0;
+  for (int di = 0; di < sc.ndyn; di++) {
+    const int b = gc(sc.dyn_body)[di]; const int* bp = gc(sc.body_plan) + BP_W * b;
+    const int g = bp[BP_GDIM], gs = bp[BP_GS], nlb = gc(sc.body_i)[DG_BODY_I_W * b + 2];
+    float* mu = WSG(C, sc.X_MACC) + gc(sc.tree_body)[4 * di + 2]; float* ma = mu + ((nlb * g + 3) & ~3);
+    for (int col = 0; col < g; col++, item++) if (item % nt == ln) {
+      float* out = WSH(C, sc.W_MINV) + bp[BP_MINVOFF] + col * gs;
+      for (int i = g; i < gs; i++) out[i] = 0.f;
+      float a0[6];
+      minv_up(C, b, col, out, mu + col, g, a0);
+      st4(ma + 8 * col, a0[0], a0[1], a0[2], a0[3]); st4(ma + 8 * col + 4, a0[4], a0[5], 0.f, 0.f);
+    }
+  }
+}
+DG_FN void phase_minv_level(const Env& C, int ln, int nt, int lev) {
+  level_links(C, ln, nt, lev, [&](int di, int b, int gl) {
+    const DevScene& sc = SC;
+    const int* bi = gc(sc.body_i) + DG_BODY_I_W * b; const int* bp = gc(sc.body_plan) + BP_W * b;
+    const int l0 = bi[1], nlb = bi[2], d0 = bi[3], g = bp[BP_GDIM], gs = bp[BP_GS], jo = bi[0] == 2 ? 6 : 0;
+    const int* li = shc(C.link_i) + DG_LINK_I_W * gl; const float* lx = shc(C.link_x) + 16 * gl;
+    const int k = gl - l0, pn = li[1] < 0 ? 0 : 1 + li[1] - l0;
+    const float* mu = WSG(C, sc.X_MACC) + gc(sc.tree_body)[4 * di + 2] + k * g; float* ma = WSG(C, sc.X_MACC) + gc(sc.tree_body)[4 * di + 2] + ((nlb * g + 3) & ~3);
+    float* row = WSH(C, sc.W_MINV) + bp[BP_MINVOFF] + jo + li[3] - d0;
+    float L[20]; ldn<20>(LNK(gl), L);
+    for (int col = 0; col < g; col++) {
+      float ap[8], aa[3], al[3];
+      ldn<8>(ma + 8 * (pn * g + col), ap);
+      minv_down_link(C, li, lx, L, mu[col], ap, aa, al, row + col * gs);
+      float* o = ma + 8 * ((k + 1) * g + col);
+      st4(o, aa[0], aa[1], aa[2], al[0]); st4(o + 4, al[1], al[2], 0.f, 0.f);
+    }
+  });
 }
 
 struct Ct { int fa, fb; float pa[3], pb[3], n[3], dist, mu; };
@@ -1866,7 +2024,8 @@
 
 DG_NOINLINE DG_FN void physics_pre(const Env& C, int nt, float h, DG_LANE_ARGS) {
   const DevScene& sc = SC;
-  DG_PHASE(phase_dynamics(C, ln, nt, h));
+  if (!sc.tree_levels) DG_PHASE(phase_dynamics(C, ln, nt, h));
+  else { DG_PHASE(phase_tree_base(C, ln, nt)); for (int l = 0; l < sc.tree_nlev; l++) DG_PHASE(phase_tree_p1(C, ln, nt, l)); for (int l = sc.tree_nlev - 1; l >= 0; l--) DG_PHASE(phase_tree_p2(C, ln, nt, l)); DG_PHASE(phase_tree_root(C, ln, nt, h)); for (int l = 0; l < sc.tree_nlev; l++) DG_PHASE(phase_tree_p3(C, ln, nt, l, h)); }
   DG_PHASE(phase_shape_world(C, ln, nt));
   if (sc.npair > 0) {
     DG_PHASE(phase_broad(C, ln, nt));
@@ -1876,7 +2035,7 @@
       DG_PHASE(phase_append(C, ln, nt));
     }
   }
-  DG_PHASE(phase_minv(C, ln, nt));
+  if (!sc.tree_levels) DG_PHASE(phase_minv(C, ln, nt)); else { DG_PHASE(phase_minv_up(C, ln, nt)); for (int l = 0; l < sc.tree_nlev; l++) DG_PHASE(phase_minv_level(C, ln, nt, l)); }
   DG_PHASE(phase_unit_rows(C, ln, nt, h));
   if (sc.ncons == 0 && !block_any(HDRV(WH_NCROW) > 0, nt)) {
     DG_PHASE(phase_pgs_unit(C, ln, nt, 0, sc.iters));
diff --git a/diy_gym_b200/csrc/dg_scene.h b/diy_gym_b200/csrc/dg_scene.h
--- a/diy_gym_b200/csrc/dg_scene.h
+++ b/diy_gym_b200/csrc/dg_scene.h
@@ -57,6 +57,14 @@
   int crow_stride, mscr_stride, ctmp_stride, ik_stride;
   int sem;
   int precise;
+  int tree_levels, tree_nlev;
+  const int* tree_body;
+  const int* tree_lvl;
+  const int* tree_link;
+  const int* tree_kid;
+  const int* tree_kids;
+  int X_CTB;
+  int X_MACC;
 };
 
 #define DG_SO(sc, name) ((sc)->so[HI_##name - HI_S_BPOS])
@@ -67,6 +75,7 @@
 #ifndef __CUDACC_RTC__
 #include <algorithm>
 #include <cmath>
+#include <cstdlib>
 #include <string>
 #include <vector>
 
@@ -79,6 +88,7 @@
   std::string error;
 
   struct Off { size_t body_i, link_i, shape_i, pair_i, vis_i, op_i, oparg_i, cam_i, dyn_body, body_plan, frame_slot, link_depth, shape_slot, grp_i, grp_pairs, loose_pairs;
+               size_t tree_body, tree_lvl, tree_link, tree_kid, tree_kids;
                size_t body_f, link_f, shape_f, vis_f, oparg_f, cam_f, param_def, state_def, shape_wb, vis_wb, link_x, body_reach, cons_i, cons_f, hull_f; } off;
 
   static void quat_to_mat(const double* q, double* m) {
@@ -99,6 +109,7 @@
     d.oparg_f = fb + off.oparg_f; d.cam_f = fb + off.cam_f; d.param_def = fb + off.param_def; d.state_def = fb + off.state_def;
     d.shape_wb = fb + off.shape_wb; d.vis_wb = fb + off.vis_wb; d.link_x = fb + off.link_x;
     d.cons_i = ib + off.cons_i; d.cons_f = fb + off.cons_f; d.hull_f = fb + off.hull_f;
+    d.tree_body = ib + off.tree_body; d.tree_lvl = ib + off.tree_lvl; d.tree_link = ib + off.tree_link; d.tree_kid = ib + off.tree_kid; d.tree_kids = ib + off.tree_kids;
   }
 
   bool build(const int32_t* ibuf, int ni, const double* fbuf, int nf, int team, int ws_mode = 0, int rs_ashared = 0) {
@@ -245,12 +256,40 @@
     d.need_react = hi[HI_S_STEP] > hi[HI_S_JREACT];
     d.precise = d.ncons > 0; d.sem = hi[HI_semantics];
 
+    std::vector<int> tree_body(std::max((size_t)1, 4 * dyn_body.size()), 0), tree_lvl, tree_link, tree_kid(d.nframes + 1, 0), tree_kids;
+    int macc = 0;
+    d.tree_nlev = 0;
+    d.tree_levels = dyn_body.empty() ? 0 : 1;
+    for (size_t di = 0; di < dyn_body.size(); di++) {
+      const int b = dyn_body[di]; const int32_t* bi = body_i + DG_BODY_I_W * b; const int l0 = bi[1], nlb = bi[2];
+      const int nlev = nlb > 0 ? body_plan[(size_t)b * BP_W + BP_DEPTH] + 1 : 0, gdim = body_plan[(size_t)b * BP_W + BP_GDIM];
+      if (nlb == 0 || 2 * nlev > nlb) d.tree_levels = 0;
+      tree_body[4 * di] = (int)tree_lvl.size(); tree_body[4 * di + 1] = nlev; tree_body[4 * di + 2] = macc; d.tree_nlev = std::max(d.tree_nlev, nlev);
+      for (int j = 0; j < nlev; j++) {
+        tree_lvl.push_back((int)tree_link.size());
+        for (int k = 0; k < nlb; k++) if (link_depth[l0 + k] == j) tree_link.push_back(l0 + k);
+      }
+      tree_lvl.push_back((int)tree_link.size());
+      macc += ((nlb * gdim + 3) & ~3) + 8 * (nlb + 1) * gdim;
+    }
+    {
+      std::vector<std::vector<int>> kids(d.nframes);
+      for (int b = 0; b < d.nb; b++) {
+        const int32_t* bi = body_i + DG_BODY_I_W * b; const int l0 = bi[1], nlb = bi[2];
+        for (int k = nlb - 1; k >= 0; k--) { int pl = link_i[DG_LINK_I_W * (l0 + k) + 1]; kids[pl < 0 ? b : d.nb + pl].push_back(l0 + k); }
+      }
+      for (int f = 0; f < d.nframes; f++) { tree_kid[f] = (int)tree_kids.size(); tree_kids.insert(tree_kids.end(), kids[f].begin(), kids[f].end()); }
+      tree_kid[d.nframes] = (int)tree_kids.size();
+    }
+    if (const char* env_tree = getenv("DG_TREE_LEVELS")) d.tree_levels = atoi(env_tree) != 0;
+
     auto put_vi = [&](const std::vector<int>& v) { size_t o = ints.size(); ints.insert(ints.end(), v.begin(), v.end()); ints.push_back(0); return o; };
     auto put_vf = [&](const std::vector<float>& v) { size_t o = floats.size(); floats.insert(floats.end(), v.begin(), v.end()); floats.push_back(0.f); return o; };
     off.dyn_body = put_vi(dyn_body); off.body_plan = put_vi(body_plan); off.frame_slot = put_vi(frame_slot);
     off.link_depth = put_vi(link_depth); off.shape_slot = put_vi(shape_slot);
     off.shape_wb = put_vf(shape_wb); off.vis_wb = put_vf(vis_wb); off.link_x = put_vf(link_x); off.body_reach = put_vf(body_reach);
     off.grp_i = put_vi(grp_i); off.grp_pairs = put_vi(grp_pairs); off.loose_pairs = put_vi(loose_pairs);
+    off.tree_body = put_vi(tree_body); off.tree_lvl = put_vi(tree_lvl); off.tree_link = put_vi(tree_link); off.tree_kid = put_vi(tree_kid); off.tree_kids = put_vi(tree_kids);
     point(d, ints.data(), floats.data());
 
     d.ndyn = (int)dyn_body.size(); d.nslot = nslot; d.nshw = nshw; d.nfloat = nfloat; d.GD = GD; d.GP = GP;
@@ -291,6 +330,7 @@
     phase_take(&d.X_ABA, RC_ABA, 0, AB_W * nslot);
     phase_take(&d.X_LNK, RC_ABA, 0, LX_W * d.nl);
     phase_take(&d.X_I0T, RC_ABA, 0, 36 * nfloat);
+    phase_take(&d.X_CTB, RC_ABA, 0, d.tree_levels ? 36 * d.nl : 0);
     phase_take(&d.X_SHW, RC_CONTACT, 1, 12 * nshw);
     phase_take(&d.X_CON, RC_CONTACT, 1, CT_W * d.maxc);
     phase_take(&d.X_SURV, RC_CONTACT, 1, (d.npair + 31) / 32 + 1);
@@ -315,6 +355,7 @@
     phase_take(&d.X_RSA, RC_SCRATCH, 1, d.rs_cap * d.rs_cap + RS_KMAX * team);
     phase_take(&d.X_RSV, RC_SCRATCH, 1, d.rs_cap * 2 * gv);
     phase_take(&d.X_RSREC, RC_SCRATCH, 1, d.rs_cap * RR_W);
+    phase_take(&d.X_MACC, RC_SCRATCH, 1, d.tree_levels ? macc : 0);
     phase_take(&d.X_IK, RC_SCRATCH, 2, n_ik ? d.ik_stride * std::min(team, n_ik) : 0);
     for (auto& pd : pend) *pd.field = enc_rc(pd.rc, pd.cold, fix[pd.cold] + pd.rel);
     d.w_total = fix[0] + std::max(ph[0][0], std::max(ph[0][1], ph[0][2]));
```

Measured after the change: 2.400 million (median of 6 runs). -6.3%, worse.
